# cafferychen777/flashdeconv

Hardware: AMD Instinct MI355X
Metric: spots/sec to convergence (1M x 2000 x 30) (higher is better)
Workload: dtype f64

## Files before the change

flashdeconv_amd/_lib.py:

```python
import ctypes
import os
import threading

import numpy as np

_HERE = os.path.dirname(os.path.abspath(__file__))
LIB_PATH = os.path.join(_HERE, "libfdx.so")

c_int = ctypes.c_int
c_i32 = ctypes.c_int32
c_i64 = ctypes.c_int64
c_double = ctypes.c_double
c_void_p = ctypes.c_void_p
c_size_t = ctypes.c_size_t
p_double = ctypes.POINTER(ctypes.c_double)
p_i64 = ctypes.POINTER(ctypes.c_int64)
p_i32 = ctypes.POINTER(ctypes.c_int32)


class FdxError(RuntimeError):
    """A libfdx call failed (message from fdx_last_error())."""


class SolveInfo(ctypes.Structure):
    _fields_ = [
        ("converged", c_i32),
        ("n_iterations", c_i32),
        ("final_objective", c_double),
        ("final_change", c_double),
        ("n_objectives", c_i32),
        ("reserved", c_i32),
        ("sweep_ms", c_double),
        ("total_ms", c_double),
    ]

    def as_dict(self, rel_changes=None, objective=True):
        n_it = int(self.n_iterations)
        d = {"converged": bool(self.converged), "n_iterations": n_it, "final_change": float(self.final_change)}
        if objective:
            d["final_objective"] = float(self.final_objective)
        if rel_changes is not None:
            d["rel_changes"] = [float(v) for v in rel_changes[:n_it]]
        return d


class FitParams(ctypes.Structure):
    _fields_ = [
        ("sketch_dim", c_i32), ("mode_y", c_i32), ("mode_x", c_i32), ("graph_method", c_i32), ("k_neighbors", c_i32),
        ("lambda_auto", c_i32), ("max_iter", c_i32), ("verbose", c_i32),
        ("radius", c_double), ("lambda_spatial", c_double), ("rho_sparsity", c_double), ("tol", c_double),
        ("stop_on_ties", c_i32), ("reserved", c_i32), ("carry", c_void_p), ("spot_diag_out_dev", c_void_p),
    ]


class ShardFitParams(ctypes.Structure):
    _fields_ = [("sketch_dim", c_i32), ("mode_y", c_i32), ("mode_x", c_i32), ("lambda_auto", c_i32), ("max_iter", c_i32),
                ("stop_on_ties", c_i32), ("lambda_spatial", c_double), ("rho_sparsity", c_double), ("tol", c_double),
                ("n_total_spots", c_i64), ("nnz_total", c_i64), ("X_dev", c_void_p)]


class ShardFitInfo(ctypes.Structure):
    _fields_ = [("status", c_i32), ("reserved", c_i32), ("nnz_total", c_i64), ("knn_ties_total", c_i64), ("own_nnz", c_i64),
                ("n_halo", c_i64), ("lambda_used", c_double), ("rho_effective", c_double), ("YtY", c_double), ("solve", SolveInfo)]


SHARD_FAR, SHARD_OVERFLOW, SHARD_TIES = 1, 2, 3


class CsrView(ctypes.Structure):
    _fields_ = [("indptr", c_void_p), ("indices", c_void_p), ("data", c_void_p), ("dtype", c_i32), ("n", c_i64),
                ("nnz", c_i64), ("G", c_i32), ("sorted_rows", c_i32)]


class FitInfo(ctypes.Structure):
    _fields_ = [
        ("solve", SolveInfo), ("lambda_used", c_double), ("rho_effective", c_double), ("YtY", c_double), ("nnz", c_i64),
        ("graph_ms", c_double), ("sketch_ms", c_double), ("gram_ms", c_double), ("solve_ms", c_double),
        ("finish_ms", c_double), ("total_ms", c_double), ("prologue_ms", c_double), ("span_ms", c_double),
        ("knn_ties", c_i64), ("status", c_i32), ("reserved", c_i32), ("carry", c_void_p), ("diag_ms", c_double),
    ]


FIT_TIES = 3


GRAPH_KNN, GRAPH_RADIUS, GRAPH_GIVEN = 0, 1, 2

SIGNATURES = {
    "fdx_column_sums_dev": (c_int, [c_void_p, c_i32, c_i64, c_i32, c_i64, p_double, c_void_p]),
    "fdx_leverage_scores": (c_int, [p_double, c_i32, c_i32, c_double, p_double]),
    "fdx_csr_check_dev": (c_int, [ctypes.POINTER(CsrView), c_void_p]),
    "fdx_csr_gene_moments_dev": (c_int, [ctypes.POINTER(CsrView), p_double, p_double, p_double, c_void_p]),
    "fdx_fit_csr_dev": (c_int, [ctypes.POINTER(CsrView), p_i32, c_i32, p_double, c_i32, p_i32, p_double, p_double, c_void_p,
                                c_i32, ctypes.POINTER(FitParams), ctypes.POINTER(c_void_p), c_void_p, c_void_p, p_double,
                                p_double, ctypes.POINTER(FitInfo), c_void_p]),
    "fdx_type_sums_dev": (c_int, [c_void_p, c_i32, c_i64, c_i32, c_i64, c_void_p, c_void_p, c_i32, c_i32, c_void_p, c_void_p]),
    "fdx_type_sums_csr_dev": (c_int, [ctypes.POINTER(CsrView), c_void_p, c_void_p, c_i32, c_i32, c_void_p, c_void_p]),
    "fdx_metrics_moments_dev": (c_int, [c_void_p, c_void_p, c_i32, c_i64, c_i32, c_i64, c_i64, c_double, c_double, c_void_p,
                                        p_double, p_i64, c_void_p]),
    "fdx_metrics_spearman_dev": (c_int, [c_void_p, c_void_p, c_i32, c_i64, c_i32, c_i64, c_i64, c_i32, p_double, c_void_p]),
    "fdx_metrics_evaluate_dev": (c_int, [c_void_p, c_void_p, c_i32, c_i64, c_i32, c_i64, c_i64, c_double, c_double, c_i32,
                                         c_void_p, p_double, p_i64, p_double, c_void_p]),
    "fdx_graph_build_radius_rows_dev": (c_int, [c_void_p, c_i64, c_i32, c_double, c_i64, c_i64, c_void_p, ctypes.POINTER(c_void_p)]),
    "fdx_graph_knn_lists_dev": (c_int, [c_void_p, c_i64, c_i32, c_i32, c_i64, c_i64, c_void_p, c_void_p, c_void_p,
                                        ctypes.POINTER(c_void_p)]),
    "fdx_graph_knn_lists_band_dev": (c_int, [c_void_p, c_i64, c_i32, c_i32, c_i64, c_i64, c_void_p, c_void_p, c_void_p,
                                             ctypes.POINTER(c_void_p)]),
    "fdx_graph_from_knn_lists_dev": (c_int, [c_void_p, c_void_p, c_void_p, c_i64, c_i64, c_void_p, ctypes.POINTER(c_void_p)]),
    "fdx_leverage_begin": (c_int, [p_double, c_i32, c_i32, c_double, ctypes.POINTER(c_void_p)]),
    "fdx_leverage_begin_opt": (c_int, [p_double, c_i32, c_i32, c_double, c_i32, ctypes.POINTER(c_void_p)]),
    "fdx_leverage_end": (c_int, [c_void_p, p_double]),
    "fdx_leverage_end_keep": (c_int, [c_void_p, p_double, ctypes.POINTER(c_void_p)]),
    "fdx_fit_dev": (c_int, [c_void_p, c_i32, c_i64, c_i32, c_i64, p_double, c_i32, p_i32, p_double, p_double, c_void_p,
                            c_i32, ctypes.POINTER(FitParams), ctypes.POINTER(c_void_p), c_void_p, c_void_p, p_double,
                            p_double, ctypes.POINTER(FitInfo), c_void_p]),
    "fdx_fit_carry_free": (c_int, [c_void_p]),
    "fdx_graph_build_dev": (c_int, [c_void_p, c_i64, c_i32, c_i32, c_i32, c_double, c_void_p, ctypes.POINTER(c_void_p)]),
    "fdx_graph_perm_dev": (c_int, [c_void_p, c_void_p, c_void_p]),
    "fdx_side_stream": (c_int, [ctypes.POINTER(c_void_p)]),
    "fdx_stream_wait_stream": (c_int, [c_void_p, c_void_p]),
    "fdx_graph_localize": (c_int, [c_void_p, c_i32, p_i64, c_i32, c_void_p, ctypes.POINTER(c_void_p)]),
    "fdx_graph_shard_knn_dev": (c_int, [c_void_p, c_i64, c_i32, c_i32, c_i32, p_i64, c_i32, c_void_p, ctypes.POINTER(c_void_p)]),
    "fdx_graph_shard_status": (c_int, [c_void_p, p_i64, p_i64, p_i32, p_i32]),
    "fdx_graph_row_indices": (c_int, [c_void_p, c_i64, p_i32, c_i32, p_i32]),
    "fdx_graph_tile_info": (c_int, [c_void_p, p_i32, p_i32, p_i32]),
    "fdx_graph_halo_info": (c_int, [c_void_p, p_i64, p_i32, p_i32]),
    "fdx_graph_send_indices_dev": (c_int, [c_void_p, c_void_p, c_void_p]),
    "fdx_prepare_dev": (c_int, [c_void_p, c_i32, c_i64, c_i32, c_i64, c_void_p, p_double, c_i32, p_i32, p_double, p_double,
                                c_i32, c_i32, c_i32, c_void_p, c_i64, c_void_p, p_double, p_double, c_void_p]),
    "fdx_init_beta_dev": (c_int, [c_void_p, c_i64, c_i64, c_i32, c_void_p]),
    "fdx_bcd_sweep_dev": (c_int, [c_void_p, c_void_p, c_i64, c_void_p, c_void_p, c_void_p, c_i64, c_i32, c_double, c_double,
                                  c_double, c_i32, c_void_p, c_void_p, c_void_p]),
    "fdx_bcd_fold_dev": (c_int, [c_void_p, c_void_p, c_i32, c_void_p]),
    "fdx_objective_partials_dev": (c_int, [c_void_p, c_void_p, c_i64, c_void_p, c_i64, c_void_p, c_i32, p_double, c_void_p]),
    "fdx_spot_diagnostics_dev": (c_int, [c_void_p, c_void_p, c_i64, c_void_p, c_i64, c_void_p, c_i32, c_i32, c_void_p, c_void_p,
                                         c_void_p]),
    "fdx_spatial_autocorr_dev": (c_int, [c_void_p, c_void_p, c_i64, c_i32, p_double, p_double, p_double, p_i64, c_void_p, c_void_p]),
    "fdx_spatial_perm_dev": (c_int, [c_void_p, c_void_p, c_i64, c_i32, ctypes.c_uint64, c_i64, c_i64, c_i32, c_void_p, p_double,
                                     p_double, p_double, p_i64, p_double, p_i64, p_i64, p_double, p_double, p_i32, c_void_p]),
    "fdx_permutation_indices_dev": (c_int, [ctypes.c_uint64, c_i64, c_i64, c_void_p, c_void_p]),
    "fdx_kmeans_assign_dev": (c_int, [c_void_p, c_i64, c_i64, c_i32, c_void_p, c_i32, c_void_p, c_void_p, p_i64, p_double, c_void_p]),
    "fdx_label_sums_dev": (c_int, [c_void_p, c_i64, c_i64, c_i32, c_void_p, c_i32, p_double, p_i64, c_void_p]),
    "fdx_kmeans_seed_dist_dev": (c_int, [c_void_p, c_i64, c_i64, c_i32, c_void_p, c_void_p, p_double, p_i64, p_i32, c_void_p]),
    "fdx_kmeans_dev": (c_int, [c_void_p, c_i64, c_i64, c_i32, c_i32, c_i32, c_void_p, c_void_p, p_i64, p_double, p_i32, p_i32,
                               c_void_p]),
    "fdx_normalize_dev": (c_int, [c_void_p, c_i64, c_i64, c_i32, c_void_p, c_void_p, c_void_p]),
    "fdx_export_dev": (c_int, [c_void_p, c_void_p, c_i64, c_i32, c_void_p, c_void_p, c_void_p]),
    "fdx_gene_moments_dev": (c_int, [c_void_p, c_i32, c_i64, c_i32, c_i64, p_double, p_double, c_void_p]),
    "fdx_gather_columns_dev": (c_int, [c_void_p, c_i32, c_i64, c_i32, c_i64, p_i32, c_i32, c_void_p, c_void_p]),
    "fdx_version": (c_int, []),
    "fdx_env_reload": (c_int, []),
    "fdx_env_switch": (ctypes.c_char_p, [c_i32, ctypes.POINTER(ctypes.c_char_p)]),
    "fdx_last_error": (ctypes.c_char_p, []),
    "fdx_device_count": (c_int, [ctypes.POINTER(c_int)]),
    "fdx_set_device": (c_int, [c_int]),
    "fdx_device_name": (c_int, [ctypes.c_char_p, c_int]),
    "fdx_malloc": (c_int, [ctypes.POINTER(c_void_p), c_size_t]),
    "fdx_free": (c_int, [c_void_p]),
    "fdx_trim": (c_int, []),
    "fdx_x_cache_stats": (c_int, [p_i64]),
    "fdx_memcpy_h2d": (c_int, [c_void_p, c_void_p, c_size_t, c_void_p]),
    "fdx_memcpy_d2h": (c_int, [c_void_p, c_void_p, c_size_t, c_void_p]),
    "fdx_memset": (c_int, [c_void_p, c_int, c_size_t, c_void_p]),
    "fdx_upload_convert_dev": (c_int, [c_void_p, c_i32, c_void_p, c_i32, c_i64, p_double, c_void_p]),
    "fdx_download_dev": (c_int, [c_void_p, c_void_p, c_size_t, c_void_p]),
    "fdx_pinned_copy_rate": (c_int, [c_size_t, c_i32, p_double]),
    "fdx_stream_sync": (c_int, [c_void_p]),
    "fdx_sketch": (c_int, [c_void_p, c_i32, c_i64, c_i32, p_i64, p_i32, p_double, c_i32, c_i32, p_double]),
    "fdx_prepare_csr_dev": (c_int, [ctypes.POINTER(CsrView), p_i32, c_i32, p_double, c_i32, p_i32, p_double, p_double, c_i32, c_i32,
                                    c_i32, c_void_p, c_i64, c_void_p, p_double, ctypes.POINTER(c_double), c_void_p]),
    "fdx_gram_xty": (c_int, [p_double, p_double, c_i64, c_i32, c_i32, p_double, p_double]),
    "fdx_objective": (c_int, [c_void_p, p_double, p_double, p_double, c_i64, c_i32, c_double, c_double, c_double, p_double]),
    "fdx_comm_unique_id": (c_int, [c_void_p]),
    "fdx_comm_init": (c_int, [c_void_p, c_i32, c_i32, ctypes.POINTER(c_void_p)]),
    "fdx_local_world_create": (c_int, [c_i32, ctypes.POINTER(c_void_p)]),
    "fdx_local_world_destroy": (c_int, [c_void_p]),
    "fdx_comm_init_local": (c_int, [c_void_p, c_i32, ctypes.POINTER(c_void_p)]),
    "fdx_comm_init_loopback": (c_int, [c_i32, c_i32, ctypes.POINTER(c_void_p)]),
    "fdx_comm_destroy": (c_int, [c_void_p]),
    "fdx_comm_info": (c_int, [c_void_p, p_i32, p_i32]),
    "fdx_comm_rccl_count": (c_int, [c_void_p, p_i32]),
    "fdx_comm_allreduce_sum_dev": (c_int, [c_void_p, c_void_p, c_i32, c_void_p]),
    "fdx_sharded_solve_dev": (c_int, [c_void_p, c_void_p, c_void_p, c_i64, c_void_p, c_i32, c_double, c_double, c_double, c_i32,
                                      c_void_p, c_void_p, c_i64, ctypes.POINTER(SolveInfo), p_double, p_i32, c_void_p]),
    "fdx_solver_padded_k": (c_i32, [c_i32]),
    "fdx_shard_fit_dev": (c_int, [c_void_p, c_void_p, c_void_p, c_i32, c_i64, c_i32, c_i64, p_double, c_i32, p_i32, p_double, p_double,
                                  ctypes.POINTER(ShardFitParams), c_void_p, c_void_p, p_double, ctypes.POINTER(ShardFitInfo), c_void_p]),
    "fdx_sharded_solve_padded_dev": (c_int, [c_void_p, c_void_p, c_void_p, c_i64, c_void_p, c_i32, c_i32, c_double, c_double, c_double,
                                             c_i32, c_void_p, c_void_p, c_i64, ctypes.POINTER(SolveInfo), p_double, p_i32, c_void_p]),
    "fdx_tile_schedule": (c_int, [p_i32, p_double, c_i32, c_i32, c_i32, c_i32, c_i32, p_i32, p_i32, c_void_p, p_i32, p_double,
                                  c_void_p, c_i64]),
    "fdx_sketch_path": (c_int, [c_i32, c_void_p, c_i64, c_i32, c_i32, c_i32, c_i32, p_i32, p_double, p_i32, p_i32]),
    "fdx_column_sums": (c_int, [c_void_p, c_i32, c_i64, c_i32, p_double]),
    "fdx_log1p_f32": (c_int, [c_void_p, ctypes.c_float, c_i64, c_void_p]),
    "fdx_graph_build_knn": (c_int, [p_double, c_i64, c_i32, c_i32, ctypes.POINTER(c_void_p)]),
    "fdx_graph_build_radius": (c_int, [p_double, c_i64, c_i32, c_double, ctypes.POINTER(c_void_p)]),
    "fdx_nearest_distance": (c_int, [p_double, c_i64, c_i32, p_double]),
    "fdx_graph_export_csr": (c_int, [c_void_p, p_i64, p_i32]),
    "fdx_graph_from_csr": (c_int, [p_i64, p_i64, c_i64, ctypes.POINTER(c_void_p)]),
    "fdx_graph_destroy": (c_int, [c_void_p]),
    "fdx_graph_info": (c_int, [c_void_p, p_i64, p_i64, p_i32]),
    "fdx_graph_knn_ties": (c_int, [c_void_p, p_i64]),
    "fdx_graph_knn_far": (c_int, [c_void_p, ctypes.POINTER(c_i32)]),
    "fdx_kdtree_set_threads": (c_int, [c_i32]),
    "fdx_kdtree_tune": (c_int, [c_i32, c_i64]),
    "fdx_ckdtree_indices_dev": (c_int, [c_void_p, c_i64, c_i32, p_i64, p_i32, c_void_p]),
    "fdx_ckdtree_prebuild": (c_int, [p_double, c_void_p, c_i64, c_i32]),
    "fdx_hvg_from_moments": (c_int, [p_double, p_double, c_i32, p_double, c_i32, c_i32, c_double, c_double, c_double, p_i64,
                                     ctypes.POINTER(c_i32), ctypes.POINTER(c_i32)]),
    "fdx_ckdtree_knn": (c_int, [p_double, c_i64, c_i32, c_i32, c_void_p, c_void_p]),
    "fdx_ckdtree_knn_rows": (c_int, [p_double, c_i64, c_i32, c_i32, p_i64, c_i64, c_void_p]),
    "fdx_graph_plan_set_ckdtree_lists_dev": (c_int, [c_void_p, p_double, c_void_p, c_i64, c_i32, c_void_p, c_i64, c_void_p, c_void_p, c_void_p]),
    "fdx_graph_plan_order_dev": (c_int, [c_void_p, c_void_p, c_void_p, c_void_p]),
    "fdx_graph_plan_lists_replaced": (c_int, [c_void_p]),
    "fdx_graph_plan_set_lists_dev": (c_int, [c_void_p, c_void_p, c_void_p, c_i64, c_void_p, c_void_p, c_void_p]),
    "fdx_bcd_solve": (c_int, [c_void_p, p_double, p_double, c_i64, c_i32, c_i32, c_double, c_double, c_i32, c_double,
                              c_i32, p_double, p_double, p_double, ctypes.POINTER(SolveInfo)]),
}

_lock = threading.Lock()
_lib = None


def _preload_shared_hip_runtime():
    import importlib.util
    try:
        spec = importlib.util.find_spec("torch")
    except (ImportError, ValueError):
        spec = None
    if spec is None or not spec.submodule_search_locations:
        return
    libdir = os.path.join(list(spec.submodule_search_locations)[0], "lib")
    for name in ("libhsa-runtime64.so", "libamdhip64.so"):
        path = os.path.join(libdir, name)
        if os.path.exists(path):
            try:
                ctypes.CDLL(path, mode=ctypes.RTLD_GLOBAL)
            except OSError:
                pass


def load():
    global _lib
    with _lock:
        if _lib is None:
            if not os.path.exists(LIB_PATH):
                raise FdxError(
                    f"{LIB_PATH} not found: build it with `make -C flashdeconv_amd/csrc` "
                    "(or `python -c 'import __graft_entry__ as g; g.build()'`). There is no CPU fallback.")
            _preload_shared_hip_runtime()
            lib = ctypes.CDLL(LIB_PATH)
            for name, (res, args) in SIGNATURES.items():
                fn = getattr(lib, name)
                fn.restype = res
                fn.argtypes = args
            _lib = lib
    return _lib


def env_reload():
    if _lib is not None:
        _lib.fdx_env_reload()


def runtime_switches():
    lib, out, i = load(), [], 0
    while True:
        what = ctypes.c_char_p()
        name = lib.fdx_env_switch(i, ctypes.byref(what))
        if not name:
            return out
        out.append((name.decode(), (what.value or b"").decode()))
        i += 1


def check(rc):
    if rc != 0:
        msg = load().fdx_last_error()
        raise FdxError(f"libfdx error {rc}: {msg.decode() if msg else 'unknown'}")


def require_gpu():
    lib = load()
    n = c_int(0)
    rc = lib.fdx_device_count(ctypes.byref(n))
    if rc != 0 or n.value <= 0:
        raise FdxError("flashdeconv_amd needs an AMD Instinct GPU (gfx950); no HIP device is visible "
                       "and there is no CPU fallback.")
    return n.value


def host_cpu_budget():
    cpus = float(len(os.sched_getaffinity(0))) if hasattr(os, "sched_getaffinity") else float(os.cpu_count() or 1)
    try:
        with open("/sys/fs/cgroup/cpu.max") as f:
            q, period = f.read().split()[:2]
        if q != "max" and float(period) > 0:
            cpus = min(cpus, float(q) / float(period))
    except (OSError, ValueError):
        try:
# ... 319 lines not shown
```

flashdeconv_amd/core/deconv.py:

```python
import ctypes
import os
import sys
import time

import numpy as np
from scipy import sparse

from .. import _lib
from ..utils import genes as _genes
from .sketching import sketch_tables

_PRE_MODES = ("log_cpm", "pearson", "raw")


def _is_torch_cuda(x):
    return hasattr(x, "data_ptr") and hasattr(x, "is_cuda") and bool(x.is_cuda)


def device_counts_as_float(Y):
    import torch
    f64_math = False
    if Y.dtype not in (torch.float32, torch.float64):
        f64_math = not Y.dtype.is_floating_point
        small = Y.dtype in (torch.uint8, torch.int8, torch.int16, torch.bool, torch.float16, torch.bfloat16)
# ... 284 lines not shown
                      file=sys.stderr)
            if G != G_all and csr is None:
                sub = _DeviceBuffer(n * G * (4 if y_code == _lib.FDX_F32 else 8))
                owned.append(sub)
                gi32 = np.ascontiguousarray(gene_idx, dtype=np.int32)
                _lib.check(lib.fdx_gather_columns_dev(y_ptr, y_code, n, G_all, G_all, _lib.ptr_i32(gi32), G, sub.ptr, None))
                y_ptr = sub.ptr
            ldy = G

            if big_k:
                from ..utils.graph import ckdtree_knn_adjacency
                t_graph = time.perf_counter()
                A = ckdtree_knn_adjacency(coords_host if coords_host is not None else _lib.tensor_to_host(coords), int(self.k_neighbors))
                self._graph = _lib.Graph.from_csr(A.indptr, A.indices, n)
                self._adjacency = A
            elif not graph_early:
                t_graph = time.perf_counter()
                gh = ctypes.c_void_p()
                _lib.check(lib.fdx_graph_build_dev(c_ptr, n, dim, g_method, g_k, g_radius, None, ctypes.byref(gh)))
                self._graph = _lib.Graph(gh.value)
            n_ties = 0
            if self.spatial_method == "knn" and self.knn_ties == "ckdtree" and not big_k:
                n_ties = self._graph.knn_ties()
                if n_ties:
                    self._graph.close()
                    self._graph = None
                    self._graph = reference_tie_graph(c_ptr, coords_host, n, dim, int(self.k_neighbors))
            t_lev = time.perf_counter()
            leverage = lev_job.result()
            t_done = time.perf_counter()

            log(f"Step 2: Preprocessing with method='{self.preprocess}'...")

            def y_colsum():
                if csr is not None:
                    return (csr_colsum if csr_colsum is not None else csr.gene_moments(want_colsum=True)[2])[gene_idx]
                sums = np.empty(G, dtype=np.float64)
                _lib.check(lib.fdx_column_sums_dev(y_ptr, y_code, n, G, ldy, _lib.ptr_f64(sums), None))
                return sums
            bucket32, wy, wx, mode_y, mode_x = sketch_tables(
                G, self.sketch_dim, leverage, self.random_state, self.preprocess, Xsel, y_sparse=y_sparse_rule,
                f64_math=y_f64_math and csr is None and y_code == _lib.FDX_F32, y_colsum=y_colsum, n_spots=n)
            log({"log_cpm": "  Y and X normalized to log-CPM space", "pearson": "  Y and X transformed with uncentered Pearson residuals",
                 "raw": "  No preprocessing applied (raw)"}[self.preprocess])
            log(f"Step 3: Sketching to {self.sketch_dim} dimensions...")
            log(f"  Compressed {G} genes -> {self.sketch_dim} dims")

            prm = _lib.FitParams()
            prm.sketch_dim = int(self.sketch_dim)
            prm.mode_y, prm.mode_x = mode_y, mode_x
            prm.k_neighbors = int(self.k_neighbors)
            prm.max_iter, prm.tol, prm.verbose = int(self.max_iter), float(self.tol), 1 if self.verbose else 0
            prm.rho_sparsity = float(self.rho_sparsity)
            prm.lambda_auto = 1 if self.lambda_spatial == "auto" else 0
            prm.lambda_spatial = 0.0 if prm.lambda_auto else float(self.lambda_spatial)
            prm.radius = 0.0
            prm.graph_method = _lib.GRAPH_GIVEN
            prm.stop_on_ties = 1 if (self.spatial_method == "knn" and self.knn_ties == "auto" and not big_k) else 0
            log("Step 4: Building spatial graph...")

            if output == "torch":
                import torch
                dev = Y.device if _is_torch_cuda(Y) else torch.device("cuda", torch.cuda.current_device())
                beta_t = torch.empty((n, K), dtype=torch.float64, device=dev)
                prop_t = torch.empty((n, K), dtype=torch.float64, device=dev)
                b_ptr, p_ptr = beta_t.data_ptr(), prop_t.data_ptr()
            else:
                bbuf, pbuf = _DeviceBuffer(n * K * 8), _DeviceBuffer(n * K * 8)
                owned += [bbuf, pbuf]
                b_ptr, p_ptr = bbuf.ptr, pbuf.ptr

            diag_t = dbuf = None
            if spot_diagnostics:
                if output == "torch":
                    diag_t = torch.empty(3 * n, dtype=torch.float64, device=dev)
                    prm.spot_diag_out_dev = diag_t.data_ptr()
                else:
                    dbuf = _DeviceBuffer(3 * n * 8)
                    owned.append(dbuf)
                    prm.spot_diag_out_dev = dbuf.ptr
            objs = np.zeros(max(int(self.max_iter), 1), dtype=np.float64)
            rels = np.zeros(max(int(self.max_iter), 1), dtype=np.float64)
            info = _lib.FitInfo()
            gh = ctypes.c_void_p(self._graph.handle.value)
            t_call = time.perf_counter()
            gi32 = np.ascontiguousarray(gene_idx, dtype=np.int32)

            def run_fit():
                if csr is not None:
                    _lib.check(lib.fdx_fit_csr_dev(ctypes.byref(csr.view), _lib.ptr_i32(gi32), G, _lib.ptr_f64(Xsel), K,
                                                   _lib.ptr_i32(bucket32), _lib.ptr_f64(wy), _lib.ptr_f64(wx), c_ptr, dim,
                                                   ctypes.byref(prm), ctypes.byref(gh), b_ptr, p_ptr, _lib.ptr_f64(objs),
                                                   _lib.ptr_f64(rels), ctypes.byref(info), None))
                else:
                    _lib.check(lib.fdx_fit_dev(y_ptr, y_code, n, G, ldy, _lib.ptr_f64(Xsel), K, _lib.ptr_i32(bucket32),
                                               _lib.ptr_f64(wy), _lib.ptr_f64(wx), c_ptr, dim, ctypes.byref(prm),
                                               ctypes.byref(gh), b_ptr, p_ptr, _lib.ptr_f64(objs), _lib.ptr_f64(rels),
                                               ctypes.byref(info), None))

            run_fit()
            ties_remedy_ms = 0.0
            if info.status == _lib.FIT_TIES:
                n_ties = int(info.knn_ties)
                log(f"k-NN ties on {n_ties} of {n} spots: rebuilding the graph on the reference's (cKDTree) neighbour choice")
                stale, carry = self._graph, info.carry
                self._graph = None
                try:
                    self._graph = reference_tie_graph(c_ptr, coords_host, n, dim, int(self.k_neighbors))
                    gh = ctypes.c_void_p(self._graph.handle.value)
                    prm.stop_on_ties = 0
                    prm.carry, carry = carry, None
                    ties_resolved_here = True
                    ties_remedy_ms = (time.perf_counter() - t_call) * 1e3
                    t_call = time.perf_counter()
                    run_fit()
                finally:
                    if carry:
                        lib.fdx_fit_carry_free(carry)
                    stale.close()
            else:
                ties_resolved_here = False
            t_ret = time.perf_counter()
            if os.environ.get("FDX_TRACE_HOST"):
                print(f"[fdx-host] python: entry->build {1e6 * (t_graph - t_entry):.0f} us, build call {1e6 * (t_lev - t_graph):.0f}, leverage wait "
                      f"{1e6 * (t_done - t_lev):.0f}, tables + setup {1e6 * (t_call - t_done):.0f}, fit call {1e6 * (t_ret - t_call):.0f}", file=sys.stderr)
            if output == "torch":
                self.beta_, self.proportions_ = beta_t, prop_t
            else:
                self.beta_ = bbuf.to_host((n, K), out=self._recyclable("beta_", (n, K)))
                self.proportions_ = pbuf.to_host((n, K), out=self._recyclable("proportions_", (n, K)))
            self.spot_diagnostics_ = None
            if spot_diagnostics:
                planes = diag_t if diag_t is not None else dbuf.to_host((3 * n,))
                self.spot_diagnostics_ = {name: planes[j * n:(j + 1) * n]
                                          for j, name in enumerate(("residual_sq", "sketch_sq", "neighbor_sq"))}
        finally:
            for b in owned:
                b.free()

        log(f"  Average neighbors per spot: {info.nnz / max(n, 1):.1f}")
        self.lambda_used_ = float(info.lambda_used)
        log(f"Step 5: {'Auto-tuned' if prm.lambda_auto else 'Using'} lambda = {self.lambda_used_:.4f}")
        log("Step 6: Solving via Block Coordinate Descent...")
        n_it = int(info.solve.n_iterations)
        objectives = [float(v) for v in objs[:info.solve.n_objectives]]
        if self.verbose:
            its = [t for t in range(n_it) if t % 10 == 0 or t == self.max_iter - 1]
            for t, obj in zip(its, objectives):
                print(f"Iteration {t}: objective = {obj:.6f}, rel_change = {rels[t]:.6e}")
            if info.solve.converged:
                print(f"Converged at iteration {n_it - 1}")
        self.info_ = info.solve.as_dict()
        self.info_["objectives"] = objectives if self.verbose else []
        resolved = self.spatial_method == "knn" and (self.knn_ties == "ckdtree" or ties_resolved_here)
        self.info_["knn_ties"] = (n_ties if resolved else int(info.knn_ties)) if self.spatial_method == "knn" else 0
        if self.info_["knn_ties"] and not resolved:
            import warnings
            warnings.warn(
                f"k-NN ties: {self.info_['knn_ties']} of {n} spots have their k-th and (k+1)-th nearest neighbours at exactly "
                "the same distance (regular lattice?), so the neighbour graph depends on how ties are broken - here by "
                "spot index, in the reference by cKDTree's traversal, i.e. by the order the spots are listed in.  "
                "Proportions can differ from the reference's by a few 1e-4 (relative); knn_ties='auto' (the default) or "
                "'ckdtree' reproduce the reference's choice (host-side, about a second per million spots), "
                "spatial_method='grid' builds a tie-free graph on lattices.", UserWarning, stacklevel=2)
        self.timings_ = _fit_timings(info, t_entry, t_graph, t_graph_done if graph_early else t_lev, t_sel, t_lev, t_done, t_call, t_ret,
                                     ties_remedy_ms, span_from_call=graph_early or ties_resolved_here or bool(resolved and n_ties))
        if spot_diagnostics:
            self.timings_["diagnostics_ms"] = float(info.diag_ms)
        self._fitted = True
        log(f"  Converged: {self.info_['converged']}")
        log(f"  Iterations: {self.info_['n_iterations']}")
        log("FlashDeconv: Done!")
        return self

    def _recyclable(self, name, shape):
        old = getattr(self, name, None)
        ok = (isinstance(old, np.ndarray) and old.shape == tuple(shape) and old.dtype == np.float64 and old.flags.c_contiguous
              and old.flags.owndata and old.flags.writeable and sys.getrefcount(old) <= 3)
        return old if ok else None

    def _graph_request(self, coords, coords_host):
        if self.spatial_method == "knn":
            return _lib.GRAPH_KNN, int(self.k_neighbors), 0.0
        if self.spatial_method == "radius":
            if self.radius is None:
                raise ValueError("radius must be specified for radius method")
            return _lib.GRAPH_RADIUS, 0, float(self.radius)
        if self.spatial_method == "grid":
            if coords.shape[0] < 2:
                return _lib.GRAPH_KNN, 0, 0.0
            from ..utils.graph import grid_radius
            ch = coords_host if coords_host is not None else _lib.tensor_to_host(coords)
            return _lib.GRAPH_RADIUS, 0, grid_radius(ch)
        raise ValueError(f"Unknown method: {self.spatial_method}. Choose from 'knn', 'radius', 'grid'.")

    def fit_transform(self, Y, X, coords, **kwargs):
        self.fit(Y, X, coords, **kwargs)
        return self.proportions_

    def _require_fitted(self):
        if not self._fitted:
            raise RuntimeError("Model has not been fitted. Call fit() first.")

    def get_cell_type_proportions(self):
        self._require_fitted()
        return self.proportions_

    def get_abundances(self):
        self._require_fitted()
        return self.beta_

    def get_spot_residuals(self, relative=True):
        self._require_fitted()
        if self.spot_diagnostics_ is None:
            raise RuntimeError("No per-spot diagnostics: call fit(..., spot_diagnostics=True) first.")
        res, sq = self.spot_diagnostics_["residual_sq"], self.spot_diagnostics_["sketch_sq"]
        if isinstance(res, np.ndarray):
            if not relative:
                return np.sqrt(res)
            return np.sqrt(np.divide(res, sq, out=np.zeros_like(res), where=sq > 0))
        import torch
        if not relative:
            return torch.sqrt(res)
        return torch.sqrt(torch.where(sq > 0, res / torch.where(sq > 0, sq, torch.ones_like(sq)), torch.zeros_like(res)))

    def get_spatial_autocorrelation(self, what="proportions", neighbor_mean=False, n_permutations=0, random_state=None):
        self._require_fitted()
        if what not in ("proportions", "abundances"):
            raise ValueError(f"Unknown what: {what}. Choose from 'proportions', 'abundances'.")
        from ..utils.spatial_stats import spatial_autocorrelation, spatial_permutation_test, spatial_sums
        values = self.proportions_ if what == "proportions" else self.beta_
        if isinstance(n_permutations, (bool, np.bool_)) or not isinstance(n_permutations, (int, np.integer)) or n_permutations < 0:
            raise ValueError(f"n_permutations must be an int >= 0, got {n_permutations!r}")
        if n_permutations == 0:
            return spatial_autocorrelation(values, self, neighbor_mean=neighbor_mean)
        out = spatial_permutation_test(values, self, n_permutations=n_permutations,
                                       random_state=self.random_state if random_state is None else random_state)
        if neighbor_mean:
            out["neighbor_mean"] = spatial_sums(values, self, neighbor_mean=True)["neighbor_mean"]
        return out

    def get_spatial_niches(self, n_niches, what="proportions", features="both", **kw):
        self._require_fitted()
        if what not in ("proportions", "abundances"):
            raise ValueError(f"Unknown what: {what}. Choose from 'proportions', 'abundances'.")
        from ..utils.niches import spatial_niches
        return spatial_niches(self.proportions_ if what == "proportions" else self.beta_, n_niches, graph=self, features=features,
                              **kw)

    def get_dominant_cell_type(self):
        self._require_fitted()
        if hasattr(self.proportions_, "argmax") and not isinstance(self.proportions_, np.ndarray):
            return self.proportions_.argmax(dim=1)
        return np.argmax(self.proportions_, axis=1)

    def summary(self):
        if not self._fitted:
            return {"fitted": False}
        return {
            "fitted": True,
            "n_spots": self.n_spots_,
            "n_cell_types": self.n_cell_types_,
            "n_genes_used": len(self.gene_idx_),
            "sketch_dim": self.sketch_dim,
            "lambda_spatial": self.lambda_used_,
            "rho_sparsity": self.rho_sparsity,
            "preprocess_method": self.preprocess,
            "converged": self.info_["converged"],
            "n_iterations": self.info_["n_iterations"],
            "final_objective": self.info_["final_objective"],
        }

    def __repr__(self):
        status = "fitted" if self._fitted else "not fitted"
        return f"FlashDeconv(sketch_dim={self.sketch_dim}, lambda_spatial={self.lambda_spatial}, status={status})"
```

flashdeconv_amd/csrc/bcd_sweep_inst.cpp:

```cpp
#include <algorithm>
#include <cstdlib>
#include "bcd_device.h"
#include "fdx_graph.h"

#ifndef FDX_PART
#error "compile with -DFDX_PART=<n> -DFDX_K_LO=<lo> -DFDX_K_HI=<hi>"
#endif

namespace fdx {

constexpr int sweep_chunk(int K) {
#ifdef FDX_KC_OVERRIDE
    return K < FDX_KC_OVERRIDE ? K : FDX_KC_OVERRIDE;
#endif
    return K < 8 ? K : K <= 29 ? 8 : K <= 33 ? 7 : K <= 37 ? 6 : K <= 41 ? 5 : K <= 45 ? 4 : K <= 49 ? 3 : K <= 51 ? 2 : K <= 64 ? 8 : K <= 72 ? 6 : K <= 88 ? 4 : K <= 96 ? 2 : 8;
}

template <int K, int KC>
__global__ __launch_bounds__(256) void bcd_sweep_kernel(
    const double* __restrict__ H, const double* __restrict__ XtX, const double* __restrict__ beta_in,
    double* __restrict__ beta_out, const int* __restrict__ ell_base, const int* __restrict__ slice_off,
    const int* __restrict__ deg, unsigned long long* __restrict__ stats, double* __restrict__ rel_change,
    const double lambda, const double rho, const double tol, const int ldh, const int ld_, const int n,
    const int n_slices, const int it) {
    const int lane = threadIdx.x & 63;
    const int wib = __builtin_amdgcn_readfirstlane(threadIdx.x >> 6);

    if (it > 0) {
        const double rc = fold_rel_change(stats + (size_t)(it - 1) * 128, lane);
        if (blockIdx.x == 0 && threadIdx.x == 0) rel_change[it - 1] = rc;
        if (rc < tol) return;
    }

    const int slice = xcd_remap(blockIdx.x, gridDim.x) * 4 + wib;
    if (slice >= n_slices) return;
    const int i = min(slice * 64 + lane, n - 1);
    const size_t ld = (size_t)ld_;

    const int w0 = slice_off[slice];
    const int w = slice_off[slice + 1] - w0;

    double b[K];
#pragma unroll
    for (int k = 0; k < K; ++k) b[k] = beta_in[k * ld + i];
    const int* ell = ell_base + (size_t)w0 * 64 + (i & 63);
    const int dg = deg[i];
    const double lam_deg = lambda * (double)dg;
    const double lam_eff = (dg > 0) ? lambda : 0.0;

    double dmax = 0.0, amax = 0.0;
#pragma unroll
    for (int kc = 0; kc < K; kc += KC) {
        double c[KC];
#pragma unroll
        for (int q = 0; q < KC; ++q) c[q] = 0.0;
#pragma unroll 2
        for (int m = 0; m < w; ++m) {
            const int j = ell[(size_t)m * 64];
#pragma unroll
            for (int q = 0; q < KC; ++q)
                if (kc + q < K) c[q] += beta_in[(kc + q) * ld + j];
        }
#pragma unroll
        for (int q = 0; q < KC; ++q) {
            const int k = kc + q;
            if (k < K) {
                const double h = H[k * (size_t)ldh + i];
                const double* g = XtX + k * K;
                double r0 = 0.0, r1 = 0.0;
#pragma unroll
                for (int j = 0; j + 1 < K; j += 2) {
                    r0 = fma(g[j], b[j], r0);
                    r1 = fma(g[j + 1], b[j + 1], r1);
                }
                if (K & 1) r0 = fma(g[K - 1], b[K - 1], r0);
                const double gkk = g[k];
                const double old = b[k];
                const double res = (h - (r0 + r1) + gkk * old) + lam_eff * c[q];
                const double den = gkk + lam_deg;
                const double st = res > rho ? res - rho : (res < -rho ? res + rho : 0.0);
                const double qv = fmax(0.0, st / den);
                const double nw = (den > 1e-10) ? qv : 0.0;
                dmax = fmax(dmax, fabs(nw - old));
                amax = fmax(amax, fabs(old));
                b[k] = nw;
                beta_out[k * ld + i] = nw;
            }
        }
    }
    dmax = wave_max(dmax);
    amax = wave_max(amax);
    if (lane == 0) {
        unsigned long long* s = stats + (size_t)it * 128;
        const int slot = slice & 63;
        atomicMax(s + slot, (unsigned long long)__double_as_longlong(dmax));
        atomicMax(s + 64 + slot, (unsigned long long)__double_as_longlong(amax));
    }
}

__device__ __forceinline__ const char __attribute__((address_space(1)))* plane_base(const double* p) {
    unsigned long long v = (unsigned long long)p;
    asm("" : "+s"(v));
    return (const char __attribute__((address_space(1)))*)v;
}

__device__ __forceinline__ unsigned lane_off(unsigned off) {
    asm("" : "+v"(off));
    return off;
}

#ifndef FDX_SWEEP_WPE
#define FDX_SWEEP_WPE 1
#endif
template <int K, int KC, bool OBJ, bool QUAD = true, bool INIT = false>
__global__ __launch_bounds__(256, ((OBJ && K > 40 && K <= 64) || (K > 64 && K <= 96)) ? 2 : (OBJ ? 1 : FDX_SWEEP_WPE)) void bcd_sweep_tiled_kernel(
    const double* __restrict__ H, const double* __restrict__ XtX, const double* __restrict__ beta_in,
    double* __restrict__ beta_out, const unsigned short* __restrict__ ell_local, const int* __restrict__ slice_off,
    const int* __restrict__ deg, const int* __restrict__ tile_halo, const int* __restrict__ tile_hcnt,
    unsigned long long* __restrict__ stats, double* __restrict__ rel_change, const double lambda, const double rho,
    const double tol, const int ldh, const int ld_, const int n, const int S, const int it,
    const int* __restrict__ tile_list, const double init_v, const int* __restrict__ send_head, const int4* __restrict__ send_ent,
    double* __restrict__ send_buf) {
    extern __shared__ __attribute__((aligned(16))) double lds[];
    const int tid = threadIdx.x;
    const int lane = tid & 63;
    const int tile = tile_list ? tile_list[xcd_remap(blockIdx.x, gridDim.x)] : xcd_remap(blockIdx.x, gridDim.x);
    const bool real = (tile * 256 + tid) < n;
    const int i = min(tile * 256 + tid, n - 1);
    const size_t ld = (size_t)ld_;
    const int slice = __builtin_amdgcn_readfirstlane(i >> 6);
    const int w0 = slice_off[slice];
    const int w = slice_off[slice + 1] - w0;
    const int Ht = tile_hcnt[tile];
    const int* halo = tile_halo + (size_t)tile * FDX_TILE_HALO_CAP;
    const int dg = deg[i];
    int hidx0 = halo[tid];
    if (!OBJ && it > 0) {
        const double rc = fold_rel_change(stats + (size_t)(it - 1) * 128, lane);
        if (blockIdx.x == 0 && tid == 0) rel_change[it - 1] = rc;
        asm volatile("" :: "v"(dg), "v"(hidx0), "s"(w0), "s"(w), "s"(Ht));
        if (rc < tol) return;
    }
    hidx0 = (tid < Ht) ? hidx0 : 0;

    const unsigned ioff = (unsigned)i * 8u, hoff = (unsigned)hidx0 * 8u;
#define PLANE_AT(base, off) (*(const double __attribute__((address_space(1)))*)(plane_base(base) + lane_off(off)))
    double b[K];
#pragma unroll
    for (int k = 0; k < K; ++k) b[k] = INIT ? init_v : PLANE_AT(beta_in + k * ld, ioff);
    const unsigned short* ell = ell_local + (size_t)w0 * 64 + (i & 63);
    const double lam_deg = lambda * (double)dg;
    const double lam_eff = (dg > 0) ? lambda : 0.0;
    unsigned slots[8];
    const unsigned zslot = (unsigned)(256 + Ht);
#pragma unroll
    for (int m2 = 0; m2 < 8; ++m2) {
        unsigned lo = (unsigned)__builtin_nontemporal_load(&ell[(size_t)(2 * m2) * 64]);
        unsigned hi = (unsigned)__builtin_nontemporal_load(&ell[(size_t)(2 * m2 + 1) * 64]);
        lo = (2 * m2 < w) ? lo : zslot;
        hi = (2 * m2 + 1 < w) ? hi : zslot;
        slots[m2] = lo | (hi << 16);
    }
    double hv[KC], hreg[KC];
#pragma unroll
    for (int q = 0; q < KC; ++q) {
        hv[q] = INIT ? init_v : PLANE_AT(beta_in + q * ld, hoff);
        hreg[q] = __builtin_nontemporal_load(&PLANE_AT(H + q * (size_t)ldh, ioff));
    }

    double dmax = 0.0, amax = 0.0;
    double o_cross = 0.0, o_quad = 0.0, o_spat = 0.0, o_l1 = 0.0;
#pragma unroll
    for (int kc = 0; kc < K; kc += KC) {
#pragma unroll
        for (int q = 0; q < KC; ++q)
            if (kc + q < K) lds[q * S + tid] = b[kc + q];
        if (tid < Ht) {
#pragma unroll
            for (int q = 0; q < KC; ++q)
                if (kc + q < K) lds[q * S + 256 + tid] = hv[q];
        }
        for (int h = tid + 256; h < Ht; h += 256) {
            const int j = halo[h];
#pragma unroll
            for (int q = 0; q < KC; ++q)
                if (kc + q < K) lds[q * S + 256 + h] = INIT ? init_v : beta_in[(kc + q) * ld + j];
        }
        if (tid < KC) lds[tid * S + 256 + Ht] = 0.0;
        __syncthreads();
        double c[KC];
#pragma unroll
        for (int q = 0; q < KC; ++q) c[q] = 0.0;
#pragma unroll
        for (int m4 = 0; m4 < 16; m4 += 4) {
            if (m4 < w) {
#pragma unroll
                for (int m = m4; m < m4 + 4; ++m) {
                    const int slot = (int)((slots[m >> 1] >> (16 * (m & 1))) & 0xffffu);
#pragma unroll
                    for (int q = 0; q < KC; ++q)
                        if (kc + q < K) c[q] += lds[q * S + slot];
                }
            }
        }
        for (int m = 16; m < w; ++m) {
            const int slot = ell[(size_t)m * 64];
#pragma unroll
            for (int q = 0; q < KC; ++q)
                if (kc + q < K) c[q] += lds[q * S + slot];
        }
        __syncthreads();
#pragma unroll
        for (int q = 0; q < KC; ++q) {
            const int k = kc + q;
            if (k < K) {
                const double h = hreg[q];
                const double* g = XtX + k * K;
                double r0 = 0.0, r1 = 0.0;
                if (!OBJ || QUAD) {
#pragma unroll
                    for (int j = 0; j + 1 < K; j += 2) {
                        r0 = fma(g[j], b[j], r0);
                        r1 = fma(g[j + 1], b[j + 1], r1);
                    }
                    if (K & 1) r0 = fma(g[K - 1], b[K - 1], r0);
                }
                const double gkk = (!OBJ || QUAD) ? g[k] : 0.0;
                const double old = b[k];
                if (OBJ) {
                    o_cross = fma(old, h, o_cross);
                    if (QUAD) o_quad = fma(old, r0 + r1, o_quad);
                    o_spat = fma(old, (double)dg * old - c[q], o_spat);
                    o_l1 += fabs(old);
                    asm volatile("" : "+v"(o_quad));
                } else {
                    const double res = (h - (r0 + r1) + gkk * old) + lam_eff * c[q];
                    const double den = gkk + lam_deg;
                    const double st = res > rho ? res - rho : (res < -rho ? res + rho : 0.0);
                    const double qv = fmax(0.0, st / den);
                    const double nw = (den > 1e-10) ? qv : 0.0;
                    dmax = fmax(dmax, fabs(nw - old));
                    amax = fmax(amax, fabs(old));
                    b[k] = nw;
                    __builtin_nontemporal_store(nw, (double __attribute__((address_space(1)))*)(plane_base(beta_out + k * ld) + lane_off(ioff)));
                }
            }
            if (kc + KC < K) {
#pragma unroll
                for (int t = 2 * q; t < 2 * q + 2; ++t) {
                    const int j = t < KC ? t : t - KC;
                    if (kc + KC + j < K) {
                        if (t < KC) { if (!INIT) hv[j] = PLANE_AT(beta_in + (kc + KC + j) * ld, hoff); }
                        else hreg[j] = __builtin_nontemporal_load(&PLANE_AT(H + (kc + KC + j) * (size_t)ldh, ioff));
                    }
                }
                __builtin_amdgcn_sched_barrier(0);
            }
        }
    }
    if (OBJ) {
        if (!real) { o_cross = o_quad = o_spat = o_l1 = 0.0; }
#pragma unroll
        for (int off = 32; off > 0; off >>= 1) {
            o_cross += __shfl_xor(o_cross, off, 64);
            o_quad += __shfl_xor(o_quad, off, 64);
            o_spat += __shfl_xor(o_spat, off, 64);
            o_l1 += __shfl_xor(o_l1, off, 64);
        }
        __syncthreads();
        if (lane == 0) { lds[(tid >> 6) * 4 + 0] = o_cross; lds[(tid >> 6) * 4 + 1] = o_quad; lds[(tid >> 6) * 4 + 2] = o_spat; lds[(tid >> 6) * 4 + 3] = o_l1; }
        __syncthreads();
        if (tid < 4) rel_change[(size_t)tile * 4 + tid] = ((lds[tid] + lds[4 + tid]) + lds[8 + tid]) + lds[12 + tid];
        return;
    }
    if (!OBJ && send_head != nullptr) {
        int hd = real ? send_head[i] : 0;
        while (hd != 0) {
            const int4 e = send_ent[hd - 1];
            double* o = send_buf + (size_t)K * e.x + e.z;
#pragma unroll
            for (int k = 0; k < K; ++k) o[(size_t)k * e.y] = b[k];
            hd = e.w;
        }
    }
    dmax = wave_max(dmax);
    amax = wave_max(amax);
    if (lane == 0) {
        unsigned long long* s = stats + (size_t)it * 128;
        const int slot = slice & 63;
        atomicMax(s + slot, (unsigned long long)__double_as_longlong(dmax));
        atomicMax(s + 64 + slot, (unsigned long long)__double_as_longlong(amax));
    }
}

template <int K>
static void launch_k(const BcdSweepArgs& a, hipStream_t st) {
    if (a.tiled) {
        constexpr int KC = sweep_chunk(K);
        const int S = 256 + a.halo_max + 1;
        const size_t lds = (size_t)KC * S * sizeof(double);
        if (lds <= 64 * 1024 && (long long)a.ld * 8 < (1LL << 32) && (long long)a.ldh * 8 < (1LL << 32)) {
            if (a.objective) {
                if constexpr (K > 64) {
                    hipLaunchKernelGGL((bcd_sweep_tiled_kernel<K, KC, true, false>), dim3(a.n_tiles), dim3(256), lds, st, a.H, a.XtX,
                                       a.beta_in, a.beta_out, a.ell_local, a.slice_off, a.deg, a.tile_halo, a.tile_hcnt,
                                       a.stats, a.rel_change, a.lambda, a.rho, a.tol, a.ldh, a.ld, a.n, S, a.it, nullptr, 0.0, a.send_head, a.send_ent, a.send_buf);
                } else {
                    hipLaunchKernelGGL((bcd_sweep_tiled_kernel<K, KC, true>), dim3(a.n_tiles), dim3(256), lds, st, a.H, a.XtX,
                                       a.beta_in, a.beta_out, a.ell_local, a.slice_off, a.deg, a.tile_halo, a.tile_hcnt,
                                       a.stats, a.rel_change, a.lambda, a.rho, a.tol, a.ldh, a.ld, a.n, S, a.it, nullptr, 0.0, a.send_head, a.send_ent, a.send_buf);
                }
            }
            else if (a.tile_list) {
                if (a.n_list > 0)
                    hipLaunchKernelGGL((bcd_sweep_tiled_kernel<K, KC, false>), dim3(a.n_list), dim3(256), lds, st, a.H, a.XtX,
                                       a.beta_in, a.beta_out, a.ell_local, a.slice_off, a.deg, a.tile_halo, a.tile_hcnt,
                                       a.stats, a.rel_change, a.lambda, a.rho, a.tol, a.ldh, a.ld, a.n, S, a.it, a.tile_list, 0.0, a.send_head, a.send_ent, a.send_buf);
            } else if (a.init_uniform != 0.0) {
                if constexpr (K <= 64) {
                    hipLaunchKernelGGL((bcd_sweep_tiled_kernel<K, KC, false, true, true>), dim3(a.n_tiles), dim3(256), lds, st, a.H, a.XtX,
                                       a.beta_in, a.beta_out, a.ell_local, a.slice_off, a.deg, a.tile_halo, a.tile_hcnt,
                                       a.stats, a.rel_change, a.lambda, a.rho, a.tol, a.ldh, a.ld, a.n, S, a.it, nullptr, a.init_uniform, a.send_head, a.send_ent, a.send_buf);
                }
            } else {
                hipLaunchKernelGGL((bcd_sweep_tiled_kernel<K, KC, false>), dim3(a.n_tiles), dim3(256), lds, st, a.H, a.XtX,
                                   a.beta_in, a.beta_out, a.ell_local, a.slice_off, a.deg, a.tile_halo, a.tile_hcnt,
                                   a.stats, a.rel_change, a.lambda, a.rho, a.tol, a.ldh, a.ld, a.n, S, a.it, nullptr, 0.0, a.send_head, a.send_ent, a.send_buf);
            }
            return;
        }
    }
    const int nblk = ceil_div(a.n_slices, 4);
    hipLaunchKernelGGL((bcd_sweep_kernel<K, sweep_chunk(K)>), dim3(nblk), dim3(256), 0, st, a.H, a.XtX, a.beta_in,
                       a.beta_out, a.ell, a.slice_off, a.deg, a.stats, a.rel_change, a.lambda, a.rho, a.tol, a.ldh,
                       a.ld, a.n, a.n_slices, a.it);
}

#ifndef FDX_K_STEP
#define FDX_K_STEP 1
#endif
template <int... Is>
static bool dispatch_range(const BcdSweepArgs& a, hipStream_t st, std::integer_sequence<int, Is...>) {
    bool hit = false;
    (void)std::initializer_list<int>{((a.K == FDX_K_LO + Is * FDX_K_STEP) ? (launch_k<FDX_K_LO + Is * FDX_K_STEP>(a, st), hit = true, 0) : 0)...};
    return hit;
}

#define FDX_CAT2(a, b) a##b
#define FDX_CAT(a, b) FDX_CAT2(a, b)
bool FDX_CAT(bcd_sweep_dispatch_part, FDX_PART)(const BcdSweepArgs& a, hipStream_t st) {
    if (a.K < FDX_K_LO || a.K > FDX_K_HI) return false;
    return dispatch_range(a, st, std::make_integer_sequence<int, (FDX_K_HI - FDX_K_LO) / FDX_K_STEP + 1>{});
}

}
```

flashdeconv_amd/csrc/capi_dev.cpp:

```cpp
#include "fdx_env.h"
#include <algorithm>
#include <cmath>
#include <memory>
#include <vector>

#include "fdx_graph.h"
#include "fdx_internal.h"
#include "fdx_kernels.h"
#include "graph_build.h"
#include "prepare.h"
#include "sketch_plan.h"
#include "solver.h"

using namespace fdx;

extern "C" {

int fdx_graph_build_dev(const double* coords_dev, int64_t n, int32_t dim, int32_t method, int32_t k, double radius,
                        void* stream, fdx_graph** out) {
    PoolStream pool_stream((hipStream_t)stream);
    FDX_REQUIRE(out != nullptr, "fdx_graph_build_dev: null output");
    *out = nullptr;
    FDX_REQUIRE(n == 0 || coords_dev != nullptr, "fdx_graph_build_dev: null coords");
    fdx_graph* g = new fdx_graph();
// ... 408 lines not shown
    FDX_TRY(out.alloc(plan.out_doubles * sizeof(double)));
    const int* perm = (g->identity_order || !g->perm.p) ? nullptr : g->perm.as<int>();
    FDX_TRY(launch_spatial_perm(plan, V_dev, ldv, (int)g->n, K, g->ell.as<int>(), g->slice_off.as<int>(), g->deg.as<int>(), perm,
                                seed, first_perm, n_perm, null_dev, scratch.as<double>(), out.as<double>(), st));
    std::vector<double> host(plan.out_doubles);
    FDX_TRY(copy_d2h(host.data(), out.p, plan.out_doubles * sizeof(double), st));
    const double* h = host.data();
    std::copy(h, h + K, mean_out);
    std::copy(h + K, h + 2 * (size_t)K, m2_out);
    std::copy(h + 2 * (size_t)K, h + 2 * (size_t)K + KK, C_out);
    std::memcpy(counts_out + 1, h + 2 * (size_t)K + KK, 2 * sizeof(int64_t));
    h += plan.s.out_doubles;
    std::copy(h, h + K, m4_out);
    std::memcpy(count_ge_out, h + K, KK * sizeof(int64_t));
    std::memcpy(count_le_out, h + K + KK, KK * sizeof(int64_t));
    std::copy(h + K + 2 * KK, h + K + 3 * KK, sum_d_out);
    std::copy(h + K + 3 * KK, h + K + 4 * KK, sumsq_d_out);
    return 0;
}

int fdx_permutation_indices_dev(uint64_t seed, int64_t r, int64_t n, int32_t* out_dev, void* stream) {
    FDX_REQUIRE(n >= 0 && n < (1LL << 31) - 128, "fdx_permutation_indices_dev: n must be between 0 and 2^31 - 129");
    FDX_REQUIRE(r >= 0, "fdx_permutation_indices_dev: r must not be negative");
    FDX_REQUIRE(n == 0 || out_dev, "fdx_permutation_indices_dev: null argument");
    return launch_permutation_indices(seed, r, (int)n, out_dev, (hipStream_t)stream);
}

}

static int kmeans_check_shape(const char* who, int64_t ldf, int64_t n, int32_t D, int32_t C, bool centres_are_rows) {
    const std::string w(who);
    FDX_REQUIRE(D >= 1, w + ": D must be positive");
    FDX_REQUIRE(ldf >= D, w + ": ldf must be at least D");
    FDX_REQUIRE(C >= 1 && C <= 64, w + ": C must be between 1 and 64");
    FDX_REQUIRE(n >= 0 && n < (1LL << 31) - 128, w + ": too many rows");
    if (centres_are_rows) FDX_REQUIRE(C <= n, w + ": C must not exceed n");
    return 0;
}

extern "C" {

int fdx_kmeans_assign_dev(const double* F_dev, int64_t ldf, int64_t n, int32_t D, const double* centres_dev, int32_t C,
                          int32_t* labels_dev, double* min_d2_dev, int64_t* changed_out, double* inertia_out, void* stream) {
    FDX_REQUIRE(F_dev && centres_dev && labels_dev && changed_out && inertia_out, "fdx_kmeans_assign_dev: null argument");
    FDX_TRY(kmeans_check_shape("fdx_kmeans_assign_dev", ldf, n, D, C, true));
    hipStream_t st = (hipStream_t)stream;
    PoolStream pool_stream(st);
    const KmeansPlan plan = kmeans_plan(n, D, C);
    DevBuf part, out;
    FDX_TRY(part.alloc(plan.dist_part_bytes));
    FDX_TRY(out.alloc(16));
    FDX_TRY(launch_kmeans_assign(plan, F_dev, ldf, (int)n, D, centres_dev, C, labels_dev, min_d2_dev, part.p, out.as<long long>(),
                                 out.as<double>() + 1, st));
    unsigned char host[16];
    FDX_TRY(copy_d2h(host, out.p, 16, st));
    std::memcpy(changed_out, host, 8);
    std::memcpy(inertia_out, host + 8, 8);
    return 0;
}

int fdx_label_sums_dev(const double* F_dev, int64_t ldf, int64_t n, int32_t D, const int32_t* labels_dev, int32_t C,
                       double* sums_out, int64_t* counts_out, void* stream) {
    FDX_REQUIRE(sums_out && counts_out && (n == 0 || (F_dev && labels_dev)), "fdx_label_sums_dev: null argument");
    FDX_TRY(kmeans_check_shape("fdx_label_sums_dev", ldf, n, D, C, false));
    const size_t CD = (size_t)C * D;
    std::fill(sums_out, sums_out + CD, 0.0);
    std::fill(counts_out, counts_out + C, (int64_t)0);
    if (n == 0) return 0;
    hipStream_t st = (hipStream_t)stream;
    PoolStream pool_stream(st);
    const KmeansPlan plan = kmeans_plan(n, D, C);
    DevBuf part, out;
    FDX_TRY(part.alloc(plan.sums_part_bytes));
    FDX_TRY(out.alloc((CD + C) * 8));
    FDX_TRY(launch_label_sums(plan, F_dev, ldf, labels_dev, (int)n, D, C, part.p, out.as<double>(),
                              reinterpret_cast<long long*>(out.as<double>() + CD), nullptr, st));
    std::vector<double> host(CD + C);
    FDX_TRY(copy_d2h(host.data(), out.p, (CD + C) * 8, st));
    std::copy(host.begin(), host.begin() + CD, sums_out);
    std::memcpy(counts_out, host.data() + CD, (size_t)C * 8);
    return 0;
}

int fdx_kmeans_seed_dist_dev(const double* F_dev, int64_t ldf, int64_t n, int32_t D, const double* centre_dev, double* d2_dev,
                             double* block_sums_out, int64_t* block_rows_out, int32_t* n_blocks_out, void* stream) {
    FDX_REQUIRE(F_dev && centre_dev && d2_dev && block_sums_out && block_rows_out && n_blocks_out,
                "fdx_kmeans_seed_dist_dev: null argument");
    FDX_TRY(kmeans_check_shape("fdx_kmeans_seed_dist_dev", ldf, n, D, 1, true));
    hipStream_t st = (hipStream_t)stream;
    PoolStream pool_stream(st);
    const KmeansPlan plan = kmeans_plan(n, D, 1);
    DevBuf part, out;
    FDX_TRY(part.alloc(plan.dist_part_bytes));
    FDX_TRY(out.alloc((size_t)plan.seed_blocks * 8));
    FDX_TRY(launch_kmeans_seed_dist(plan, F_dev, ldf, (int)n, D, centre_dev, d2_dev, part.p, out.as<double>(), st));
    FDX_TRY(copy_d2h(block_sums_out, out.p, (size_t)plan.seed_blocks * 8, st));
    *block_rows_out = plan.seed_rows;
    *n_blocks_out = plan.seed_blocks;
    return 0;
}

int fdx_kmeans_dev(const double* F_dev, int64_t ldf, int64_t n, int32_t D, int32_t C, int32_t max_iter, double* centres_dev,
                   int32_t* labels_dev, int64_t* counts_out, double* inertia_out, int32_t* n_iter_out, int32_t* converged_out,
                   void* stream) {
    FDX_REQUIRE(F_dev && centres_dev && labels_dev && counts_out && inertia_out && n_iter_out && converged_out,
                "fdx_kmeans_dev: null argument");
    FDX_TRY(kmeans_check_shape("fdx_kmeans_dev", ldf, n, D, C, true));
    FDX_REQUIRE(max_iter >= 1, "fdx_kmeans_dev: max_iter must be positive");
    hipStream_t st = (hipStream_t)stream;
    PoolStream pool_stream(st);
    const KmeansPlan plan = kmeans_plan(n, D, C);
    const size_t CD = (size_t)C * D;
    DevBuf dist_part, sums_part, out;
    FDX_TRY(dist_part.alloc(plan.dist_part_bytes));
    FDX_TRY(sums_part.alloc(plan.sums_part_bytes));
    FDX_TRY(out.alloc(16 + (CD + C) * 8));
    long long* changed_d = out.as<long long>();
    double* inertia_d = out.as<double>() + 1;
    double* sums_d = out.as<double>() + 2;
    long long* counts_d = reinterpret_cast<long long*>(sums_d + CD);
    FDX_HIP(hipMemsetAsync(labels_dev, 0xFF, (size_t)n * sizeof(int32_t), st));
    int it = 0, converged = 0;
    unsigned char host[16];
    for (;;) {
        ++it;
        FDX_TRY(launch_kmeans_assign(plan, F_dev, ldf, (int)n, D, centres_dev, C, labels_dev, nullptr, dist_part.p, changed_d,
                                     inertia_d, st));
        FDX_TRY(copy_d2h(host, out.p, 16, st));
        int64_t changed;
        std::memcpy(&changed, host, 8);
        if (changed == 0) { converged = 1; break; }
        if (it == max_iter) break;
        FDX_TRY(launch_label_sums(plan, F_dev, ldf, labels_dev, (int)n, D, C, sums_part.p, sums_d, counts_d, centres_dev, st));
    }
    FDX_TRY(launch_label_sums(plan, nullptr, ldf, labels_dev, (int)n, D, C, sums_part.p, sums_d, counts_d, nullptr, st));
    FDX_TRY(copy_d2h(counts_out, counts_d, (size_t)C * 8, st));
    std::memcpy(inertia_out, host + 8, 8);
    *n_iter_out = it;
    *converged_out = converged;
    return 0;
}

int fdx_export_dev(const fdx_graph* g, const double* beta_dev, int64_t ld, int32_t K, double* beta_out_dev, double* prop_out_dev,
                   void* stream) {
    FDX_TRY(fdx::graph_meta_sync(g));
    FDX_REQUIRE(g && beta_dev && K > 0, "fdx_export_dev: bad arguments");
    FDX_REQUIRE(ld >= g->n, "fdx_export_dev: ld must cover the own spots");
    FDX_REQUIRE(g->world_n == 0 && g->n_total == g->n, "fdx_export_dev: a shard's local graph is refused (its perm holds global ids)");
    if (g->n == 0) return 0;
    const int* perm = (g->identity_order || !g->perm.p) ? nullptr : g->perm.as<int>();
    return launch_normalize_export(beta_dev, ld, perm, (int)g->n, g->n_slices, K, beta_out_dev, prop_out_dev, (hipStream_t)stream);
}

int fdx_normalize_dev(const double* beta_dev, int64_t ld, int64_t n, int32_t K, double* beta_out_dev, double* prop_out_dev,
                      void* stream) {
    FDX_REQUIRE(beta_dev && n >= 0 && K > 0, "fdx_normalize_dev: bad arguments");
    if (n == 0) return 0;
    return launch_normalize_export(beta_dev, ld, nullptr, (int)n, (int)((n + 63) / 64), K, beta_out_dev, prop_out_dev,
                                   (hipStream_t)stream);
}

}

extern "C" int fdx_gene_moments_dev(const void* Y_dev, int32_t dtype, int64_t n, int32_t G, int64_t ldy, double* mean_out_host,
                                    double* var_out_host, void* stream) {
    FDX_REQUIRE(Y_dev && mean_out_host && var_out_host && n > 0 && G > 0, "fdx_gene_moments_dev: bad arguments");
    hipStream_t st = (hipStream_t)stream;
    PoolStream pool_stream(st);
    DevBuf scale, part, mean, var;
    FDX_TRY(scale.alloc((size_t)n * 8));
    FDX_TRY(part.alloc((size_t)column_sums_parts(n) * 2 * G * 8));
    FDX_TRY(mean.alloc((size_t)G * 8));
    FDX_TRY(var.alloc((size_t)G * 8));
    FDX_TRY(launch_gene_moments(Y_dev, dtype, ldy, n, G, scale.as<double>(), part.as<double>(), mean.as<double>(), var.as<double>(), st));
    FDX_TRY(copy_d2h(mean_out_host, mean.p, (size_t)G * 8, st));
    FDX_TRY(copy_d2h(var_out_host, var.p, (size_t)G * 8, st));
    return 0;
}

extern "C" int fdx_gather_columns_dev(const void* Y_dev, int32_t dtype, int64_t n, int32_t G, int64_t ldy, const int32_t* idx_host,
                                      int32_t G_sel, void* out_dev, void* stream) {
    FDX_REQUIRE(n >= 0 && G > 0 && G_sel > 0 && idx_host && (n == 0 || (Y_dev && out_dev)), "fdx_gather_columns_dev: bad arguments");
    for (int j = 0; j < G_sel; ++j) FDX_REQUIRE(idx_host[j] >= 0 && idx_host[j] < G, "fdx_gather_columns_dev: column index out of range");
    hipStream_t st = (hipStream_t)stream;
    PoolStream pool_stream(st);
    DevBuf di;
    FDX_TRY(di.alloc((size_t)G_sel * 4));
    FDX_TRY(copy_h2d(di.p, idx_host, (size_t)G_sel * 4, st));
    FDX_TRY(launch_gather_columns(Y_dev, dtype, ldy, n, G, di.as<int>(), G_sel, out_dev, st));
    FDX_HIP(hipStreamSynchronize(st));
    return 0;
}
```

flashdeconv_amd/csrc/fdx_env.cpp:

```cpp
#include "fdx_env.h"

#include <atomic>
#include <chrono>
#include <cstdio>
#include <cstdlib>
#include <cstring>
#include <deque>
#include <mutex>
#include <string>

#include "fdx_internal.h"

namespace fdx {
namespace {

struct Switch {
    const char* name;
    const char* what;
    std::atomic<const char*> value{nullptr};
};

Switch g_switches[] = {
    {"FDX_TRACE_HOST", "host time between the marked points of a fit / a graph build (stderr)"},
    {"FDX_DEBUG", "one-line reports of the routes taken (leverage route, ELL rebuilds)"},
    {"FDX_NO_LOG_TABLE", "log1p without the per-row table of the 64 small counts (bit-identical: tests)"},
    {"FDX_GRAPH_WCAP", "ELL width bound of a graph build: forces the 'bound too small' rebuild / remedy (tests)"},
    {"FDX_GRAPH_WCAP_RANK", "... on this rank of a shard plan only"},
    {"FDX_NO_TILED", "global-gather sweep instead of the LDS-tiled one"},
    {"FDX_NO_INIT_SWEEP", "first sweep reads a written start vector instead of the constant 1/K"},
    {"FDX_SPLIT_MIN_TILES", "tiles from which a shard sweeps boundary and interior separately"},
    {"FDX_NO_OVERLAP", "sharded loop: one sweep launch per iteration, halo on the compute stream"},
    {"FDX_NO_FUSED", "two-kernel sketch -> H (scatter + contraction) instead of the tile kernel"},
    {"FDX_NO_TILE_WIDE", "no wide tile kernel (K > 32 / d > 704): the two-kernel path takes those shapes"},
    {"FDX_TILE_LOGV", "0: float64 log1p chain for float32 rows in the tile kernel"},
    {"FDX_SKETCH_GATHER", "gather form of the row sketch kernel"},
    {"FDX_GRAPH_SORT", "Morton order by a radix sort instead of by counting"},
    {"FDX_GRAPH_SYNC", "graph build completed inside the call (no deferred counts)"},
    {"FDX_GRAPH_TWO_ELL_KERNELS", "fill_ell + tile_halo as two kernels"},
    {"FDX_NO_FUSED_PACK", "sharded loop: halo_pack_kernel instead of the sweep writing the send staging"},
    {"FDX_LEV_ONE_WG", "leverage scores by the single-workgroup route"},
    {"FDX_KDTREE_HOST_QUERIES", "tie remedy: cKDTree queries on host threads instead of kd_query_kernel"},
    {"FDX_KDTREE_THREADS", "host threads of the restated cKDTree (build forks, host queries)"},
    {"FDX_KDTREE_PAR_DEPTH", "fork depth of the restated cKDTree build"},
    {"FDX_NO_PLAN_CACHE", "sketch plans / tile schedules, leverage scores and the X side recomputed every fit (bench.py: cold_ms)"},
    {"FDX_NO_SIDE_STREAM", "everything on the caller's stream"},
    {"FDX_CSR_KEEP_CAP", "entries per wave of the fused CSR sketch's keep buffer (tests: rows that overflow it)"},
};
constexpr int kSwitches = sizeof(g_switches) / sizeof(g_switches[0]);
std::once_flag g_once;
std::mutex g_mu;
std::atomic<bool> g_trace_host{false};

const char* lookup(const char* name) {
    for (const Switch& s : g_switches)
        if (std::strcmp(s.name, name) == 0) return s.value.load(std::memory_order_acquire);
    return nullptr;
}

void load_all() {
    static std::deque<std::string>* const kept = new std::deque<std::string>();
    std::lock_guard<std::mutex> lk(g_mu);
    for (Switch& s : g_switches) {
        const char* v = getenv(s.name);
        const char* cur = s.value.load(std::memory_order_relaxed);
        if (v && cur && std::strcmp(v, cur) == 0) continue;
        if (v) {
            kept->emplace_back(v);
            v = kept->back().c_str();
        }
        s.value.store(v, std::memory_order_release);
    }
    g_trace_host.store(lookup("FDX_TRACE_HOST") != nullptr, std::memory_order_relaxed);
}

}

const char* env(const char* name) {
    std::call_once(g_once, load_all);
    return lookup(name);
}

void trace_host(const char* scope, const char* what) {
    std::call_once(g_once, load_all);
    if (!g_trace_host.load(std::memory_order_relaxed)) return;
    thread_local auto t_prev = std::chrono::steady_clock::now();
    const auto t = std::chrono::steady_clock::now();
    std::fprintf(stderr, "[fdx-host] +%7.1f us  %s%s%s\n", std::chrono::duration<double, std::micro>(t - t_prev).count(),
                 scope ? scope : "", scope ? ": " : "", what);
    t_prev = t;
}

void env_reload() {
    std::call_once(g_once, load_all);
    load_all();
}

}

extern "C" int fdx_env_reload(void) {
    fdx::env_reload();
    return 0;
}

extern "C" const char* fdx_env_switch(int32_t i, const char** what_out) {
    if (i < 0 || i >= fdx::kSwitches) return nullptr;
    if (what_out) *what_out = fdx::g_switches[i].what;
    return fdx::g_switches[i].name;
}
```

flashdeconv_amd/csrc/fdx_kernels.h:

```cpp
#pragma once
#include <cstdlib>
#include <hip/hip_runtime.h>

#include <cstddef>
#include <cstdint>
#include <utility>
#include <initializer_list>

namespace fdx {

constexpr int FDX_MAX_K_FAST = 64;
constexpr int FDX_MAX_K_PAD = 96;
inline int solver_padded_K(int K) {
    if (K <= FDX_MAX_K_FAST || K > FDX_MAX_K_PAD) return K;
    for (int kp : {72, 80, 88, 96})
        if (K <= kp) return kp;
    return K;
}
inline bool sweep_instantiated(int K) { return K >= 1 && (K <= FDX_MAX_K_FAST || K == 72 || K == 80 || K == 88 || K == 96); }

struct BcdSweepArgs {
    const double* H;
    const double* XtX;
    const double* beta_in;
    double* beta_out;
    const int* ell;
    const int* slice_off;
    const int* deg;
    const unsigned short* ell_local = nullptr;
    const int* tile_halo = nullptr;
    const int* tile_hcnt = nullptr;
    int n_tiles = 0;
    int halo_max = 0;
    int tiled = 0;
    int objective = 0;
    int skip_quad = 0;
    const int* tile_list = nullptr;
    int n_list = 0;
    const int* send_head = nullptr;
    const int4* send_ent = nullptr;
    double* send_buf = nullptr;
    double init_uniform = 0.0;
    unsigned long long* stats;
    double* rel_change;
    double lambda;
    double rho;
    double tol;
    int ldh;
    int ld;
    int n;
    int n_slices;
    int K;
    int it;
};

struct SketchPlanDev {
    const int* sched_gene = nullptr;
    const double* sched_w = nullptr;
    const int* group_off = nullptr;
    const int* slot_bucket = nullptr;
    int n_groups = 0;
    int total_len = 0;
    const unsigned int* sched_pack = nullptr;
    unsigned long long end_mask = 0ULL;
    int pack_ok = 0;
    const double* gene_w = nullptr;
    const int* gene_bucket = nullptr;
    int scatter_ok = 0;
    const struct SketchPlan* owner = nullptr;
};
inline bool sketch_scatter_fits(int G, int d) {
    return d < 65535 && (((size_t)G + 256 + 7) & ~(size_t)7) * 10 + ((size_t)d + 64) * 8 <= 150 * 1024;
}
int launch_sketch_rows(const void* Y, int dtype, long long ldy, const int* row_map, long long n, int G, int d, int mode,
                       const SketchPlanDev& plan, double* Ys, long long ldys, double* row_sumsq, hipStream_t st);
bool fused_sketch_contract_ok(int dtype, long long ldy, const void* Y, int G, int d, int K, int mode, const SketchPlanDev& plan,
                              hipStream_t st = nullptr);
struct TileF64Math {
    bool prev;
    explicit TileF64Math(bool on);
    ~TileF64Math();
};
bool tile_sketch_ok(int dtype, long long ldy, const void* Y, int G, int d, int K, int mode, const SketchPlanDev& plan, hipStream_t st);
int launch_tile_sketch(const void* Y, int dtype, long long ldy, const int* row_map, long long n, int G, int d, int mode,
                       const SketchPlanDev& plan, const double* Xs, int K, double* H, long long ldh, double* row_sumsq,
                       hipStream_t st);
int launch_sketch_contract(const void* Y, int dtype, long long ldy, const int* row_map, long long n, int G, int d, int mode,
                           const SketchPlanDev& plan, const double* Xs, int K, double* H, long long ldh, double* row_sumsq,
                           hipStream_t st);
int column_sums_parts(long long n);
int launch_column_sums(const void* Y, int dtype, long long ldy, long long n, int G, double* partials, double* out,
                       hipStream_t st);

int launch_xyt(const double* Xs, const double* Ys, long long ldy, long long n, int d, int K, double* Hout,
               long long ldh, double* sumsq_partials, hipStream_t st);
long long xyt_partials_count(long long n);
int launch_sum_partials(const double* in, long long count, double* out, int n_out, long long stride, hipStream_t st);

int objective_partials_count(int n_slices);
int launch_objective_partials(const double* beta, long long ld, const double* H, long long ldh, const double* XtX,
                              const int* ell, const int* slice_off, const int* deg, int n, int n_slices, int K,
                              double* partials, hipStream_t st, int skip_quad = 0);
int launch_normalize_export(const double* beta, long long ld, const int* perm, int n, int n_slices, int K,
                            double* beta_out, double* prop_out, hipStream_t st);
int launch_spot_diagnostics(const double* beta, long long ld, const double* H, long long ldh, const double* XtX, int ldg,
                            const double* row_sq, const int* ell, const int* slice_off, const int* deg, const int* perm, int n,
                            int n_slices, int K, double* out, hipStream_t st);

struct SpatialStatsPlan {
    long long ld;
    int n_slices;
    int colsum_blocks, rows_per_block, centre_blocks, lag_blocks, cross_blocks, pair_tiles_1d;
    size_t partials_doubles;
    size_t scratch_doubles;
    size_t out_doubles;
};
SpatialStatsPlan spatial_stats_plan(long long n, int K);
int launch_spatial_stats(const SpatialStatsPlan& s, const double* V, long long ldv, int n, int K, const int* ell,
                         const int* slice_off, const int* deg, const int* perm, double* scratch, double* out, double* nbr_mean,
                         hipStream_t st);
struct SpatialPermPlan {
    SpatialStatsPlan s;
    int batch, m4_blocks;
    size_t plane_doubles;
    size_t cross_part_doubles;
    size_t part_doubles;
    size_t null_doubles;
    size_t scratch_doubles;
    size_t out_doubles;
};
SpatialPermPlan spatial_perm_plan(long long n, int K, long long n_perm, int max_batch, bool own_null);
int launch_spatial_perm(const SpatialPermPlan& p, const double* V, long long ldv, int n, int K, const int* ell,
                        const int* slice_off, const int* deg, const int* perm, unsigned long long seed, long long first_perm,
                        long long n_perm, double* null_dev, double* scratch, double* out, hipStream_t st);
int launch_permutation_indices(unsigned long long seed, long long r, int n, int* out, hipStream_t st);

struct KmeansPlan {
    int dist_blocks;
    int seed_per, seed_blocks;
    long long seed_rows;
    int sums_blocks, rows_per_block;
    size_t dist_part_bytes;
    size_t sums_part_bytes;
};
KmeansPlan kmeans_plan(long long n, int D, int C);
int launch_kmeans_assign(const KmeansPlan& p, const double* F, long long ldf, int n, int D, const double* M, int C, int* labels,
                         double* min_d2, void* dist_part, long long* changed_out, double* inertia_out, hipStream_t st);
int launch_kmeans_seed_dist(const KmeansPlan& p, const double* F, long long ldf, int n, int D, const double* m, double* d2,
                            void* dist_part, double* block_sums, hipStream_t st);
int launch_label_sums(const KmeansPlan& p, const double* F, long long ldf, const int* labels, int n, int D, int C, void* sums_part,
                      double* sums, long long* counts, double* centres, hipStream_t st);

int launch_bcd_sweep(const BcdSweepArgs& a, double* generic_scratch, size_t scratch_ld, hipStream_t st);
bool sweep_uses_lds(int K);
size_t sweep_lds_pad_doubles(int K);
int sweep_lds_prepare(const double* XtX, int K, double* padded, hipStream_t st);
bool bcd_sweep_uses_tiles(const BcdSweepArgs& a);
int launch_bcd_objective_tiled(const BcdSweepArgs& a, double* partials , hipStream_t st);
int launch_bcd_fold_last(const unsigned long long* stats, double* rel_change, int it, hipStream_t st);
int launch_beta_quad(const double* beta, long long ld, long long n, int K, const double* XtX, double* partials, int rows,
                     hipStream_t st);

}

namespace fdx {
size_t leverage_scratch_doubles(int K, int G);
constexpr int LEV_ROUTE_SVD = 0, LEV_ROUTE_QR = 1;
bool leverage_qr_applies(int K, int G);
int launch_leverage(const double* X, int K, int G, double reg, double* work, double* sig2, double* lev, int* sweeps,
                    double* scratch, hipStream_t st, int route = LEV_ROUTE_SVD);
}

namespace fdx {
int launch_sketch_csr(const long long* indptr, const int* indices, const void* data, int dtype, const int* row_map,
                      long long row0, long long n, int d, int mode, const void* table, const unsigned* sel_bits,
                      int sel_words, double* Ys, long long ldys, double* row_sumsq, hipStream_t st);
bool csr_contract_ok(int d, int K, int sel_words);
struct CsrSelection;
int launch_sketch_csr_contract(const long long* indptr, const int* indices, const void* data, int dtype, const int* row_map,
                               long long n, int d, int mode, const CsrSelection& sel, const double* Xs, int K, double* H,
                               long long ldh, double* row_sumsq, hipStream_t st);
int csr_moment_stripes(long long n);
int launch_csr_moments(const long long* indptr, const int* indices, const void* data, int dtype, long long n, long long nnz, int G,
                       double* scale, double* part, double* mean, double* var, double* colsum, bool sorted_rows, hipStream_t st);
int launch_csr_check(const long long* indptr, const int* indices, long long n, long long nnz, int G, int check_sorted, int* flag,
                     hipStream_t st);
}

namespace fdx {
int launch_gene_moments(const void* Y, int dtype, long long ldy, long long n, int G, double* scale, double* partials,
                        double* mean, double* var, hipStream_t st);
int launch_gather_columns(const void* Y, int dtype, long long ldy, long long n, int G, const int* idx, int Gs, void* out,
                          hipStream_t st);
}
```

flashdeconv_amd/csrc/fit.cpp:

```cpp
#include "fdx_env.h"
#include <algorithm>
#include <cstdio>
#include <cmath>
#include <cstdlib>
#include <memory>
#include <vector>

#include "fdx_graph.h"
#include "fdx_internal.h"
#include "fdx_kernels.h"
#include "graph_build.h"
#include "prepare.h"
#include "sketch_plan.h"
#include "solver.h"
#include "x_cache.h"

using namespace fdx;

namespace {

int build_csc_from_tables(const int32_t* bucket, const double* weight, int G, int d, std::vector<long long>* col_ptr,
                          std::vector<int>* gene_idx, std::vector<double>* w) {
    col_ptr->assign((size_t)d + 1, 0);
    for (int g = 0; g < G; ++g) {
        FDX_REQUIRE(bucket[g] >= 0 && bucket[g] < d, "fit: bucket index out of range");
        (*col_ptr)[(size_t)bucket[g] + 1]++;
    }
    for (int c = 0; c < d; ++c) (*col_ptr)[(size_t)c + 1] += (*col_ptr)[(size_t)c];
    gene_idx->assign((size_t)G, 0);
    w->assign((size_t)G, 0.0);
    std::vector<long long> cur(col_ptr->begin(), col_ptr->end() - 1);
    for (int g = 0; g < G; ++g) {
        const long long e = cur[(size_t)bucket[g]]++;
        (*gene_idx)[(size_t)e] = g;
        (*w)[(size_t)e] = weight[g];
    }
    return 0;
}

}

struct LevEntry {
    XCacheKey key;
    std::vector<double> X;
    std::vector<double> scores;
    int route = LEV_ROUTE_SVD;
    int dbg[8] = {0};
};
static XCache<LevEntry>& lev_cache() {
    static XCache<LevEntry>* const c = new XCache<LevEntry>(4);
    return *c;
}
namespace fdx {
void leverage_cache_clear() { lev_cache().clear(); }
void leverage_cache_stats(long long* hits, long long* misses) { lev_cache().stats(hits, misses); }
}

struct fdx_leverage_job {
    double* pin = nullptr;
    size_t pin_cap = 0;
    Event done;
    double* hX = nullptr;
    size_t hX_cap = 0;
    ~fdx_leverage_job() {
        if (pin) fdx::pinned_buffer_put(pin, pin_cap);
        if (hX) fdx::pinned_buffer_put(hX, hX_cap);
    }
    DevBuf dX, dW, dS, dL, dDbg, dScratch;
    int K = 0, G = 0, route = LEV_ROUTE_SVD;
    double reg = 0.0;
    hipStream_t st = nullptr;
    std::shared_ptr<fdx::HelperTicket> ticket;
    std::shared_ptr<LevEntry> hit;
    bool cacheable = false;
    int route0 = LEV_ROUTE_SVD;
};

namespace fdx {
hipStream_t library_side_stream() {
    static hipStream_t streams[64] = {};
    int dev = 0;
    if (hipGetDevice(&dev) != hipSuccess || dev < 0 || dev >= 64) return nullptr;
    if (!streams[dev]) {
        int lo = 0, hi = 0;
        (void)hipDeviceGetStreamPriorityRange(&lo, &hi);
        if (hipStreamCreateWithPriority(&streams[dev], hipStreamNonBlocking, hi) != hipSuccess &&
            hipStreamCreateWithFlags(&streams[dev], hipStreamNonBlocking) != hipSuccess)
            streams[dev] = nullptr;
    }
    return streams[dev];
}
}

extern "C" int fdx_leverage_begin(const double* X, int32_t K, int32_t G, double regularization, fdx_leverage_job** out) {
    return fdx_leverage_begin_opt(X, K, G, regularization, 1, out);
}

extern "C" int fdx_leverage_begin_opt(const double* X, int32_t K, int32_t G, double regularization, int32_t queue_async,
                                      fdx_leverage_job** out) {
    FDX_REQUIRE(X && out && K > 0 && G > 0, "fdx_leverage_begin: bad arguments");
    *out = nullptr;
    auto* job = new fdx_leverage_job();
    job->K = K;
    job->G = G;
    job->reg = regularization;
    job->route0 = leverage_qr_applies(K, G) ? LEV_ROUTE_QR : LEV_ROUTE_SVD;
    if (!fdx::env("FDX_NO_PLAN_CACHE")) {
        XCacheKey key;
        key.K = K; key.G = G; key.reg = regularization; key.route = job->route0; key.X = X;
        job->hit = lev_cache().find(key);
        if (job->hit) {
            *out = job;
            return 0;
        }
        job->cacheable = true;
    }
    job->st = library_side_stream();
    job->hX = (double*)pinned_buffer_get((size_t)K * G * sizeof(double), &job->hX_cap);
    if (!job->hX) { delete job; return fail(FDX_ERR_HIP, "fdx_leverage_begin: pinned host buffer"); }
    std::memcpy(job->hX, X, (size_t)K * G * sizeof(double));
    const bool async = queue_async != 0;
    auto run = [job, K, G, regularization]() -> int {
        PoolStream pool_stream(job->st);
        FDX_TRY(job->dX.alloc((size_t)K * G * sizeof(double)));
        FDX_TRY(job->dW.alloc((size_t)K * G * sizeof(double)));
        FDX_TRY(job->dS.alloc((size_t)K * sizeof(double)));
        FDX_TRY(job->dL.alloc((size_t)G * sizeof(double)));
        FDX_TRY(job->dDbg.alloc(8 * sizeof(int)));
        FDX_HIP(hipMemcpyAsync(job->dX.p, job->hX, (size_t)K * G * sizeof(double), hipMemcpyHostToDevice, job->st));
        FDX_TRY(job->dScratch.alloc(leverage_scratch_doubles(K, G) * sizeof(double)));
        job->route = job->route0;
        FDX_TRY(launch_leverage(job->dX.as<double>(), K, G, regularization, job->dW.as<double>(), job->dS.as<double>(),
                                job->dL.as<double>(), job->dDbg.as<int>(), job->dScratch.as<double>(), job->st, job->route));
        job->pin = (double*)pinned_buffer_get((size_t)G * sizeof(double) + 64, &job->pin_cap);
        FDX_REQUIRE(job->pin != nullptr, "fdx_leverage_begin: pinned host buffer");
        FDX_HIP(hipMemcpyAsync(job->pin, job->dL.p, (size_t)G * sizeof(double), hipMemcpyDeviceToHost, job->st));
        FDX_HIP(hipMemcpyAsync(job->pin + G, job->dDbg.p, 8 * sizeof(int), hipMemcpyDeviceToHost, job->st));
        return job->done.record(job->st);
    };
    if (async) {
        job->ticket = helper_submit(run);
        *out = job;
        return 0;
    }
    const int rc = run();
    if (rc) {
        (void)hipStreamSynchronize(job->st);
        delete job;
        return rc;
    }
    *out = job;
    return 0;
}

static int leverage_end_impl(fdx_leverage_job* job, double* lev_out, double** x_dev_out);
extern "C" int fdx_leverage_end(fdx_leverage_job* job, double* lev_out) { return leverage_end_impl(job, lev_out, nullptr); }
extern "C" int fdx_leverage_end_keep(fdx_leverage_job* job, double* lev_out, double** x_dev_out) {
// ... 127 lines not shown
extern "C" int fdx_fit_carry_free(void* carry) {
    delete static_cast<fdx_fit_carry*>(carry);
    return 0;
}

namespace {

std::unique_ptr<fdx_fit_carry> adopt_carry(const fdx_fit_params* prm) {
    return std::unique_ptr<fdx_fit_carry>(prm ? static_cast<fdx_fit_carry*>(prm->carry) : nullptr);
}

int fit_impl(const YSource& ysrc, int64_t n, int32_t G, const double* X, int32_t K, const int32_t* bucket,
             const double* weight_y, const double* weight_x, const double* coords_dev, int32_t dim,
             const fdx_fit_params* prm_in, std::unique_ptr<fdx_fit_carry> carry_in, fdx_graph** graph_inout, double* beta_out_dev,
             double* prop_out_dev, double* objectives_out, double* rel_changes_out, fdx_fit_info* info, void* stream) {
    FDX_REQUIRE(info != nullptr && prm_in != nullptr && graph_inout != nullptr, "fdx_fit_dev: null argument");
    fdx_fit_params prm_local = *prm_in;
    prm_local.mode_y &= 0xff;
    const fdx_fit_params* prm = &prm_local;
    TileF64Math f64_math((prm_in->mode_y & FDX_PRE_F64_MATH) != 0);
    std::memset(info, 0, sizeof(*info));
    const int32_t y_dtype = ysrc.row_dtype();
    FDX_REQUIRE(y_dtype == FDX_F32 || y_dtype == FDX_F64, "fdx_fit_dev: Y dtype must be FDX_F32 or FDX_F64");
    FDX_REQUIRE(n > 0 && G > 0 && K > 0, "fdx_fit_dev: empty problem");
    FDX_REQUIRE(n < 0x7fffff00LL, "fdx_fit_dev: n too large for one device");
    FDX_REQUIRE(ysrc.csr || ysrc.ldy >= G, "fdx_fit_dev: ldy < G");
    FDX_REQUIRE((ysrc.dense || ysrc.csr) && X && bucket && weight_y && weight_x, "fdx_fit_dev: null array");
    const int d = prm->sketch_dim;
    FDX_REQUIRE(d > 0, "fdx_fit_dev: sketch_dim must be positive");
    FDX_REQUIRE(prm->max_iter >= 0, "fdx_fit_dev: max_iter must be non-negative");
    hipStream_t st = (hipStream_t)stream;
    PoolStream pool_stream(st);
    Event t_begin(true), t_graph(true), eS0(true), eS1(true), t_solved(true), t_end(true);
    FDX_TRY(t_begin.record(st));
    trace_host("fit", "entry");

    fdx_graph* g = nullptr;
    if (prm->graph_method == FDX_GRAPH_GIVEN) {
        g = *graph_inout;
        FDX_REQUIRE(g != nullptr && g->n == n, "fdx_fit_dev: given graph does not match n");
    } else {
        FDX_REQUIRE(coords_dev != nullptr, "fdx_fit_dev: null coords");
        g = new fdx_graph();
        int rc = (prm->graph_method == FDX_GRAPH_KNN)
                     ? graph_build_knn(coords_dev, n, dim, prm->k_neighbors, g, st)
                     : graph_build_radius(coords_dev, n, dim, prm->radius, 0, n, g, st);
        if (rc) { delete g; return rc; }
        *graph_inout = g;
    }
    if (g->meta_pending && g->meta_event && g->meta_stream != st) FDX_HIP(hipStreamWaitEvent(st, g->meta_event, 0));
    FDX_TRY(t_graph.record(st));

    const long long ld = round_up(n + 1, 64);
    const int KP = solver_padded_K(K);
    DevBuf dB0, dB1, dH, dSum;
    XSide x;
    YTables tables;
    RowsToH rows;
    struct SideDrain { hipStream_t s = nullptr; ~SideDrain() { if (s) (void)hipStreamSynchronize(s); } } side_drain;
    struct AbortDrain { hipStream_t s; bool armed = true; ~AbortDrain() { if (armed) (void)hipStreamSynchronize(s); } } abort_drain{st};
    Event evInit, evG;
    hipStream_t side = fdx::env("FDX_NO_SIDE_STREAM") ? nullptr : library_side_stream();
    if (side == st) side = nullptr;
    const hipStream_t xs = side ? side : st;
    if (side) side_drain.s = side;
    for (int g_ = 0; g_ < G; ++g_) FDX_REQUIRE(bucket[g_] >= 0 && bucket[g_] < d, "fit: bucket index out of range");
    double* Gh = (double*)pinned_scratch(0, (size_t)K * K * sizeof(double));
    FDX_REQUIRE(Gh != nullptr, "fit: pinned host buffer");
    const bool beta0_virtual = side && KP == K && K <= FDX_MAX_K_FAST && prm->max_iter > 0 && !prm->verbose && !fdx::env("FDX_NO_INIT_SWEEP");
    {
        PoolStream pool_xs(xs);
        FDX_TRY(dB0.alloc((size_t)KP * ld * sizeof(double)));
        FDX_TRY(dB1.alloc((size_t)KP * ld * sizeof(double)));
        if (side) {
            if (beta0_virtual) FDX_TRY(solver_zero_pad(dB0.as<double>(), ld, g->n_total, KP, xs));
            else FDX_TRY(solver_init_beta(dB0.as<double>(), ld, g->n_total, K, xs, KP));
            FDX_TRY(solver_zero_pad(dB1.as<double>(), ld, g->n_total, KP, xs));
        }
        FDX_TRY(tables.build(ysrc, G, d, K, bucket, weight_y, xs, "fdx_fit_csr_dev"));
    }
    if (weight_x == weight_y) x.plan = tables.plan;
    FDX_TRY(queue_x_side(&x, X, nullptr, K, KP, G, d, prm->mode_x, bucket, weight_x, nullptr, Gh, &evG, xs));
    if (side) {
        FDX_TRY(evInit.record(side));
        FDX_TRY(evInit.wait_on(st));
    }
    const double* XtX_dev = x.XtX(K, KP);

    if (carry_in) {
        FDX_REQUIRE(carry_in->n == n && carry_in->ld == ld && carry_in->K == K && carry_in->KP == KP && carry_in->d == d &&
                        carry_in->G == G && carry_in->mode_y == prm->mode_y && carry_in->y_id == ysrc.id(),
                    "fdx_fit_dev: the carry belongs to a different problem");
    } else {
        FDX_TRY(dH.alloc((size_t)KP * ld * sizeof(double)));
        if (KP != K) FDX_HIP(hipMemsetAsync(dH.as<double>() + (size_t)K * ld, 0, (size_t)(KP - K) * ld * sizeof(double), st));
        FDX_TRY(solver_zero_pad(dH.as<double>(), ld, n, K, st));
    }
    FDX_TRY(dSum.alloc(sizeof(double)));
    const int* row_map = g->identity_order ? nullptr : g->perm.as<int>();
    trace_host("fit", "side-stream preamble queued, buffers allocated");
    FDX_TRY(eS0.record(st));
    if (carry_in) {
        FDX_TRY(carry_in->done.wait_on(st));
        dH.take(carry_in->dH);
        rows.dRowSq.take(carry_in->dRowSq);
        rows.fused = carry_in->fused;
        rows.gram_ms = carry_in->gram_ms;
    } else {
        FDX_TRY(queue_rows_to_h(ysrc, tables, n, G, d, K, prm->mode_y, row_map, x.Xs(), dH.as<double>(), ld, true, &rows, st));
    }
    FDX_TRY(eS1.record(st));
    if (!prm->verbose && evG) FDX_TRY(evG.sync());
    if (!prm->verbose) x_side_publish(&x, X, Gh);
    FDX_TRY(graph_meta_sync(g));
    info->knn_ties = g->knn_ties;
    info->nnz = g->nnz;
    if (prm->stop_on_ties && g->knn_ties > 0) {
        info->status = FDX_FIT_TIES;
        if (carry_in) return 0;
        auto carry = std::make_unique<fdx_fit_carry>();
        FDX_TRY(carry->done.record(st));
        carry->dH.take(dH);
        carry->dRowSq.take(rows.dRowSq);
        carry->xs = x.b;
        carry->tables = std::move(tables);
        carry->n = n; carry->ld = ld; carry->K = K; carry->KP = KP; carry->d = d; carry->G = G; carry->mode_y = prm->mode_y;
        carry->y_id = ysrc.id();
        carry->fused = rows.fused;
        carry->gram_ms = rows.gram_ms;
        if (!rows.fused) FDX_HIP(hipStreamSynchronize(st));
        info->carry = carry.release();
        abort_drain.armed = false;
        return 0;
    }
    double* YtY_h = (double*)pinned_scratch(1, sizeof(double));
    FDX_REQUIRE(YtY_h != nullptr, "fit: pinned host buffer");
    *YtY_h = 0.0;
    Event evY;
    FDX_TRY(queue_yty(rows.dRowSq.as<double>(), n, dSum.as<double>(), YtY_h, &evY, st, (side && !prm->verbose) ? side : st));
    if (prm->verbose) {
        FDX_HIP(hipStreamSynchronize(st));
        x_side_publish(&x, X, Gh);
    }
    trace_host("fit", "sketch queued, XtX on the host");
    const double diag_mean = xtx_diag_mean(Gh, K);
    const double lambda = prm->lambda_auto ? auto_lambda(diag_mean, (double)g->nnz / (double)n) : prm->lambda_spatial;

    SolveProblem p;
    p.graph = g; p.H = dH.as<double>(); p.ldh = ld; p.XtX = XtX_dev;
    p.beta[0] = dB0.as<double>(); p.beta[1] = dB1.as<double>(); p.ld = ld; p.K = KP; p.K_real = K; p.YtY = prm->verbose ? *YtY_h : 0.0;
    p.lambda = lambda; p.rho_eff = prm->rho_sparsity * diag_mean; p.max_iter = prm->max_iter; p.tol = prm->tol;
    p.verbose = prm->verbose;
    p.compute_objective = prm->verbose ? 1 : 0;
    SolveResult r;
    if (evInit) {
        p.init_beta = 0;
        p.beta0_virtual = beta0_virtual ? 1 : 0;
        FDX_TRY(evInit.wait_on(st));
    }
    FDX_TRY(solver_run(p, &r, st));
    Event evSolved, evExported;
    if ((beta_out_dev || prop_out_dev) && !prm->verbose && side) {
        FDX_TRY(evSolved.record(st));
        FDX_TRY(evSolved.wait_on(side));
        FDX_TRY(launch_normalize_export(p.beta[r.result_buffer], ld, row_map, (int)n, g->n_slices, K, beta_out_dev,
                                        prop_out_dev, side));
        FDX_TRY(evExported.record(side));
    }
    if (!prm->verbose) {
        DevBuf objp, objo;
        FDX_TRY(objp.alloc((size_t)std::max(objective_partials_count(g->n_slices), g->n_tiles) * 4 * sizeof(double)));
        FDX_TRY(objo.alloc(4 * sizeof(double)));
        if (prm->max_iter == 0) FDX_HIP(hipStreamSynchronize(st));
        if (evY) FDX_TRY(evY.sync());
        FDX_TRY(solver_objective(*g, p.beta[r.result_buffer], ld, p.H, ld, p.XtX, KP, *YtY_h, lambda, p.rho_eff, objp.as<double>(),
                                 objo.as<double>(), &r.final_objective, st));
    }
    FDX_TRY(t_solved.record(st));
    if (evExported) FDX_TRY(evExported.wait_on(st));
    else if (beta_out_dev || prop_out_dev)
        FDX_TRY(launch_normalize_export(p.beta[r.result_buffer], ld, row_map, (int)n, g->n_slices, K, beta_out_dev,
                                        prop_out_dev, st));
    Event t_diag0(true), t_diag1(true);
    if (prm->spot_diag_out_dev) {
        FDX_TRY(t_diag0.record(st));
        FDX_TRY(launch_spot_diagnostics(p.beta[r.result_buffer], ld, p.H, ld, XtX_dev, KP, rows.dRowSq.as<double>(), g->ell.as<int>(),
                                        g->slice_off.as<int>(), g->deg.as<int>(), row_map, (int)n, g->n_slices, K,
                                        prm->spot_diag_out_dev, st));
        FDX_TRY(t_diag1.record(st));
    }
    FDX_TRY(t_end.record(st));
    FDX_HIP(hipStreamSynchronize(st));
    abort_drain.armed = false;

    info->solve.converged = r.converged;
    info->solve.n_iterations = r.n_iterations;
    info->solve.final_objective = r.final_objective;
    info->solve.final_change = r.final_change;
    info->solve.n_objectives = (int32_t)r.objectives.size();
    info->solve.sweep_ms = r.sweep_ms;
    info->lambda_used = lambda;
    info->rho_effective = p.rho_eff;
    info->YtY = *YtY_h;
    info->nnz = g->nnz;
    info->graph_ms = t_graph.ms_since(t_begin.e);
    info->sketch_ms = rows.fused ? eS1.ms_since(eS0.e) : rows.sketch_ms;
    info->gram_ms = rows.gram_ms;
    const bool from_build = g->begin_event && g->begin_stream == st && prm->graph_method == FDX_GRAPH_GIVEN;
    const hipEvent_t t0 = from_build ? g->begin_event : t_begin.e;
    info->prologue_ms = eS0.ms_since(t0);
    info->span_ms = t_end.ms_since(t0);
    if (from_build) {
        (void)hipEventDestroy(g->begin_event);
        g->begin_event = nullptr;
        g->begin_stream = nullptr;
    }
    info->solve_ms = t_solved.ms_since(eS1.e);
    info->finish_ms = t_end.ms_since(t_solved.e);
    info->diag_ms = t_diag1.ms_since(t_diag0.e);
    info->total_ms = t_end.ms_since(t_begin.e);
    info->solve.total_ms = info->total_ms;
    if (objectives_out)
        for (size_t t = 0; t < r.objectives.size(); ++t) objectives_out[t] = r.objectives[t];
    if (rel_changes_out)
        for (size_t t = 0; t < r.rel_changes.size(); ++t) rel_changes_out[t] = r.rel_changes[t];
    return 0;
}

}

extern "C" int fdx_fit_dev(const void* Y_dev, int32_t y_dtype, int64_t n, int32_t G, int64_t ldy, const double* X, int32_t K,
                           const int32_t* bucket, const double* weight_y, const double* weight_x, const double* coords_dev,
                           int32_t dim, const fdx_fit_params* prm, fdx_graph** graph_inout, double* beta_out_dev,
                           double* prop_out_dev, double* objectives_out, double* rel_changes_out, fdx_fit_info* info,
                           void* stream) {
    auto carry = adopt_carry(prm);
    FDX_REQUIRE(Y_dev != nullptr, "fdx_fit_dev: null array");
    YSource ys;
    ys.dense = Y_dev;
    ys.dtype = y_dtype;
    ys.ldy = ldy;
    return fit_impl(ys, n, G, X, K, bucket, weight_y, weight_x, coords_dev, dim, prm, std::move(carry), graph_inout, beta_out_dev,
                    prop_out_dev, objectives_out, rel_changes_out, info, stream);
}

static int csr_view_ok(const fdx_csr_view* Y, const char* who) {
    FDX_REQUIRE(Y != nullptr, std::string(who) + ": null matrix");
    FDX_REQUIRE(Y->n >= 0 && Y->nnz >= 0 && Y->G > 0, std::string(who) + ": bad CSR shape");
    FDX_REQUIRE(Y->indptr != nullptr && (Y->nnz == 0 || (Y->indices && Y->data)), std::string(who) + ": null CSR array");
    FDX_REQUIRE(Y->dtype == FDX_F32 || Y->dtype == FDX_F64, std::string(who) + ": dtype must be FDX_F32 or FDX_F64");
    return 0;
}

extern "C" int fdx_csr_check_dev(const fdx_csr_view* Y, void* stream) {
    FDX_TRY(csr_view_ok(Y, "fdx_csr_check_dev"));
    hipStream_t st = (hipStream_t)stream;
    PoolStream pool_stream(st);
    DevBuf flag;
    FDX_TRY(flag.alloc(sizeof(int)));
    FDX_TRY(launch_csr_check((const long long*)Y->indptr, Y->indices, Y->n, Y->nnz, Y->G, Y->sorted_rows, flag.as<int>(), st));
    int bad = 0;
    FDX_HIP(hipMemcpyAsync(&bad, flag.p, sizeof(int), hipMemcpyDeviceToHost, st));
    FDX_HIP(hipStreamSynchronize(st));
    FDX_REQUIRE((bad & 1) == 0, "CSR matrix is malformed (indptr not monotone from 0 to nnz, or a column index outside [0, G))");
    FDX_REQUIRE((bad & 2) == 0, "CSR matrix claims sorted_rows but a row's column indices are not ascending");
    return 0;
}

extern "C" int fdx_csr_gene_moments_dev(const fdx_csr_view* Y, double* mean_out_host, double* var_out_host,
                                        double* colsum_out_host, void* stream) {
    FDX_TRY(csr_view_ok(Y, "fdx_csr_gene_moments_dev"));
    FDX_REQUIRE(Y->n > 0, "fdx_csr_gene_moments_dev: empty matrix");
    hipStream_t st = (hipStream_t)stream;
    PoolStream pool_stream(st);
    const size_t G = (size_t)Y->G;
    DevBuf scale, part, out;
    const int ns = colsum_out_host ? 3 : 2;
    FDX_TRY(scale.alloc((size_t)Y->n * sizeof(double)));
    FDX_TRY(part.alloc((size_t)csr_moment_stripes(Y->n) * ns * G * sizeof(double)));
    FDX_TRY(out.alloc(3 * G * sizeof(double)));
    double* o = out.as<double>();
    FDX_TRY(launch_csr_moments((const long long*)Y->indptr, Y->indices, Y->data, Y->dtype, Y->n, Y->nnz, Y->G, scale.as<double>(),
                               part.as<double>(), o, o + G, colsum_out_host ? o + 2 * G : nullptr, Y->sorted_rows != 0, st));
    if (mean_out_host) FDX_TRY(copy_d2h(mean_out_host, o, G * sizeof(double), st));
    if (var_out_host) FDX_TRY(copy_d2h(var_out_host, o + G, G * sizeof(double), st));
    if (colsum_out_host) FDX_TRY(copy_d2h(colsum_out_host, o + 2 * G, G * sizeof(double), st));
    FDX_HIP(hipStreamSynchronize(st));
    return 0;
}

extern "C" int fdx_fit_csr_dev(const fdx_csr_view* Y, const int32_t* gene_idx, int32_t G, const double* X, int32_t K,
                               const int32_t* bucket, const double* weight_y, const double* weight_x,
                               const double* coords_dev, int32_t dim, const fdx_fit_params* prm, fdx_graph** graph_inout,
                               double* beta_out_dev, double* prop_out_dev, double* objectives_out, double* rel_changes_out,
                               fdx_fit_info* info, void* stream) {
    auto carry = adopt_carry(prm);
    FDX_TRY(csr_view_ok(Y, "fdx_fit_csr_dev"));
    FDX_REQUIRE(gene_idx != nullptr || G == Y->G, "fdx_fit_csr_dev: gene_idx may be NULL only when G equals the matrix width");
    FDX_REQUIRE(prm != nullptr, "fdx_fit_csr_dev: null argument");
    FDX_REQUIRE(prm->mode_y == FDX_PRE_RAW || prm->mode_y == FDX_PRE_LOG_CPM_SPARSE,
                "fdx_fit_csr_dev: mode_y must be FDX_PRE_RAW or FDX_PRE_LOG_CPM_SPARSE");
    YSource ys;
    ys.csr = Y;
    ys.gene_idx = gene_idx;
    return fit_impl(ys, Y->n, G, X, K, bucket, weight_y, weight_x, coords_dev, dim, prm, std::move(carry), graph_inout,
                    beta_out_dev, prop_out_dev, objectives_out, rel_changes_out, info, stream);
}
```

flashdeconv_amd/csrc/gram_kernels.cpp:

```cpp
#include <algorithm>
#include <cstdlib>

#include "fdx_internal.h"
#include "fdx_kernels.h"

namespace fdx {

typedef double double4_t __attribute__((ext_vector_type(4)));

__device__ __forceinline__ void load4_guarded(const double* row, int c0, int d, bool row_ok, double (&v)[4]) {
#pragma unroll
    for (int s = 0; s < 4; ++s) v[s] = (row_ok && (c0 + s) < d) ? row[c0 + s] : 0.0;
}

template <bool ALIGNED>
__global__ __launch_bounds__(256) void xyt_kernel(const double* __restrict__ Xs, const double* __restrict__ Ys,
                                                  long long ldy, int n, int d, int K, double* __restrict__ Hout,
                                                  long long ldh, double* __restrict__ sumsq_partials) {
    const int lane = threadIdx.x & 63;
    const int wave = (int)((blockIdx.x * (long long)blockDim.x + threadIdx.x) >> 6);
    const int s0 = wave * 16;
    if (s0 >= n) return;
    const int r = lane & 15, q = lane >> 4;
    const int spot = s0 + r;
    const bool spot_ok = spot < n;
    const double* yrow = Ys + (size_t)(spot_ok ? spot : (n - 1)) * ldy;
    double sq = 0.0;
    const int n_tt = (K + 15) / 16;
    for (int tg = 0; tg < n_tt; tg += 4) {
        double4_t acc[4];
#pragma unroll
        for (int t = 0; t < 4; ++t) acc[t] = double4_t{0.0, 0.0, 0.0, 0.0};
        for (int d0 = 0; d0 < d; d0 += 16) {
            const int c0 = d0 + 4 * q;
            double bv[4];
            if (ALIGNED) {
                const double4_t t4 = *reinterpret_cast<const double4_t*>(yrow + c0);
                bv[0] = t4.x; bv[1] = t4.y; bv[2] = t4.z; bv[3] = t4.w;
                if (!spot_ok) { bv[0] = bv[1] = bv[2] = bv[3] = 0.0; }
            } else {
                load4_guarded(yrow, c0, d, spot_ok, bv);
            }
            if (tg == 0) sq += bv[0] * bv[0] + bv[1] * bv[1] + bv[2] * bv[2] + bv[3] * bv[3];
#pragma unroll
            for (int t = 0; t < 4; ++t) {
                const int type = (tg + t) * 16 + r;
                if ((tg + t) < n_tt) {
                    double av[4];
                    const bool type_ok = type < K;
                    const double* xrow = Xs + (size_t)(type_ok ? type : 0) * d;
                    if (ALIGNED) {
                        const double4_t t4 = *reinterpret_cast<const double4_t*>(xrow + c0);
                        av[0] = t4.x; av[1] = t4.y; av[2] = t4.z; av[3] = t4.w;
                        if (!type_ok) { av[0] = av[1] = av[2] = av[3] = 0.0; }
                    } else {
                        load4_guarded(xrow, c0, d, type_ok, av);
                    }
#pragma unroll
                    for (int s = 0; s < 4; ++s)
                        acc[t] = __builtin_amdgcn_mfma_f64_16x16x4f64(av[s], bv[s], acc[t], 0, 0, 0);
                }
            }
        }
#pragma unroll
        for (int t = 0; t < 4; ++t) {
            if ((tg + t) < n_tt) {
#pragma unroll
                for (int rr = 0; rr < 4; ++rr) {
                    const int type = (tg + t) * 16 + q + 4 * rr;
                    if (type < K && spot_ok) Hout[(size_t)type * ldh + spot] = acc[t][rr];
                }
            }
        }
    }
    if (sumsq_partials) {
#pragma unroll
        for (int off = 32; off > 0; off >>= 1) sq += __shfl_xor(sq, off, 64);
        if (lane == 0) sumsq_partials[wave] = sq;
    }
}

template <int NB, int T>
__global__ __launch_bounds__(512) void xyt_split_kernel(const double* __restrict__ Xs, const double* __restrict__ Ys,
                                                        long long ldy, int n, int d, int K, double* __restrict__ Hout,
                                                        long long ldh) {
    constexpr int NBUF = (T <= 2) ? 2 : 1;
    __shared__ double red[NBUF][8][T * 4 * 64];
    const int tid = threadIdx.x, lane = tid & 63;
    const int wave = __builtin_amdgcn_readfirstlane(tid >> 6);
    const int r = lane & 15, q = lane >> 4;
    double a[NB][T][4];
#pragma unroll
    for (int b = 0; b < NB; ++b) {
        const int c0 = (wave * NB + b) * 16 + 4 * q;
#pragma unroll
        for (int t = 0; t < T; ++t) {
            const int type = t * 16 + r;
            const bool ok = type < K && c0 < d;
            const double4_t v = ok ? *reinterpret_cast<const double4_t*>(Xs + (size_t)type * d + c0) : double4_t{0.0, 0.0, 0.0, 0.0};
            a[b][t][0] = v.x; a[b][t][1] = v.y; a[b][t][2] = v.z; a[b][t][3] = v.w;
        }
    }
    const int n_tiles = (n + 15) / 16;
    int buf = 0;
    for (int tile = blockIdx.x; tile < n_tiles; tile += gridDim.x, buf = (NBUF == 2) ? (buf ^ 1) : 0) {
        const int s0 = tile * 16;
        const int spot = s0 + r;
        const bool spot_ok = spot < n;
        const double* yrow = Ys + (size_t)(spot_ok ? spot : (n - 1)) * ldy;
        double4_t acc[T];
#pragma unroll
        for (int t = 0; t < T; ++t) acc[t] = double4_t{0.0, 0.0, 0.0, 0.0};
        double4_t bv[NB];
#pragma unroll
        for (int b = 0; b < NB; ++b) {
            const int c0 = (wave * NB + b) * 16 + 4 * q;
            bv[b] = (c0 < d) ? *reinterpret_cast<const double4_t*>(yrow + c0) : double4_t{0.0, 0.0, 0.0, 0.0};
        }
#pragma unroll
        for (int b = 0; b < NB; ++b) {
            double x[4] = {bv[b].x, bv[b].y, bv[b].z, bv[b].w};
            if (!spot_ok) { x[0] = x[1] = x[2] = x[3] = 0.0; }
#pragma unroll
            for (int t = 0; t < T; ++t)
#pragma unroll
                for (int s = 0; s < 4; ++s) acc[t] = __builtin_amdgcn_mfma_f64_16x16x4f64(a[b][t][s], x[s], acc[t], 0, 0, 0);
        }
#pragma unroll
        for (int t = 0; t < T; ++t)
#pragma unroll
            for (int rr = 0; rr < 4; ++rr) red[buf][wave][(t * 4 + rr) * 64 + lane] = acc[t][rr];
        __syncthreads();
        for (int o = tid; o < T * 4 * 64; o += 512) {
            double sum = 0.0;
#pragma unroll
            for (int v = 0; v < 8; ++v) sum += red[buf][v][o];
            const int l = o & 63, tr = o >> 6;
            const int type = (tr >> 2) * 16 + (l >> 4) + 4 * (tr & 3);
            const int sp = s0 + (l & 15);
            if (type < K && sp < n) Hout[(size_t)type * ldh + sp] = sum;
        }
        if (NBUF == 1) __syncthreads();
    }
}

__global__ __launch_bounds__(1024) void sum_partials_kernel(const double* __restrict__ in, long long count,
                                                            double* __restrict__ out, int n_out, long long stride) {
    __shared__ double sh[1024];
    for (int o = 0; o < n_out; ++o) {
        double acc = 0.0;
        for (long long i = threadIdx.x; i < count; i += 1024) acc += in[i * stride + o];
        sh[threadIdx.x] = acc;
        __syncthreads();
        for (int s = 512; s > 0; s >>= 1) {
            if ((int)threadIdx.x < s) sh[threadIdx.x] += sh[threadIdx.x + s];
            __syncthreads();
        }
        if (threadIdx.x == 0) out[o] = sh[0];
        __syncthreads();
    }
}

__global__ __launch_bounds__(256) void sum_ranges_kernel(const double* __restrict__ in, long long count, int n_out,
                                                         long long stride, long long per_block, double* __restrict__ mid) {
    __shared__ double sh[256];
    const long long i0 = (long long)blockIdx.x * per_block, i1 = min(count, i0 + per_block);
    for (int o = 0; o < n_out; ++o) {
        double acc = 0.0;
        for (long long i = i0 + threadIdx.x; i < i1; i += 256) acc += in[i * stride + o];
        sh[threadIdx.x] = acc;
        __syncthreads();
        for (int s = 128; s > 0; s >>= 1) {
            if ((int)threadIdx.x < s) sh[threadIdx.x] += sh[threadIdx.x + s];
            __syncthreads();
        }
        if (threadIdx.x == 0) mid[(size_t)blockIdx.x * n_out + o] = sh[0];
        __syncthreads();
    }
}

int launch_sum_partials(const double* in, long long count, double* out, int n_out, long long stride, hipStream_t st) {
    if (count > 65536) {
        static thread_local DevBuf mid;
        const int nb = 512;
        const long long per_block = (count + nb - 1) / nb;
        if (mid.bytes < (size_t)nb * n_out * sizeof(double)) FDX_TRY(mid.alloc((size_t)nb * n_out * sizeof(double)));
        hipLaunchKernelGGL(sum_ranges_kernel, dim3(nb), dim3(256), 0, st, in, count, n_out, stride, per_block, mid.as<double>());
        FDX_CHECK_LAUNCH();
        hipLaunchKernelGGL(sum_partials_kernel, dim3(1), dim3(1024), 0, st, mid.as<double>(), (long long)nb, out, n_out, (long long)n_out);
        FDX_CHECK_LAUNCH();
        return 0;
    }
    hipLaunchKernelGGL(sum_partials_kernel, dim3(1), dim3(1024), 0, st, in, count, out, n_out, stride);
    FDX_CHECK_LAUNCH();
    return 0;
}

long long xyt_partials_count(long long n) { return (n + 15) / 16; }

int launch_xyt(const double* Xs, const double* Ys, long long ldy, long long n, int d, int K, double* Hout,
               long long ldh, double* sumsq_partials, hipStream_t st) {
    if (n <= 0 || K <= 0) return 0;
    if (n > 0x7fffff00LL) return fail(FDX_ERR_UNSUPPORTED, "launch_xyt: n too large");
    const long long waves = (n + 15) / 16;
    const int blocks = (int)((waves + 3) / 4);
    {
        const bool ok = !sumsq_partials && (d % 16 == 0) && d <= 1024 && K <= 64 && (ldy % 4 == 0) &&
                        ((reinterpret_cast<uintptr_t>(Xs) & 31) == 0) && ((reinterpret_cast<uintptr_t>(Ys) & 31) == 0);
        if (ok) {
            const int nb = (d + 127) / 128;
            const int T = (K + 15) / 16;
            const int grid = (int)std::min<long long>(waves, 256LL * 2);
#define FDX_XYT_SPLIT(NB_, T_, XS_, H_, K_) hipLaunchKernelGGL((xyt_split_kernel<NB_, T_>), dim3(grid), dim3(512), 0, st, XS_, Ys, ldy, (int)n, d, K_, H_, ldh)
            if (T <= 2) {
                if (nb <= 1) { if (T == 1) FDX_XYT_SPLIT(1, 1, Xs, Hout, K); else FDX_XYT_SPLIT(1, 2, Xs, Hout, K); }
                else if (nb <= 2) { if (T == 1) FDX_XYT_SPLIT(2, 1, Xs, Hout, K); else FDX_XYT_SPLIT(2, 2, Xs, Hout, K); }
                else if (nb <= 4) { if (T == 1) FDX_XYT_SPLIT(4, 1, Xs, Hout, K); else FDX_XYT_SPLIT(4, 2, Xs, Hout, K); }
                else { if (T == 1) FDX_XYT_SPLIT(8, 1, Xs, Hout, K); else FDX_XYT_SPLIT(8, 2, Xs, Hout, K); }
            } else if (nb <= 4) {
                if (nb <= 1) FDX_XYT_SPLIT(1, 4, Xs, Hout, K);
                else if (nb <= 2) FDX_XYT_SPLIT(2, 4, Xs, Hout, K);
                else FDX_XYT_SPLIT(4, 4, Xs, Hout, K);
            } else {
                const int K2 = K - 32;
                FDX_XYT_SPLIT(8, 2, Xs, Hout, 32);
                FDX_CHECK_LAUNCH();
                if (K2 <= 16) FDX_XYT_SPLIT(8, 1, Xs + (size_t)32 * d, Hout + (size_t)32 * ldh, K2);
                else FDX_XYT_SPLIT(8, 2, Xs + (size_t)32 * d, Hout + (size_t)32 * ldh, K2);
            }
#undef FDX_XYT_SPLIT
            FDX_CHECK_LAUNCH();
            return 0;
        }
    }
    const bool aligned = (d % 16 == 0) && (ldy % 4 == 0) && ((reinterpret_cast<uintptr_t>(Xs) & 31) == 0) &&
                         ((reinterpret_cast<uintptr_t>(Ys) & 31) == 0);
    if (aligned)
        hipLaunchKernelGGL(xyt_kernel<true>, dim3(blocks), dim3(256), 0, st, Xs, Ys, ldy, (int)n, d, K, Hout, ldh, sumsq_partials);
    else
        hipLaunchKernelGGL(xyt_kernel<false>, dim3(blocks), dim3(256), 0, st, Xs, Ys, ldy, (int)n, d, K, Hout, ldh, sumsq_partials);
    FDX_CHECK_LAUNCH();
    return 0;
}

}
```

flashdeconv_amd/csrc/solver.cpp:

```cpp
#include "fdx_env.h"
#include "solver.h"

#include <algorithm>
#include <cmath>
#include <cstdlib>
#include <vector>

namespace fdx {

__global__ void fill_beta_kernel(double* b, long long ld, long long n_fill, int K, double value, int K_planes) {
    const long long i = blockIdx.x * (long long)blockDim.x + threadIdx.x;
    if (i >= ld) return;
    const double v = (i < n_fill) ? value : 0.0;
    for (int k = 0; k < K; ++k) b[(size_t)k * ld + i] = v;
    for (int k = K; k < K_planes; ++k) b[(size_t)k * ld + i] = 0.0;
}

__global__ void pad_square_kernel(const double* __restrict__ A, int K, double* __restrict__ B, int KP) {
    const int e = blockIdx.x * blockDim.x + threadIdx.x;
    if (e >= KP * KP) return;
    const int i = e / KP, j = e - i * KP;
    B[e] = (i < K && j < K) ? A[i * K + j] : 0.0;
}

__global__ void zero_pad_kernel(double* b, long long ld, long long n_used, int K) {
    const long long i = n_used + blockIdx.x * (long long)blockDim.x + threadIdx.x;
    if (i >= ld) return;
    for (int k = 0; k < K; ++k) b[(size_t)k * ld + i] = 0.0;
}

int solver_zero_pad(double* b, long long ld, long long n_used, int K, hipStream_t st) {
    if (ld <= n_used || K <= 0) return 0;
    hipLaunchKernelGGL(zero_pad_kernel, dim3(ceil_div(ld - n_used, 256)), dim3(256), 0, st, b, ld, n_used, K);
    FDX_CHECK_LAUNCH();
    return 0;
}

int solver_init_beta(double* beta, long long ld, long long n_fill, int K, hipStream_t st, int K_planes) {
    if (ld <= 0 || K <= 0) return 0;
    hipLaunchKernelGGL(fill_beta_kernel, dim3(ceil_div(ld, 256)), dim3(256), 0, st, beta, ld, n_fill, K, 1.0 / (double)K, K_planes);
    FDX_CHECK_LAUNCH();
    return 0;
}

int solver_pad_square(const double* A, int K, double* B, int KP, hipStream_t st) {
    hipLaunchKernelGGL(pad_square_kernel, dim3(ceil_div((long long)KP * KP, 256)), dim3(256), 0, st, A, K, B, KP);
    FDX_CHECK_LAUNCH();
    return 0;
}

BcdSweepArgs sweep_args_for_graph(const fdx_graph& g, bool honour_no_tiled) {
    BcdSweepArgs a{};
    a.ell = g.ell.as<int>(); a.slice_off = g.slice_off.as<int>(); a.deg = g.deg.as<int>();
    a.n = (int)g.n; a.n_slices = g.n_slices;
    if (g.tiled && !(honour_no_tiled && fdx::env("FDX_NO_TILED"))) {
        a.tiled = 1; a.ell_local = g.ell_local.as<unsigned short>(); a.tile_halo = g.tile_halo.as<int>();
        a.tile_hcnt = g.tile_hcnt.as<int>(); a.n_tiles = g.n_tiles; a.halo_max = g.halo_max;
    }
    return a;
}

int sweep_scratch_prepare(const double* XtX, int K, int n_slices, DevBuf* scratch, size_t* scratch_ld, hipStream_t st) {
    *scratch_ld = 0;
    if (sweep_uses_lds(K)) {
        FDX_TRY(scratch->alloc(sweep_lds_pad_doubles(K) * sizeof(double)));
        FDX_TRY(sweep_lds_prepare(XtX, K, scratch->as<double>(), st));
    } else if (!sweep_instantiated(K)) {
        *scratch_ld = (size_t)n_slices * 64;
        FDX_TRY(scratch->alloc(*scratch_ld * 2 * K * sizeof(double)));
    }
    return 0;
}

double xtx_diag_mean(const double* XtX_host, int K) {
    double diag_mean = 0.0;
    for (int k = 0; k < K; ++k) diag_mean += XtX_host[(size_t)k * K + k];
    return diag_mean / (double)K;
}

double auto_lambda(double diag_mean, double mean_degree) { return 0.005 * diag_mean / std::max(mean_degree, 1.0); }

int solver_objective_partials(const fdx_graph& g, const double* beta, long long ld, const double* H, long long ldh,
                              const double* XtX, int K, double* scratch_partials, double* out4_dev, hipStream_t st) {
    int nblk = objective_partials_count(g.n_slices);
    int rc_t = 1;
    BcdSweepArgs a = sweep_args_for_graph(g, true);
    if (a.tiled) {
        a.H = H; a.XtX = XtX; a.beta_in = beta; a.ldh = (int)ldh; a.ld = (int)ld; a.K = K;
        a.skip_quad = (K > FDX_MAX_K_FAST && sweep_instantiated(K)) ? 1 : 0;
        rc_t = launch_bcd_objective_tiled(a, scratch_partials, st);
        if (rc_t < 0) return rc_t;
        if (rc_t == 0) {
            nblk = g.n_tiles;
            if (a.skip_quad) FDX_TRY(launch_beta_quad(beta, ld, g.n, K, XtX, scratch_partials, g.n_tiles, st));
        }
    }
    if (rc_t != 0) {
        const int skip_quad = K > FDX_MAX_K_FAST ? 1 : 0;
        FDX_TRY(launch_objective_partials(beta, ld, H, ldh, XtX, g.ell.as<int>(), g.slice_off.as<int>(), g.deg.as<int>(),
                                          (int)g.n, g.n_slices, K, scratch_partials, st, skip_quad));
        if (skip_quad) FDX_TRY(launch_beta_quad(beta, ld, g.n, K, XtX, scratch_partials, nblk, st));
    }
    return launch_sum_partials(scratch_partials, nblk, out4_dev, 4, 4, st);
}

int solver_objective(const fdx_graph& g, const double* beta, long long ld, const double* H, long long ldh,
                     const double* XtX, int K, double YtY, double lambda, double rho_eff, double* scratch_partials,
                     double* scratch_out4, double* obj_host, hipStream_t st) {
    FDX_TRY(solver_objective_partials(g, beta, ld, H, ldh, XtX, K, scratch_partials, scratch_out4, st));
    double r[4];
    FDX_HIP(hipMemcpyAsync(r, scratch_out4, sizeof(r), hipMemcpyDeviceToHost, st));
    FDX_HIP(hipStreamSynchronize(st));
    *obj_host = objective_from_sums(r, YtY, lambda, rho_eff);
    return 0;
}

int SweepStats::init(int max_iter, hipStream_t st) {
    const size_t iters = (size_t)std::max(max_iter, 1);
    const size_t stats_bytes = iters * 128 * sizeof(unsigned long long);
    FDX_TRY(block.alloc(stats_bytes + iters * sizeof(double)));
    FDX_HIP(hipMemsetAsync(block.p, 0, block.bytes, st));
    stats = block.as<unsigned long long>();
    rel_change = reinterpret_cast<double*>(static_cast<char*>(block.p) + stats_bytes);
    return 0;
}

int solver_loop(const SweepStats& s, int max_iter, double tol, int first_chunk, int n_ahead,
                const std::function<int(int, bool)>& queue_iteration, LoopResult* res, hipStream_t st) {
    Event ev0[2] = {Event(true), Event(true)}, ev1[2] = {Event(true), Event(true)}, evCopy;
    const size_t rc_count = (size_t)std::max(max_iter, 1);
    double* rc_host = (double*)pinned_scratch(2, rc_count * sizeof(double));
    if (!rc_host) return fail(FDX_ERR_HIP, "solver: pinned host buffer");
    for (size_t j = 0; j < rc_count; ++j) rc_host[j] = 0.0;
    *res = LoopResult();
    res->rel_changes = rc_host;
    int done = 0;
    int chunk = first_chunk > 0 ? first_chunk : 4;
    int queued_ahead = 0;
    int ci = 0;
    while (done < max_iter && !res->converged) {
        const int end = std::min(max_iter, done + chunk);
        const int pair = ci & 1;
        if (queued_ahead == 0) FDX_TRY(ev0[pair].record(st));
        for (int it = done + queued_ahead; it < end; ++it) FDX_TRY(queue_iteration(it, it + 1 == end));
        FDX_TRY(launch_bcd_fold_last(s.stats, s.rel_change, end - 1, st));
        FDX_TRY(ev1[pair].record(st));
        FDX_HIP(hipMemcpyAsync(rc_host + done, s.rel_change + done, (size_t)(end - done) * sizeof(double), hipMemcpyDeviceToHost, st));
        FDX_TRY(evCopy.record(st));
        int ahead = 0;
        if (end < max_iter && n_ahead > 0) {
            ahead = std::min(n_ahead, max_iter - end);
            FDX_TRY(ev0[pair ^ 1].record(st));
            for (int it = end; it < end + ahead; ++it) FDX_TRY(queue_iteration(it, false));
        }
        FDX_TRY(evCopy.sync());
        float ms_chunk = 0.f;
        FDX_HIP(hipEventElapsedTime(&ms_chunk, ev0[pair].e, ev1[pair].e));
        res->sweep_ms += ms_chunk;
        for (int it = done; it < end; ++it) {
            res->n_iter = it + 1;
            if (rc_host[it] < tol) { res->converged = true; break; }
        }
        done = end;
        queued_ahead = ahead;
        chunk = std::max(std::min(ci == 0 ? chunk : chunk * 2, 32), ahead);
        ++ci;
    }
    return 0;
}

int solver_run(const SolveProblem& p, SolveResult* res, hipStream_t st) {
    const fdx_graph& g = *p.graph;
    const int K = p.K;
    *res = SolveResult();
    if (g.n == 0 || K == 0) {
        res->converged = 1;
        return 0;
    }
    FDX_REQUIRE(p.ld >= g.n_total + 1, "solver: ld must cover owned + halo spots + the zero pad row");
    FDX_REQUIRE(p.max_iter >= 0, "solver: max_iter must be >= 0");

    const int max_iter = p.max_iter;
    SweepStats stats;
    DevBuf obj_partials, obj_out, generic_scratch;
    FDX_TRY(stats.init(max_iter, st));
    FDX_TRY(obj_partials.alloc((size_t)objective_partials_count(g.n_slices) * 4 * sizeof(double)));
    FDX_TRY(obj_out.alloc(4 * sizeof(double)));
    size_t scratch_ld = 0;
    FDX_TRY(sweep_scratch_prepare(p.XtX, K, g.n_slices, &generic_scratch, &scratch_ld, st));
    const int K_real = p.K_real > 0 ? p.K_real : K;
    if (p.init_beta) FDX_TRY(solver_init_beta(p.beta[0], p.ld, g.n_total, K_real, st, K));
    if (p.init_beta) FDX_TRY(solver_zero_pad(p.beta[1], p.ld, g.n_total, K, st));

    BcdSweepArgs a = sweep_args_for_graph(g, true);
    a.H = p.H; a.XtX = p.XtX; a.stats = stats.stats; a.rel_change = stats.rel_change;
    a.lambda = p.lambda; a.rho = p.rho_eff; a.tol = p.tol; a.ldh = (int)p.ldh; a.ld = (int)p.ld; a.K = K;

    double init_uniform = 0.0;
    if (!p.init_beta && p.beta0_virtual) {
        BcdSweepArgs probe = a;
        probe.beta_in = p.beta[0];
        probe.beta_out = p.beta[1];
        if (max_iter > 0 && K_real == K && K <= FDX_MAX_K_FAST && g.n_total == g.n && bcd_sweep_uses_tiles(probe) && !fdx::env("FDX_NO_INIT_SWEEP"))
            init_uniform = 1.0 / (double)K;
        else
            FDX_TRY(solver_init_beta(p.beta[0], p.ld, g.n_total, K_real, st, K));
    }

    std::vector<std::pair<int, double>> trace;
    auto queue_sweep = [&](int it, bool) -> int {
        a.it = it;
        a.beta_in = p.beta[it & 1];
        a.beta_out = p.beta[(it + 1) & 1];
        a.init_uniform = it == 0 ? init_uniform : 0.0;
        FDX_TRY(launch_bcd_sweep(a, generic_scratch.as<double>(), scratch_ld, st));
        if (p.verbose && (it % 10 == 0 || it == max_iter - 1)) {
            double obj = 0.0;
            FDX_TRY(solver_objective(g, a.beta_out, p.ld, p.H, p.ldh, p.XtX, K, p.YtY, p.lambda, p.rho_eff,
                                     obj_partials.as<double>(), obj_out.as<double>(), &obj, st));
            trace.emplace_back(it, obj);
        }
        return 0;
    };
    LoopResult loop;
    const int n_ahead = p.verbose ? 0 : 2;
    FDX_TRY(solver_loop(stats, max_iter, p.tol, p.first_chunk, n_ahead, queue_sweep, &loop, st));

    const int n_iter = loop.n_iter;
    res->sweep_ms = loop.sweep_ms;
    res->n_iterations = n_iter;
    res->converged = loop.converged ? 1 : 0;
    res->final_change = n_iter > 0 ? loop.rel_changes[n_iter - 1] : 0.0;
    res->result_buffer = n_iter & 1;
    res->rel_changes.assign(loop.rel_changes, loop.rel_changes + n_iter);
    for (auto& t : trace)
        if (t.first < n_iter) { res->objective_iters.push_back(t.first); res->objectives.push_back(t.second); }
    if (p.compute_objective)
        FDX_TRY(solver_objective(g, p.beta[res->result_buffer], p.ld, p.H, p.ldh, p.XtX, K, p.YtY, p.lambda, p.rho_eff,
                                 obj_partials.as<double>(), obj_out.as<double>(), &res->final_objective, st));
    return 0;
}

}
```

flashdeconv_amd/csrc/solver.h:

```cpp
#pragma once
#include <functional>
#include <vector>

#include "fdx_graph.h"
#include "fdx_internal.h"
#include "fdx_kernels.h"

namespace fdx {

struct SolveProblem {
    const fdx_graph* graph = nullptr;
    const double* H = nullptr;
    long long ldh = 0;
    const double* XtX = nullptr;
    double* beta[2] = {nullptr, nullptr};
    long long ld = 0;
    int K = 0;
    int K_real = 0;
    double YtY = 0.0;
    double lambda = 0.0;
    double rho_eff = 0.0;
    int max_iter = 100;
    double tol = 1e-4;
    int verbose = 0;
    int init_beta = 1;
    int beta0_virtual = 0;
    int compute_objective = 1;
    int first_chunk = 4;
};

struct SolveResult {
    int result_buffer = 0;
    int n_iterations = 0;
    int converged = 0;
    double final_change = 0.0;
    double final_objective = 0.0;
    double sweep_ms = 0.0;
    std::vector<int> objective_iters;
    std::vector<double> objectives;
    std::vector<double> rel_changes;
};

int solver_init_beta(double* beta, long long ld, long long n_fill, int K, hipStream_t st, int K_planes = 0);
int solver_pad_square(const double* A, int K, double* B, int KP, hipStream_t st);
int solver_zero_pad(double* b, long long ld, long long n_used, int K, hipStream_t st);
int solver_objective_partials(const fdx_graph& g, const double* beta, long long ld, const double* H, long long ldh,
                              const double* XtX, int K, double* scratch_partials, double* out4_dev, hipStream_t st);
int solver_objective(const fdx_graph& g, const double* beta, long long ld, const double* H, long long ldh,
                     const double* XtX, int K, double YtY, double lambda, double rho_eff, double* scratch_partials,
                     double* scratch_out4, double* obj_host, hipStream_t st);
int solver_run(const SolveProblem& p, SolveResult* res, hipStream_t st);

BcdSweepArgs sweep_args_for_graph(const fdx_graph& g, bool honour_no_tiled);
int sweep_scratch_prepare(const double* XtX, int K, int n_slices, DevBuf* scratch, size_t* scratch_ld, hipStream_t st);
double xtx_diag_mean(const double* XtX_host, int K);
double auto_lambda(double diag_mean, double mean_degree);
inline double objective_from_sums(const double* r4, double YtY, double lambda, double rho_eff) {
    return 0.5 * (YtY - 2.0 * r4[0] + r4[1]) + 0.5 * lambda * r4[2] + rho_eff * r4[3];
}

struct SweepStats {
    DevBuf block;
    unsigned long long* stats = nullptr;
    double* rel_change = nullptr;
    int init(int max_iter, hipStream_t st);
};
struct LoopResult {
    int n_iter = 0;
    bool converged = false;
    const double* rel_changes = nullptr;
    double sweep_ms = 0.0;
};
int solver_loop(const SweepStats& s, int max_iter, double tol, int first_chunk, int n_ahead,
                const std::function<int(int, bool)>& queue_iteration, LoopResult* res, hipStream_t st);

}
```

include/fdx.h:

```cpp
#ifndef FDX_H
#define FDX_H

#include <stddef.h>
#include <stdint.h>

#ifdef __cplusplus
extern "C" {
#endif

#define FDX_OK 0
#define FDX_ERR_INVALID (-1)
#define FDX_ERR_HIP (-2)
#define FDX_ERR_UNSUPPORTED (-3)
#define FDX_ERR_INTERNAL (-4)

#define FDX_F32 0
#define FDX_F64 1

#define FDX_PRE_RAW 0
#define FDX_PRE_LOG_CPM 1
#define FDX_PRE_LOG_CPM_SPARSE 2
#define FDX_PRE_F64_MATH 0x100

int fdx_version(void);
int fdx_env_reload(void);
const char* fdx_env_switch(int32_t i, const char** what_out);
const char* fdx_last_error(void);
int fdx_device_count(int* count);
int fdx_set_device(int device);
int fdx_device_name(char* buf, int buflen);

int fdx_malloc(void** dev_ptr, size_t bytes);
int fdx_free(void* dev_ptr);
int fdx_trim(void);
int fdx_x_cache_stats(int64_t out[4]);
int fdx_memcpy_h2d(void* dev_dst, const void* host_src, size_t bytes, void* stream);
int fdx_memcpy_d2h(void* host_dst, const void* dev_src, size_t bytes, void* stream);
int fdx_memset(void* dev_dst, int value, size_t bytes, void* stream);
int fdx_stream_sync(void* stream);

#define FDX_SRC_F32 0
#define FDX_SRC_F64 1
#define FDX_SRC_I8 2
#define FDX_SRC_U8 3
#define FDX_SRC_I16 4
#define FDX_SRC_U16 5
#define FDX_SRC_I32 6
#define FDX_SRC_U32 7
#define FDX_SRC_I64 8
#define FDX_SRC_U64 9
int fdx_upload_convert_dev(void* dst_dev, int32_t dst_dtype, const void* src_host, int32_t src_code, int64_t count,
                           double* max_abs_out, void* stream);
int fdx_download_dev(void* dst_host, const void* src_dev, size_t bytes, void* stream);
int fdx_pinned_copy_rate(size_t bytes, int32_t to_device, double* gbps_out);

int fdx_sketch(const void* Y, int32_t dtype, int64_t n, int32_t G, const int64_t* col_ptr, const int32_t* gene_idx,
               const double* weight, int32_t d, int32_t mode, double* Ys_out);
int fdx_tile_schedule(const int32_t* gene_bucket, const double* gene_w, int32_t G, int32_t d, int32_t NW, int32_t JW,
                      int32_t GB, int32_t* dims_out, int32_t* slot_bucket_out, uint8_t* len_out, int32_t* ent_base_out,
                      double* w_out, uint16_t* off_out, int64_t cap_entries);
int fdx_sketch_path(int32_t y_dtype, const void* Y_dev, int64_t ldy, int32_t G, int32_t d, int32_t K, int32_t mode_y,
                    const int32_t* bucket, const double* weight_y, int32_t* path_out, int32_t* dims_out);
int fdx_log1p_f32(const float* y, float scale, int64_t n, float* out);
int fdx_column_sums(const void* Y, int32_t dtype, int64_t n, int32_t G, double* sums_out);

int fdx_column_sums_dev(const void* Y_dev, int32_t dtype, int64_t n, int32_t G, int64_t ldy, double* sums_out_host,
                        void* stream);

int fdx_gene_moments_dev(const void* Y_dev, int32_t dtype, int64_t n, int32_t G, int64_t ldy, double* mean_out_host,
                         double* var_out_host, void* stream);
int fdx_gather_columns_dev(const void* Y_dev, int32_t dtype, int64_t n, int32_t G, int64_t ldy, const int32_t* idx_host,
                           int32_t G_sel, void* out_dev, void* stream);

int fdx_leverage_scores(const double* X, int32_t K, int32_t G, double regularization, double* lev_out);
typedef struct fdx_leverage_job fdx_leverage_job;
int fdx_leverage_begin(const double* X, int32_t K, int32_t G, double regularization, fdx_leverage_job** job);
int fdx_leverage_end(fdx_leverage_job* job, double* lev_out);
int fdx_leverage_end_keep(fdx_leverage_job* job, double* lev_out, double** x_dev_out);
int fdx_leverage_begin_opt(const double* X, int32_t K, int32_t G, double regularization, int32_t queue_async, fdx_leverage_job** job);

typedef struct fdx_graph fdx_graph;

int fdx_graph_from_csr(const int64_t* indptr, const int64_t* indices, int64_t n, fdx_graph** out);
int fdx_graph_build_knn(const double* coords, int64_t n, int32_t dim, int32_t k, fdx_graph** out);
int fdx_graph_build_radius(const double* coords, int64_t n, int32_t dim, double radius, fdx_graph** out);
int fdx_nearest_distance(const double* coords, int64_t n, int32_t dim, double* dist_out);
int fdx_graph_export_csr(const fdx_graph* g, int64_t* indptr, int32_t* indices);
int fdx_graph_destroy(fdx_graph* g);
int fdx_graph_info(const fdx_graph* g, int64_t* n, int64_t* nnz, int32_t* max_deg);
int fdx_graph_knn_ties(const fdx_graph* g, int64_t* ties);
int fdx_hvg_from_moments(const double* mean, const double* var, int32_t G, const double* sorted_pos, int32_t n_pos, int32_t n_top,
                         double min_mean, double max_mean, double min_disp, int64_t* idx_out, int32_t* n_out, int32_t* ambiguous);
int fdx_ckdtree_prebuild(const double* coords_host, const double* coords_dev, int64_t n, int32_t dim);
int fdx_kdtree_set_threads(int32_t threads);
int fdx_kdtree_tune(int32_t what, int64_t points);
int fdx_ckdtree_indices_dev(const double* coords_dev, int64_t n, int32_t dim, int64_t* indices_out, int32_t* info_out, void* stream);
int fdx_ckdtree_knn(const double* coords, int64_t n, int32_t dim, int32_t kk, int64_t* idx_out, int64_t* tree_indices_out);
int fdx_ckdtree_knn_rows(const double* coords, int64_t n, int32_t dim, int32_t kk, const int64_t* rows, int64_t n_rows,
                         int64_t* idx_out);

typedef struct fdx_solve_info {
    int32_t converged;
    int32_t n_iterations;
    double final_objective;
    double final_change;
    int32_t n_objectives;
    int32_t reserved;
    double sweep_ms;
    double total_ms;
} fdx_solve_info;

int fdx_bcd_solve(const fdx_graph* g, const double* Y_sketch, const double* X_sketch, int64_t n, int32_t d,
                  int32_t K, double lambda, double rho, int32_t max_iter, double tol, int32_t verbose,
                  double* beta_out, double* objectives_out, double* rel_changes_out, fdx_solve_info* info);

int fdx_gram_xty(const double* X_sketch, const double* Y_sketch, int64_t n, int32_t d, int32_t K, double* XtX_out,
                 double* H_out);
int fdx_objective(const fdx_graph* g, const double* beta, const double* H, const double* XtX, int64_t n, int32_t K,
                  double YtY, double lambda, double rho, double* obj_out);

#define FDX_GRAPH_KNN 0
#define FDX_GRAPH_RADIUS 1
#define FDX_GRAPH_GIVEN 2

typedef struct fdx_fit_params {
    int32_t sketch_dim;
    int32_t mode_y;
    int32_t mode_x;
    int32_t graph_method;
    int32_t k_neighbors;
    int32_t lambda_auto;
    int32_t max_iter;
    int32_t verbose;
    double radius;
    double lambda_spatial;
    double rho_sparsity;
    double tol;
    int32_t stop_on_ties;
    int32_t reserved;
    void* carry;
    double* spot_diag_out_dev;
} fdx_fit_params;
#define FDX_FIT_TIES 3

typedef struct fdx_fit_info {
    fdx_solve_info solve;
    double lambda_used;
    double rho_effective;
    double YtY;
    int64_t nnz;
    double graph_ms, sketch_ms, gram_ms, solve_ms, finish_ms, total_ms;
    double prologue_ms, span_ms;
    int64_t knn_ties;
    int32_t status;
    int32_t reserved;
    void* carry;
    double diag_ms;
} fdx_fit_info;
int fdx_fit_carry_free(void* carry);

int fdx_fit_dev(const void* Y_dev, int32_t y_dtype, int64_t n, int32_t G, int64_t ldy, const double* X, int32_t K,
                const int32_t* bucket, const double* weight_y, const double* weight_x, const double* coords_dev,
                int32_t dim, const fdx_fit_params* params, fdx_graph** graph_inout, double* beta_out_dev,
                double* prop_out_dev, double* objectives_out, double* rel_changes_out, fdx_fit_info* info, void* stream);

typedef struct fdx_csr_view {
    const int64_t* indptr;
    const int32_t* indices;
    const void* data;
    int32_t dtype;
    int64_t n;
    int64_t nnz;
    int32_t G;
    int32_t sorted_rows;
} fdx_csr_view;

int fdx_csr_check_dev(const fdx_csr_view* Y, void* stream);
int fdx_csr_gene_moments_dev(const fdx_csr_view* Y, double* mean_out_host, double* var_out_host, double* colsum_out_host,
                             void* stream);
int fdx_fit_csr_dev(const fdx_csr_view* Y, const int32_t* gene_idx, int32_t G, const double* X, int32_t K,
                    const int32_t* bucket, const double* weight_y, const double* weight_x, const double* coords_dev,
                    int32_t dim, const fdx_fit_params* params, fdx_graph** graph_inout, double* beta_out_dev,
                    double* prop_out_dev, double* objectives_out, double* rel_changes_out, fdx_fit_info* info, void* stream);

int fdx_type_sums_dev(const void* Y_dev, int32_t dtype, int64_t n, int32_t G, int64_t ldy, const int32_t* rows_dev,
                      const int32_t* type_off_dev, int32_t K, int32_t mean, double* X_out_dev, void* stream);
int fdx_type_sums_csr_dev(const fdx_csr_view* Y, const int32_t* rows_dev, const int32_t* type_off_dev, int32_t K, int32_t mean,
                          double* X_out_dev, void* stream);

#define FDX_MX_SSE 0
#define FDX_MX_SAE 1
#define FDX_MX_SUM_P 2
#define FDX_MX_SUM_T 3
#define FDX_MX_MIN_P 4
#define FDX_MX_MAX_P 5
#define FDX_MX_MIN_T 6
#define FDX_MX_MAX_T 7
#define FDX_MX_NAN_P 8
#define FDX_MX_NAN_T 9
#define FDX_MX_N_RARE 10
#define FDX_MX_TP 11
#define FDX_MX_FP 12
#define FDX_MX_FN 13
#define FDX_MX_JSD_SUM 14
#define FDX_MX_C_PT 15
#define FDX_MX_C_PP 16
#define FDX_MX_C_TT 17
#define FDX_METRICS_FIELDS 18
#define FDX_SPEARMAN_OVERALL 1
#define FDX_SPEARMAN_PER_TYPE 2

int fdx_metrics_moments_dev(const void* pred_dev, const void* true_dev, int32_t dtype, int64_t n, int32_t K, int64_t ld_pred,
                            int64_t ld_true, double threshold, double epsilon, double* jsd_out_dev, double* stats_host,
                            int64_t* rare_host, void* stream);
int fdx_metrics_spearman_dev(const void* pred_dev, const void* true_dev, int32_t dtype, int64_t n, int32_t K, int64_t ld_pred,
                             int64_t ld_true, int32_t flags, double* rho_host, void* stream);
int fdx_metrics_evaluate_dev(const void* pred_dev, const void* true_dev, int32_t dtype, int64_t n, int32_t K, int64_t ld_pred,
                             int64_t ld_true, double threshold, double epsilon, int32_t flags, double* jsd_out_dev,
                             double* stats_host, int64_t* rare_host, double* rho_host, void* stream);


int fdx_graph_build_dev(const double* coords_dev, int64_t n, int32_t dim, int32_t method, int32_t k, double radius,
                        void* stream, fdx_graph** out);
int fdx_side_stream(void** stream_out);
int fdx_stream_wait_stream(void* waiter, void* producer);
int fdx_graph_build_radius_rows_dev(const double* coords_dev, int64_t n, int32_t dim, double radius, int64_t lo, int64_t hi,
                                    void* stream, fdx_graph** out);
typedef struct fdx_graph_plan fdx_graph_plan;
int fdx_graph_knn_lists_dev(const double* coords_dev, int64_t n, int32_t dim, int32_t k, int64_t lo, int64_t hi,
                            int32_t* nbr_dev, int32_t* cnt_dev, void* stream, fdx_graph_plan** plan);
int fdx_graph_from_knn_lists_dev(fdx_graph_plan* plan, const int32_t* nbr_dev, const int32_t* cnt_dev, int64_t lo, int64_t hi,
                                 void* stream, fdx_graph** out);
int fdx_graph_knn_lists_band_dev(const double* coords_dev, int64_t n, int32_t dim, int32_t k, int64_t lo, int64_t hi,
                                 int32_t* nbr_dev, int32_t* cnt_dev, void* stream, fdx_graph_plan** plan);
int fdx_graph_knn_far(const fdx_graph* g, int32_t* far);
int fdx_graph_plan_order_dev(const fdx_graph_plan* plan, int32_t* perm_out_dev, int32_t* rank_out_dev, void* stream);
int fdx_graph_plan_lists_replaced(fdx_graph_plan* plan);
int fdx_graph_plan_set_lists_dev(fdx_graph_plan* plan, const int64_t* ids_host, const int64_t* rows_host, int64_t n_rows,
                                 int32_t* nbr_dev, int32_t* cnt_dev, void* stream);
int fdx_graph_plan_set_ckdtree_lists_dev(fdx_graph_plan* plan, const double* coords_host, const double* coords_dev, int64_t n,
                                         int32_t dim, const int64_t* rows_host, int64_t n_rows, int32_t* nbr_dev, int32_t* cnt_dev,
                                         void* stream);
int fdx_graph_perm_dev(const fdx_graph* g, int32_t* perm_out_dev, void* stream);
int fdx_graph_localize(const fdx_graph* full, int32_t n_ranks, const int64_t* bounds, int32_t my_rank, void* stream,
                       fdx_graph** local);
int fdx_graph_shard_knn_dev(const double* coords_dev, int64_t n, int32_t dim, int32_t k, int32_t n_ranks, const int64_t* bounds,
                            int32_t my_rank, void* stream, fdx_graph** local);
int fdx_graph_shard_status(const fdx_graph* local, int64_t* own_nnz, int64_t* knn_ties, int32_t* far, int32_t* overflow);
int fdx_graph_row_indices(const fdx_graph* g, int64_t row, int32_t* idx_out, int32_t cap, int32_t* deg_out);
int fdx_graph_tile_info(const fdx_graph* g, int32_t* n_tiles, int32_t* halo_max, int32_t* tiled);
int fdx_graph_halo_info(const fdx_graph* local, int64_t* n_halo, int32_t* send_counts, int32_t* recv_counts);
int fdx_graph_send_indices_dev(const fdx_graph* local, int32_t* idx_out_dev, void* stream);

int fdx_prepare_dev(const void* Y_dev, int32_t y_dtype, int64_t n, int32_t G, int64_t ldy, const int32_t* row_map_dev,
                    const double* X, int32_t K, const int32_t* bucket, const double* weight_y, const double* weight_x,
                    int32_t d, int32_t mode_y, int32_t mode_x, double* H_out_dev, int64_t ldh, double* XtX_out_dev,
                    double* XtX_out_host, double* YtY_partial_out, void* stream);
int fdx_prepare_csr_dev(const fdx_csr_view* Y, const int32_t* gene_idx, int32_t G, const double* X, int32_t K,
                        const int32_t* bucket, const double* weight_y, const double* weight_x, int32_t d, int32_t mode_y,
                        int32_t mode_x, double* H_out_dev, int64_t ldh, double* XtX_out_dev, double* XtX_out_host,
                        double* YtY_partial_out, void* stream);
int fdx_init_beta_dev(double* beta_dev, int64_t ld, int64_t n_fill, int32_t K, void* stream);
int fdx_bcd_sweep_dev(const fdx_graph* g, const double* H_dev, int64_t ldh, const double* XtX_dev, const double* beta_in,
                      double* beta_out, int64_t ld, int32_t K, double lambda, double rho_eff, double tol, int32_t it,
                      void* stats_dev, double* rel_change_dev, void* stream);
int fdx_bcd_fold_dev(void* stats_dev, double* rel_change_dev, int32_t it, void* stream);
int fdx_objective_partials_dev(const fdx_graph* g, const double* beta_dev, int64_t ld, const double* H_dev, int64_t ldh,
                               const double* XtX_dev, int32_t K, double* out4_host, void* stream);
int fdx_spot_diagnostics_dev(const fdx_graph* g, const double* beta_dev, int64_t ld, const double* H_dev, int64_t ldh,
                             const double* XtX_dev, int32_t ldg, int32_t K, const double* row_sq_dev, double* out_dev,
                             void* stream);
int fdx_spatial_autocorr_dev(const fdx_graph* g, const double* V_dev, int64_t ldv, int32_t K, double* mean_out, double* m2_out,
                             double* C_out, int64_t* counts_out, double* neighbor_mean_dev, void* stream);
int fdx_spatial_perm_dev(const fdx_graph* g, const double* V_dev, int64_t ldv, int32_t K, uint64_t seed, int64_t first_perm,
                         int64_t n_perm, int32_t max_batch, double* null_dev, double* mean_out, double* m2_out, double* C_out,
                         int64_t* counts_out, double* m4_out, int64_t* count_ge_out, int64_t* count_le_out, double* sum_d_out,
                         double* sumsq_d_out, int32_t* batch_out, void* stream);
int fdx_permutation_indices_dev(uint64_t seed, int64_t r, int64_t n, int32_t* out_dev, void* stream);
int fdx_kmeans_assign_dev(const double* F_dev, int64_t ldf, int64_t n, int32_t D, const double* centres_dev, int32_t C,
                          int32_t* labels_dev, double* min_d2_dev, int64_t* changed_out, double* inertia_out, void* stream);
int fdx_label_sums_dev(const double* F_dev, int64_t ldf, int64_t n, int32_t D, const int32_t* labels_dev, int32_t C,
                       double* sums_out, int64_t* counts_out, void* stream);
int fdx_kmeans_seed_dist_dev(const double* F_dev, int64_t ldf, int64_t n, int32_t D, const double* centre_dev, double* d2_dev,
                             double* block_sums_out, int64_t* block_rows_out, int32_t* n_blocks_out, void* stream);
int fdx_kmeans_dev(const double* F_dev, int64_t ldf, int64_t n, int32_t D, int32_t C, int32_t max_iter, double* centres_dev,
                   int32_t* labels_dev, int64_t* counts_out, double* inertia_out, int32_t* n_iter_out, int32_t* converged_out,
                   void* stream);
int fdx_normalize_dev(const double* beta_dev, int64_t ld, int64_t n, int32_t K, double* beta_out_dev, double* prop_out_dev,
                      void* stream);
int fdx_export_dev(const fdx_graph* g, const double* beta_dev, int64_t ld, int32_t K, double* beta_out_dev, double* prop_out_dev,
                   void* stream);

typedef struct fdx_comm fdx_comm;
typedef struct fdx_local_world fdx_local_world;
int fdx_comm_unique_id(void* id_out_128);
int fdx_comm_init(const void* id_128, int32_t rank, int32_t world, fdx_comm** out);
int fdx_local_world_create(int32_t world, fdx_local_world** out);
int fdx_comm_init_loopback(int32_t rank, int32_t world, fdx_comm** out);
int fdx_local_world_destroy(fdx_local_world* w);
int fdx_comm_init_local(fdx_local_world* w, int32_t rank, fdx_comm** out);
int fdx_comm_destroy(fdx_comm* comm);
int fdx_comm_info(const fdx_comm* comm, int32_t* rank, int32_t* world);
int fdx_comm_rccl_count(const fdx_comm* comm, int32_t* count);
int fdx_comm_allreduce_sum_dev(fdx_comm* comm, double* buf_dev, int32_t count, void* stream);
typedef struct {
    int32_t sketch_dim, mode_y, mode_x, lambda_auto, max_iter, stop_on_ties;
    double lambda_spatial, rho_sparsity, tol;
    int64_t n_total_spots, nnz_total;
    const double* X_dev;
} fdx_shard_fit_params;
typedef struct {
    int32_t status, reserved;
    int64_t nnz_total, knn_ties_total, own_nnz, n_halo;
    double lambda_used, rho_effective, YtY;
    fdx_solve_info solve;
} fdx_shard_fit_info;
#define FDX_SHARD_FAR 1
#define FDX_SHARD_OVERFLOW 2
#define FDX_SHARD_TIES 3
int fdx_shard_fit_dev(fdx_comm* comm, const fdx_graph* local, const void* Y_dev, int32_t y_dtype, int64_t n_own, int32_t G,
                      int64_t ldy, const double* X, int32_t K, const int32_t* bucket, const double* weight_y,
                      const double* weight_x, const fdx_shard_fit_params* prm, double* beta_out_dev, double* prop_out_dev,
                      double* rel_changes_out, fdx_shard_fit_info* info, void* stream);
int fdx_sharded_solve_dev(fdx_comm* comm, const fdx_graph* local, const double* H_dev, int64_t ldh, const double* XtX_dev,
                          int32_t K, double lambda, double rho_eff, double tol, int32_t max_iter, double* beta0_dev,
                          double* beta1_dev, int64_t ld, fdx_solve_info* info, double* rel_changes_out,
                          int32_t* result_buffer, void* stream);
int32_t fdx_solver_padded_k(int32_t K);
int fdx_sharded_solve_padded_dev(fdx_comm* comm, const fdx_graph* local, const double* H_dev, int64_t ldh, const double* XtX_dev,
                                 int32_t K, int32_t K_real, double lambda, double rho_eff, double tol, int32_t max_iter,
                                 double* beta0_dev, double* beta1_dev, int64_t ld, fdx_solve_info* info, double* rel_changes_out,
                                 int32_t* result_buffer, void* stream);

#ifdef __cplusplus
}
#endif
#endif
```

Before: 237.5 million.

## Fuse final objective pass with beta/proportion export and gate it on device

Adds a fused fit tail: the last objective sweep kernel also normalizes and writes beta and proportions (through LDS staging and the permutation), replacing a separate export kernel. A gated variant is queued by the host right after the iteration chunk and reads the convergence trace on the device to pick the right beta buffer, or exits early if not converged. This is meant to save a kernel launch, a re-read of beta, and a host round trip at the end of the solve. The cost is larger LDS for the objective kernel and speculative tail launches that may be wasted.

After: 235.2 million. -1.0%, worse.

```diff
diff --git a/flashdeconv_amd/_lib.py b/flashdeconv_amd/_lib.py
--- a/flashdeconv_amd/_lib.py
+++ b/flashdeconv_amd/_lib.py
@@ -77,8 +77,11 @@
         ("solve", SolveInfo), ("lambda_used", c_double), ("rho_effective", c_double), ("YtY", c_double), ("nnz", c_i64),
         ("graph_ms", c_double), ("sketch_ms", c_double), ("gram_ms", c_double), ("solve_ms", c_double),
         ("finish_ms", c_double), ("total_ms", c_double), ("prologue_ms", c_double), ("span_ms", c_double),
-        ("knn_ties", c_i64), ("status", c_i32), ("reserved", c_i32), ("carry", c_void_p), ("diag_ms", c_double),
+        ("knn_ties", c_i64), ("status", c_i32), ("tail_route", c_i32), ("carry", c_void_p), ("diag_ms", c_double),
     ]
+
+
+TAIL_ROUTES = ("two_kernels", "fused", "gated")
 
 
 FIT_TIES = 3
@@ -146,6 +149,8 @@
                                c_void_p]),
     "fdx_normalize_dev": (c_int, [c_void_p, c_i64, c_i64, c_i32, c_void_p, c_void_p, c_void_p]),
     "fdx_export_dev": (c_int, [c_void_p, c_void_p, c_i64, c_i32, c_void_p, c_void_p, c_void_p]),
+    "fdx_fit_tail_dev": (c_int, [c_void_p, c_void_p, c_void_p, c_i64, c_void_p, c_i64, c_void_p, c_i32, c_void_p, c_i32, c_i32, c_double,
+                                 c_void_p, c_void_p, c_void_p, p_double, p_i32, c_void_p]),
     "fdx_gene_moments_dev": (c_int, [c_void_p, c_i32, c_i64, c_i32, c_i64, p_double, p_double, c_void_p]),
     "fdx_gather_columns_dev": (c_int, [c_void_p, c_i32, c_i64, c_i32, c_i64, p_i32, c_i32, c_void_p, c_void_p]),
     "fdx_version": (c_int, []),
diff --git a/flashdeconv_amd/core/deconv.py b/flashdeconv_amd/core/deconv.py
--- a/flashdeconv_amd/core/deconv.py
+++ b/flashdeconv_amd/core/deconv.py
@@ -460,6 +460,7 @@
                 print(f"Converged at iteration {n_it - 1}")
         self.info_ = info.solve.as_dict()
         self.info_["objectives"] = objectives if self.verbose else []
+        self.info_["tail_route"] = _lib.TAIL_ROUTES[int(info.tail_route)]
         resolved = self.spatial_method == "knn" and (self.knn_ties == "ckdtree" or ties_resolved_here)
         self.info_["knn_ties"] = (n_ties if resolved else int(info.knn_ties)) if self.spatial_method == "knn" else 0
         if self.info_["knn_ties"] and not resolved:
diff --git a/flashdeconv_amd/csrc/bcd_sweep_inst.cpp b/flashdeconv_amd/csrc/bcd_sweep_inst.cpp
--- a/flashdeconv_amd/csrc/bcd_sweep_inst.cpp
+++ b/flashdeconv_amd/csrc/bcd_sweep_inst.cpp
@@ -2,6 +2,7 @@
 #include <cstdlib>
 #include "bcd_device.h"
 #include "fdx_graph.h"
+#include "tail_gate.h"
 
 #ifndef FDX_PART
 #error "compile with -DFDX_PART=<n> -DFDX_K_LO=<lo> -DFDX_K_HI=<hi>"
@@ -112,6 +113,8 @@
 #ifndef FDX_SWEEP_WPE
 #define FDX_SWEEP_WPE 1
 #endif
+constexpr size_t tail_export_lds(int K, int R) { return (size_t)R * (K | 1) * sizeof(double) + 256 * (sizeof(double) + sizeof(int)); }
+constexpr int tail_export_rows(int K) { return tail_export_lds(K, 256) <= 80 * 1024 ? 256 : 128; }
 template <int K, int KC, bool OBJ, bool QUAD = true, bool INIT = false>
 __global__ __launch_bounds__(256, ((OBJ && K > 40 && K <= 64) || (K > 64 && K <= 96)) ? 2 : (OBJ ? 1 : FDX_SWEEP_WPE)) void bcd_sweep_tiled_kernel(
     const double* __restrict__ H, const double* __restrict__ XtX, const double* __restrict__ beta_in,
@@ -120,10 +123,18 @@
     unsigned long long* __restrict__ stats, double* __restrict__ rel_change, const double lambda, const double rho,
     const double tol, const int ldh, const int ld_, const int n, const int S, const int it,
     const int* __restrict__ tile_list, const double init_v, const int* __restrict__ send_head, const int4* __restrict__ send_ent,
-    double* __restrict__ send_buf) {
+    double* __restrict__ send_buf, double* __restrict__ prop_out, const int* __restrict__ perm, const double* __restrict__ beta_alt,
+    const double* __restrict__ gate_trace, const int gate_end, const int gate_max_iter, int* __restrict__ gate_n_iter) {
     extern __shared__ __attribute__((aligned(16))) double lds[];
     const int tid = threadIdx.x;
     const int lane = tid & 63;
+    const double* bsrc = beta_in;
+    if (OBJ && gate_trace != nullptr) {
+        const int n_it = tail_gate_n_iter(gate_trace, gate_end, gate_max_iter, tol);
+        if (n_it < 0) return;
+        if (n_it & 1) bsrc = beta_alt;
+        if (blockIdx.x == 0 && tid == 0 && gate_n_iter != nullptr) *gate_n_iter = n_it;
+    }
     const int tile = tile_list ? tile_list[xcd_remap(blockIdx.x, gridDim.x)] : xcd_remap(blockIdx.x, gridDim.x);
     const bool real = (tile * 256 + tid) < n;
     const int i = min(tile * 256 + tid, n - 1);
@@ -147,7 +158,7 @@
 #define PLANE_AT(base, off) (*(const double __attribute__((address_space(1)))*)(plane_base(base) + lane_off(off)))
     double b[K];
 #pragma unroll
-    for (int k = 0; k < K; ++k) b[k] = INIT ? init_v : PLANE_AT(beta_in + k * ld, ioff);
+    for (int k = 0; k < K; ++k) b[k] = INIT ? init_v : PLANE_AT(bsrc + k * ld, ioff);
     const unsigned short* ell = ell_local + (size_t)w0 * 64 + (i & 63);
     const double lam_deg = lambda * (double)dg;
     const double lam_eff = (dg > 0) ? lambda : 0.0;
@@ -164,7 +175,7 @@
     double hv[KC], hreg[KC];
 #pragma unroll
     for (int q = 0; q < KC; ++q) {
-        hv[q] = INIT ? init_v : PLANE_AT(beta_in + q * ld, hoff);
+        hv[q] = INIT ? init_v : PLANE_AT(bsrc + q * ld, hoff);
         hreg[q] = __builtin_nontemporal_load(&PLANE_AT(H + q * (size_t)ldh, ioff));
     }
 
@@ -184,7 +195,7 @@
             const int j = halo[h];
 #pragma unroll
             for (int q = 0; q < KC; ++q)
-                if (kc + q < K) lds[q * S + 256 + h] = INIT ? init_v : beta_in[(kc + q) * ld + j];
+                if (kc + q < K) lds[q * S + 256 + h] = INIT ? init_v : bsrc[(kc + q) * ld + j];
         }
         if (tid < KC) lds[tid * S + 256 + Ht] = 0.0;
         __syncthreads();
@@ -250,7 +261,7 @@
                 for (int t = 2 * q; t < 2 * q + 2; ++t) {
                     const int j = t < KC ? t : t - KC;
                     if (kc + KC + j < K) {
-                        if (t < KC) { if (!INIT) hv[j] = PLANE_AT(beta_in + (kc + KC + j) * ld, hoff); }
+                        if (t < KC) { if (!INIT) hv[j] = PLANE_AT(bsrc + (kc + KC + j) * ld, hoff); }
                         else hreg[j] = __builtin_nontemporal_load(&PLANE_AT(H + (kc + KC + j) * (size_t)ldh, ioff));
                     }
                 }
@@ -271,6 +282,42 @@
         if (lane == 0) { lds[(tid >> 6) * 4 + 0] = o_cross; lds[(tid >> 6) * 4 + 1] = o_quad; lds[(tid >> 6) * 4 + 2] = o_spat; lds[(tid >> 6) * 4 + 3] = o_l1; }
         __syncthreads();
         if (tid < 4) rel_change[(size_t)tile * 4 + tid] = ((lds[tid] + lds[4 + tid]) + lds[8 + tid]) + lds[12 + tid];
+        if constexpr (K <= FDX_MAX_K_FAST) if (beta_out != nullptr || prop_out != nullptr) {
+            constexpr int Ks = K | 1, R = tail_export_rows(K);
+            double* const den_s = lds + R * Ks;
+            int* const row_s = (int*)(den_s + 256);
+            double s = 0.0;
+    #pragma unroll
+            for (int k = 0; k < K; ++k) s += b[k];
+            const double den = (s < 1e-10) ? 1e-10 : s;
+            const double inv_K = 1.0 / (double)K;
+            __syncthreads();
+            den_s[tid] = (s == 0.0) ? -1.0 : den;
+            row_s[tid] = real ? (perm ? perm[i] : i) : -1;
+            constexpr int ds = 256 / K, dk = 256 - ds * K;
+    #pragma unroll
+            for (int r0 = 0; r0 < 256; r0 += R) {
+                if (r0 > 0) __syncthreads();
+                if (tid >= r0 && tid < r0 + R) {
+    #pragma unroll
+                    for (int k = 0; k < K; ++k) lds[(tid - r0) * Ks + k] = b[k];
+                }
+                __syncthreads();
+                int sp = tid / K, k = tid - sp * K;
+                for (int f = tid; f < R * K; f += 256) {
+                    const int row = row_s[r0 + sp];
+                    if (row >= 0) {
+                        const double v = lds[sp * Ks + k];
+                        const double dd = den_s[r0 + sp];
+                        if (beta_out) __builtin_nontemporal_store(v, beta_out + (size_t)row * K + k);
+                        if (prop_out) __builtin_nontemporal_store((dd < 0.0) ? inv_K : v / dd, prop_out + (size_t)row * K + k);
+                    }
+                    sp += ds;
+                    k += dk;
+                    if (k >= K) { k -= K; ++sp; }
+                }
+            }
+        }
         return;
     }
     if (!OBJ && send_head != nullptr) {
@@ -304,28 +351,33 @@
                 if constexpr (K > 64) {
                     hipLaunchKernelGGL((bcd_sweep_tiled_kernel<K, KC, true, false>), dim3(a.n_tiles), dim3(256), lds, st, a.H, a.XtX,
                                        a.beta_in, a.beta_out, a.ell_local, a.slice_off, a.deg, a.tile_halo, a.tile_hcnt,
-                                       a.stats, a.rel_change, a.lambda, a.rho, a.tol, a.ldh, a.ld, a.n, S, a.it, nullptr, 0.0, a.send_head, a.send_ent, a.send_buf);
+                                       a.stats, a.rel_change, a.lambda, a.rho, a.tol, a.ldh, a.ld, a.n, S, a.it, nullptr, 0.0, a.send_head, a.send_ent, a.send_buf, nullptr, nullptr, nullptr, nullptr, 0, 0, nullptr);
                 } else {
-                    hipLaunchKernelGGL((bcd_sweep_tiled_kernel<K, KC, true>), dim3(a.n_tiles), dim3(256), lds, st, a.H, a.XtX,
-                                       a.beta_in, a.beta_out, a.ell_local, a.slice_off, a.deg, a.tile_halo, a.tile_hcnt,
-                                       a.stats, a.rel_change, a.lambda, a.rho, a.tol, a.ldh, a.ld, a.n, S, a.it, nullptr, 0.0, a.send_head, a.send_ent, a.send_buf);
+                    const bool exports = a.export_beta != nullptr || a.export_prop != nullptr;
+                    const size_t lds_tail = exports ? std::max(lds, tail_export_lds(K, tail_export_rows(K))) : lds;
+                    if (lds_tail > 64 * 1024)
+                        (void)hipFuncSetAttribute((const void*)bcd_sweep_tiled_kernel<K, KC, true>, hipFuncAttributeMaxDynamicSharedMemorySize, (int)lds_tail);
+                    hipLaunchKernelGGL((bcd_sweep_tiled_kernel<K, KC, true>), dim3(a.n_tiles), dim3(256), lds_tail, st, a.H, a.XtX,
+                                       a.beta_in, a.export_beta, a.ell_local, a.slice_off, a.deg, a.tile_halo, a.tile_hcnt,
+                                       a.stats, a.rel_change, a.lambda, a.rho, a.tol, a.ldh, a.ld, a.n, S, a.it, nullptr, 0.0, a.send_head, a.send_ent, a.send_buf,
+                                       a.export_prop, a.export_perm, a.beta_alt, a.gate_trace, a.gate_end, a.gate_max_iter, a.gate_n_iter);
                 }
             }
             else if (a.tile_list) {
                 if (a.n_list > 0)
                     hipLaunchKernelGGL((bcd_sweep_tiled_kernel<K, KC, false>), dim3(a.n_list), dim3(256), lds, st, a.H, a.XtX,
                                        a.beta_in, a.beta_out, a.ell_local, a.slice_off, a.deg, a.tile_halo, a.tile_hcnt,
-                                       a.stats, a.rel_change, a.lambda, a.rho, a.tol, a.ldh, a.ld, a.n, S, a.it, a.tile_list, 0.0, a.send_head, a.send_ent, a.send_buf);
+                                       a.stats, a.rel_change, a.lambda, a.rho, a.tol, a.ldh, a.ld, a.n, S, a.it, a.tile_list, 0.0, a.send_head, a.send_ent, a.send_buf, nullptr, nullptr, nullptr, nullptr, 0, 0, nullptr);
             } else if (a.init_uniform != 0.0) {
                 if constexpr (K <= 64) {
                     hipLaunchKernelGGL((bcd_sweep_tiled_kernel<K, KC, false, true, true>), dim3(a.n_tiles), dim3(256), lds, st, a.H, a.XtX,
                                        a.beta_in, a.beta_out, a.ell_local, a.slice_off, a.deg, a.tile_halo, a.tile_hcnt,
-                                       a.stats, a.rel_change, a.lambda, a.rho, a.tol, a.ldh, a.ld, a.n, S, a.it, nullptr, a.init_uniform, a.send_head, a.send_ent, a.send_buf);
+                                       a.stats, a.rel_change, a.lambda, a.rho, a.tol, a.ldh, a.ld, a.n, S, a.it, nullptr, a.init_uniform, a.send_head, a.send_ent, a.send_buf, nullptr, nullptr, nullptr, nullptr, 0, 0, nullptr);
                 }
             } else {
                 hipLaunchKernelGGL((bcd_sweep_tiled_kernel<K, KC, false>), dim3(a.n_tiles), dim3(256), lds, st, a.H, a.XtX,
                                    a.beta_in, a.beta_out, a.ell_local, a.slice_off, a.deg, a.tile_halo, a.tile_hcnt,
-                                   a.stats, a.rel_change, a.lambda, a.rho, a.tol, a.ldh, a.ld, a.n, S, a.it, nullptr, 0.0, a.send_head, a.send_ent, a.send_buf);
+                                   a.stats, a.rel_change, a.lambda, a.rho, a.tol, a.ldh, a.ld, a.n, S, a.it, nullptr, 0.0, a.send_head, a.send_ent, a.send_buf, nullptr, nullptr, nullptr, nullptr, 0, 0, nullptr);
             }
             return;
         }
diff --git a/flashdeconv_amd/csrc/capi_dev.cpp b/flashdeconv_amd/csrc/capi_dev.cpp
--- a/flashdeconv_amd/csrc/capi_dev.cpp
+++ b/flashdeconv_amd/csrc/capi_dev.cpp
@@ -584,6 +584,37 @@
     return launch_normalize_export(beta_dev, ld, perm, (int)g->n, g->n_slices, K, beta_out_dev, prop_out_dev, (hipStream_t)stream);
 }
 
+int fdx_fit_tail_dev(const fdx_graph* g, const double* beta0_dev, const double* beta1_dev, int64_t ld, const double* H_dev, int64_t ldh,
+                     const double* XtX_dev, int32_t K, const double* trace_dev, int32_t end, int32_t max_iter, double tol,
+                     double* beta_out_dev, double* prop_out_dev, double* partials_dev, double* out4_host, int32_t* n_iter_out,
+                     void* stream) {
+    FDX_TRY(fdx::graph_meta_sync(g));
+    FDX_REQUIRE(g && beta0_dev && H_dev && XtX_dev && out4_host && n_iter_out && K > 0, "fdx_fit_tail_dev: bad arguments");
+    FDX_REQUIRE(trace_dev == nullptr || (beta1_dev != nullptr && end >= 0 && end <= max_iter), "fdx_fit_tail_dev: bad gate");
+    FDX_REQUIRE(ld >= g->n_total + 1 && ldh >= g->n, "fdx_fit_tail_dev: ld must cover the spots and the zero pad row, ldh the spots");
+    FDX_REQUIRE(solver_tail_fused_ok(*g, ld, ldh, K), "fdx_fit_tail_dev: no fused tail for this graph and K (whole tiled graph, K <= 64)");
+    hipStream_t st = (hipStream_t)stream;
+    PoolStream pool_stream(st);
+    DevBuf part, out;
+    if (!partials_dev) FDX_TRY(part.alloc((size_t)g->n_tiles * 4 * sizeof(double)));
+    FDX_TRY(out.alloc(5 * sizeof(double)));
+    int* n_iter_dev = reinterpret_cast<int*>(out.as<double>() + 4);
+    FDX_HIP(hipMemsetAsync(n_iter_dev, 0xff, sizeof(int), st));
+    FitTail t;
+    t.beta_out = beta_out_dev; t.prop_out = prop_out_dev;
+    t.perm = (g->identity_order || !g->perm.p) ? nullptr : g->perm.as<int>();
+    t.gate_trace = trace_dev; t.gate_end = end; t.gate_max_iter = max_iter; t.tol = tol; t.gate_n_iter = n_iter_dev;
+    FDX_TRY(solver_fit_tail(*g, t, beta0_dev, beta1_dev, ld, H_dev, ldh, XtX_dev, K, partials_dev ? partials_dev : part.as<double>(),
+                            out.as<double>(), st));
+    double host[5];
+    FDX_HIP(hipMemcpyAsync(host, out.p, sizeof(host), hipMemcpyDeviceToHost, st));
+    FDX_HIP(hipStreamSynchronize(st));
+    for (int o = 0; o < 4; ++o) out4_host[o] = host[o];
+    std::memcpy(n_iter_out, &host[4], sizeof(int));
+    if (!trace_dev) *n_iter_out = 0;
+    return 0;
+}
+
 int fdx_normalize_dev(const double* beta_dev, int64_t ld, int64_t n, int32_t K, double* beta_out_dev, double* prop_out_dev,
                       void* stream) {
     FDX_REQUIRE(beta_dev && n >= 0 && K > 0, "fdx_normalize_dev: bad arguments");
diff --git a/flashdeconv_amd/csrc/fdx_env.cpp b/flashdeconv_amd/csrc/fdx_env.cpp
--- a/flashdeconv_amd/csrc/fdx_env.cpp
+++ b/flashdeconv_amd/csrc/fdx_env.cpp
@@ -44,6 +44,7 @@
     {"FDX_KDTREE_PAR_DEPTH", "fork depth of the restated cKDTree build"},
     {"FDX_NO_PLAN_CACHE", "sketch plans / tile schedules, leverage scores and the X side recomputed every fit (bench.py: cold_ms)"},
     {"FDX_NO_SIDE_STREAM", "everything on the caller's stream"},
+    {"FDX_NO_FUSED_TAIL", "fit tail as two kernels (export beside the objective pass); 'gate': one launch, but queued by the host"},
     {"FDX_CSR_KEEP_CAP", "entries per wave of the fused CSR sketch's keep buffer (tests: rows that overflow it)"},
 };
 constexpr int kSwitches = sizeof(g_switches) / sizeof(g_switches[0]);
diff --git a/flashdeconv_amd/csrc/fdx_kernels.h b/flashdeconv_amd/csrc/fdx_kernels.h
--- a/flashdeconv_amd/csrc/fdx_kernels.h
+++ b/flashdeconv_amd/csrc/fdx_kernels.h
@@ -40,6 +40,13 @@
     const int* send_head = nullptr;
     const int4* send_ent = nullptr;
     double* send_buf = nullptr;
+    double* export_beta = nullptr;
+    double* export_prop = nullptr;
+    const int* export_perm = nullptr;
+    const double* beta_alt = nullptr;
+    const double* gate_trace = nullptr;
+    int gate_end = 0, gate_max_iter = 0;
+    int* gate_n_iter = nullptr;
     double init_uniform = 0.0;
     unsigned long long* stats;
     double* rel_change;
@@ -96,6 +103,8 @@
                long long ldh, double* sumsq_partials, hipStream_t st);
 long long xyt_partials_count(long long n);
 int launch_sum_partials(const double* in, long long count, double* out, int n_out, long long stride, hipStream_t st);
+int launch_sum_partials_gated(const double* in, long long count, double* out, int n_out, long long stride, const double* gate_trace,
+                              int gate_end, int gate_max_iter, double tol, hipStream_t st);
 
 int objective_partials_count(int n_slices);
 int launch_objective_partials(const double* beta, long long ld, const double* H, long long ldh, const double* XtX,
diff --git a/flashdeconv_amd/csrc/fit.cpp b/flashdeconv_amd/csrc/fit.cpp
--- a/flashdeconv_amd/csrc/fit.cpp
+++ b/flashdeconv_amd/csrc/fit.cpp
@@ -3,6 +3,7 @@
 #include <cstdio>
 #include <cmath>
 #include <cstdlib>
+#include <cstring>
 #include <memory>
 #include <vector>
 
@@ -436,6 +437,9 @@
     p.lambda = lambda; p.rho_eff = prm->rho_sparsity * diag_mean; p.max_iter = prm->max_iter; p.tol = prm->tol;
     p.verbose = prm->verbose;
     p.compute_objective = prm->verbose ? 1 : 0;
+    const char* no_fused_tail = fdx::env("FDX_NO_FUSED_TAIL");
+    p.tail_route = !no_fused_tail ? TAIL_GATED : std::strcmp(no_fused_tail, "gate") == 0 ? TAIL_FUSED : TAIL_TWO_KERNELS;
+    p.tail.beta_out = beta_out_dev; p.tail.prop_out = prop_out_dev; p.tail.perm = row_map;
     SolveResult r;
     if (evInit) {
         p.init_beta = 0;
@@ -444,14 +448,19 @@
     }
     FDX_TRY(solver_run(p, &r, st));
     Event evSolved, evExported;
-    if ((beta_out_dev || prop_out_dev) && !prm->verbose && side) {
+    const bool tail_done = r.tail_route != TAIL_TWO_KERNELS;
+    if (tail_done) {
+        if (evY) FDX_TRY(evY.sync());
+        r.final_objective = objective_from_sums(r.tail_sums, *YtY_h, lambda, p.rho_eff);
+    }
+    if (!tail_done && (beta_out_dev || prop_out_dev) && !prm->verbose && side) {
         FDX_TRY(evSolved.record(st));
         FDX_TRY(evSolved.wait_on(side));
         FDX_TRY(launch_normalize_export(p.beta[r.result_buffer], ld, row_map, (int)n, g->n_slices, K, beta_out_dev,
                                         prop_out_dev, side));
         FDX_TRY(evExported.record(side));
     }
-    if (!prm->verbose) {
+    if (!prm->verbose && !tail_done) {
         DevBuf objp, objo;
         FDX_TRY(objp.alloc((size_t)std::max(objective_partials_count(g->n_slices), g->n_tiles) * 4 * sizeof(double)));
         FDX_TRY(objo.alloc(4 * sizeof(double)));
@@ -462,7 +471,7 @@
     }
     FDX_TRY(t_solved.record(st));
     if (evExported) FDX_TRY(evExported.wait_on(st));
-    else if (beta_out_dev || prop_out_dev)
+    else if (!tail_done && (beta_out_dev || prop_out_dev))
         FDX_TRY(launch_normalize_export(p.beta[r.result_buffer], ld, row_map, (int)n, g->n_slices, K, beta_out_dev,
                                         prop_out_dev, st));
     Event t_diag0(true), t_diag1(true);
@@ -483,6 +492,7 @@
     info->solve.final_change = r.final_change;
     info->solve.n_objectives = (int32_t)r.objectives.size();
     info->solve.sweep_ms = r.sweep_ms;
+    info->tail_route = r.tail_route;
     info->lambda_used = lambda;
     info->rho_effective = p.rho_eff;
     info->YtY = *YtY_h;
diff --git a/flashdeconv_amd/csrc/gram_kernels.cpp b/flashdeconv_amd/csrc/gram_kernels.cpp
--- a/flashdeconv_amd/csrc/gram_kernels.cpp
+++ b/flashdeconv_amd/csrc/gram_kernels.cpp
@@ -3,6 +3,7 @@
 
 #include "fdx_internal.h"
 #include "fdx_kernels.h"
+#include "tail_gate.h"
 
 namespace fdx {
 
@@ -144,9 +145,8 @@
     }
 }
 
-__global__ __launch_bounds__(1024) void sum_partials_kernel(const double* __restrict__ in, long long count,
-                                                            double* __restrict__ out, int n_out, long long stride) {
-    __shared__ double sh[1024];
+__device__ __forceinline__ void sum_partials_body(const double* __restrict__ in, long long count, double* __restrict__ out,
+                                                  int n_out, long long stride, double* sh) {
     for (int o = 0; o < n_out; ++o) {
         double acc = 0.0;
         for (long long i = threadIdx.x; i < count; i += 1024) acc += in[i * stride + o];
@@ -159,6 +159,21 @@
         if (threadIdx.x == 0) out[o] = sh[0];
         __syncthreads();
     }
+}
+
+__global__ __launch_bounds__(1024) void sum_partials_kernel(const double* __restrict__ in, long long count,
+                                                            double* __restrict__ out, int n_out, long long stride) {
+    __shared__ double sh[1024];
+    sum_partials_body(in, count, out, n_out, stride, sh);
+}
+
+__global__ __launch_bounds__(1024) void sum_partials_gated_kernel(const double* __restrict__ in, long long count,
+                                                                  double* __restrict__ out, int n_out, long long stride,
+                                                                  const double* __restrict__ gate_trace, int gate_end,
+                                                                  int gate_max_iter, double tol) {
+    __shared__ double sh[1024];
+    if (tail_gate_n_iter(gate_trace, gate_end, gate_max_iter, tol) < 0) return;
+    sum_partials_body(in, count, out, n_out, stride, sh);
 }
 
 __global__ __launch_bounds__(256) void sum_ranges_kernel(const double* __restrict__ in, long long count, int n_out,
@@ -192,6 +207,15 @@
         return 0;
     }
     hipLaunchKernelGGL(sum_partials_kernel, dim3(1), dim3(1024), 0, st, in, count, out, n_out, stride);
+    FDX_CHECK_LAUNCH();
+    return 0;
+}
+
+int launch_sum_partials_gated(const double* in, long long count, double* out, int n_out, long long stride, const double* gate_trace,
+                              int gate_end, int gate_max_iter, double tol, hipStream_t st) {
+    if (count > 65536) return fail(FDX_ERR_UNSUPPORTED, "gated sum: more rows than one level takes");
+    hipLaunchKernelGGL(sum_partials_gated_kernel, dim3(1), dim3(1024), 0, st, in, count, out, n_out, stride, gate_trace, gate_end,
+                       gate_max_iter, tol);
     FDX_CHECK_LAUNCH();
     return 0;
 }
diff --git a/flashdeconv_amd/csrc/hosttest/tail_gate_asan.cpp b/flashdeconv_amd/csrc/hosttest/tail_gate_asan.cpp
--- /dev/null
+++ b/flashdeconv_amd/csrc/hosttest/tail_gate_asan.cpp
@@ -0,0 +1,85 @@
+#include <cstdio>
+#include <vector>
+
+#include "../tail_gate.h"
+
+namespace {
+
+void plain_loop(const std::vector<double>& rc, int max_iter, double tol, int* n_iter, bool* converged) {
+    *n_iter = 0;
+    *converged = false;
+    for (int it = 0; it < max_iter; ++it) {
+        *n_iter = it + 1;
+        if (rc[it] < tol) { *converged = true; break; }
+    }
+}
+
+std::vector<int> chunk_ends(int max_iter, int first_chunk, int n_ahead) {
+    std::vector<int> ends;
+    int done = 0, chunk = first_chunk, ci = 0;
+    while (done < max_iter) {
+        const int end = done + chunk < max_iter ? done + chunk : max_iter;
+        ends.push_back(end);
+        const int ahead = end < max_iter ? (n_ahead < max_iter - end ? n_ahead : max_iter - end) : 0;
+        done = end;
+        int next = ci == 0 ? chunk : chunk * 2;
+        if (next > 32) next = 32;
+        chunk = next > ahead ? next : ahead;
+        ++ci;
+    }
+    return ends;
+}
+
+int bad = 0;
+#define CHECK(cond, ...) do { if (!(cond)) { std::printf("tail gate: line %d: %s  [", __LINE__, #cond); std::printf(__VA_ARGS__); std::printf("]\n"); ++bad; } } while (0)
+
+void replay(int max_iter, int conv, double tol, int first_chunk, int n_ahead) {
+    std::vector<double> full((size_t)max_iter);
+    for (int it = 0; it < max_iter; ++it) full[it] = (conv >= 0 && it == conv) ? tol * 0.5 : (conv >= 0 && it > conv) ? 0.0 : tol * (2.0 + it);
+    int want_n = 0;
+    bool want_conv = false;
+    plain_loop(full, max_iter, tol, &want_n, &want_conv);
+    const std::vector<int> ends = chunk_ends(max_iter, first_chunk, n_ahead);
+    bool opened = false;
+    for (size_t c = 0; c < ends.size() && !opened; ++c) {
+        const int end = ends[c];
+        std::vector<double> dev(full.begin(), full.begin() + end);
+        const int got = fdx::tail_gate_n_iter(dev.data(), end, max_iter, tol);
+        std::vector<double> padded((size_t)max_iter, 0.0);
+        for (int it = 0; it < end; ++it) padded[it] = full[it];
+        const int got_padded = fdx::tail_gate_n_iter(padded.data(), end, max_iter, tol);
+        CHECK(got == got_padded, "max_iter %d conv %d end %d: %d vs %d", max_iter, conv, end, got, got_padded);
+        const bool should_open = (want_conv && want_n <= end) || (!want_conv && end == max_iter);
+        if (!should_open) {
+            CHECK(got == -1, "max_iter %d conv %d end %d: gate open (%d) before the solve is over", max_iter, conv, end, got);
+        } else {
+            CHECK(got == want_n, "max_iter %d conv %d end %d: n_iter %d, want %d", max_iter, conv, end, got, want_n);
+            CHECK((got & 1) == (want_n & 1), "buffer parity");
+            opened = true;
+        }
+    }
+    CHECK(opened, "max_iter %d conv %d: the gate never opened", max_iter, conv);
+}
+
+}
+
+int main() {
+    const double tols[] = {1e-4, 1e-300, 0.5};
+    for (double tol : tols)
+        for (int first_chunk : {4, 1, 3})
+            for (int n_ahead : {2, 0})
+                for (int max_iter = 1; max_iter <= 80; ++max_iter)
+                    for (int conv = -1; conv < max_iter; ++conv) replay(max_iter, conv, tol, first_chunk, n_ahead);
+    for (int e : {4, 8, 16, 32, 64})
+        for (int conv : {e - 1, e, e + 1}) replay(100, conv, 1e-4, 4, 2);
+    CHECK(fdx::tail_gate_n_iter(nullptr, 0, 0, 1e-4) == 0, "max_iter 0");
+    {
+        const double nan = __builtin_nan("");
+        const double t[3] = {1.0, nan, 1e-9};
+        CHECK(fdx::tail_gate_n_iter(t, 2, 5, 1e-4) == -1, "NaN closed");
+        CHECK(fdx::tail_gate_n_iter(t, 2, 2, 1e-4) == 2, "NaN, end == max_iter");
+        CHECK(fdx::tail_gate_n_iter(t, 3, 5, 1e-4) == 3, "behind a NaN");
+    }
+    std::printf(bad ? "FAILED\n" : "tail gate: ok under the sanitizers\n");
+    return bad ? 1 : 0;
+}
diff --git a/flashdeconv_amd/csrc/solver.cpp b/flashdeconv_amd/csrc/solver.cpp
--- a/flashdeconv_amd/csrc/solver.cpp
+++ b/flashdeconv_amd/csrc/solver.cpp
@@ -1,5 +1,6 @@
 #include "fdx_env.h"
 #include "solver.h"
+#include "tail_gate.h"
 
 #include <algorithm>
 #include <cmath>
@@ -115,25 +116,53 @@
     return 0;
 }
 
+bool solver_tail_fused_ok(const fdx_graph& g, long long ld, long long ldh, int K) {
+    if (K > FDX_MAX_K_FAST || g.n <= 0 || g.n_total != g.n) return false;
+    BcdSweepArgs a = sweep_args_for_graph(g, true);
+    a.K = K; a.ld = (int)ld; a.ldh = (int)ldh;
+    return ld < (1LL << 31) && ldh < (1LL << 31) && bcd_sweep_uses_tiles(a);
+}
+
+int solver_fit_tail(const fdx_graph& g, const FitTail& t, const double* beta0, const double* beta1, long long ld, const double* H,
+                    long long ldh, const double* XtX, int K, double* scratch_partials, double* out4_dev, hipStream_t st) {
+    FDX_REQUIRE(solver_tail_fused_ok(g, ld, ldh, K), "fit tail: no tiled traversal for this graph and K");
+    BcdSweepArgs a = sweep_args_for_graph(g, true);
+    a.H = H; a.XtX = XtX; a.beta_in = beta0; a.ldh = (int)ldh; a.ld = (int)ld; a.K = K;
+    a.export_beta = t.beta_out; a.export_prop = t.prop_out; a.export_perm = t.perm;
+    if (t.gate_trace) {
+        FDX_REQUIRE(beta1 != nullptr && t.gate_end >= 0 && t.gate_end <= t.gate_max_iter, "fit tail: bad gate");
+        a.beta_alt = beta1; a.gate_trace = t.gate_trace; a.gate_end = t.gate_end; a.gate_max_iter = t.gate_max_iter;
+        a.gate_n_iter = t.gate_n_iter; a.tol = t.tol;
+    }
+    const int rc = launch_bcd_objective_tiled(a, scratch_partials, st);
+    if (rc != 0) return rc < 0 ? rc : fail(FDX_ERR_INTERNAL, "fit tail: dispatch failed");
+    if (t.gate_trace)
+        return launch_sum_partials_gated(scratch_partials, g.n_tiles, out4_dev, 4, 4, t.gate_trace, t.gate_end, t.gate_max_iter, t.tol, st);
+    return launch_sum_partials(scratch_partials, g.n_tiles, out4_dev, 4, 4, st);
+}
+
 int SweepStats::init(int max_iter, hipStream_t st) {
     const size_t iters = (size_t)std::max(max_iter, 1);
     const size_t stats_bytes = iters * 128 * sizeof(unsigned long long);
-    FDX_TRY(block.alloc(stats_bytes + iters * sizeof(double)));
+    FDX_TRY(block.alloc(stats_bytes + (iters + 4) * sizeof(double)));
     FDX_HIP(hipMemsetAsync(block.p, 0, block.bytes, st));
     stats = block.as<unsigned long long>();
     rel_change = reinterpret_cast<double*>(static_cast<char*>(block.p) + stats_bytes);
+    tail_sums = rel_change + iters;
     return 0;
 }
 
 int solver_loop(const SweepStats& s, int max_iter, double tol, int first_chunk, int n_ahead,
-                const std::function<int(int, bool)>& queue_iteration, LoopResult* res, hipStream_t st) {
+                const std::function<int(int, bool)>& queue_iteration, LoopResult* res, hipStream_t st,
+                const std::function<int(int)>& queue_tail) {
     Event ev0[2] = {Event(true), Event(true)}, ev1[2] = {Event(true), Event(true)}, evCopy;
     const size_t rc_count = (size_t)std::max(max_iter, 1);
-    double* rc_host = (double*)pinned_scratch(2, rc_count * sizeof(double));
+    double* rc_host = (double*)pinned_scratch(2, (rc_count + 4) * sizeof(double));
     if (!rc_host) return fail(FDX_ERR_HIP, "solver: pinned host buffer");
-    for (size_t j = 0; j < rc_count; ++j) rc_host[j] = 0.0;
+    for (size_t j = 0; j < rc_count + 4; ++j) rc_host[j] = 0.0;
     *res = LoopResult();
     res->rel_changes = rc_host;
+    res->tail_sums = rc_host + rc_count;
     int done = 0;
     int chunk = first_chunk > 0 ? first_chunk : 4;
     int queued_ahead = 0;
@@ -145,7 +174,9 @@
         for (int it = done + queued_ahead; it < end; ++it) FDX_TRY(queue_iteration(it, it + 1 == end));
         FDX_TRY(launch_bcd_fold_last(s.stats, s.rel_change, end - 1, st));
         FDX_TRY(ev1[pair].record(st));
-        FDX_HIP(hipMemcpyAsync(rc_host + done, s.rel_change + done, (size_t)(end - done) * sizeof(double), hipMemcpyDeviceToHost, st));
+        if (queue_tail) FDX_TRY(queue_tail(end));
+        const size_t n_copy = queue_tail ? rc_count + 4 - (size_t)done : (size_t)(end - done);
+        FDX_HIP(hipMemcpyAsync(rc_host + done, s.rel_change + done, n_copy * sizeof(double), hipMemcpyDeviceToHost, st));
         FDX_TRY(evCopy.record(st));
         int ahead = 0;
         if (end < max_iter && n_ahead > 0) {
@@ -157,10 +188,11 @@
         float ms_chunk = 0.f;
         FDX_HIP(hipEventElapsedTime(&ms_chunk, ev0[pair].e, ev1[pair].e));
         res->sweep_ms += ms_chunk;
-        for (int it = done; it < end; ++it) {
-            res->n_iter = it + 1;
-            if (rc_host[it] < tol) { res->converged = true; break; }
-        }
+        const int gate = tail_gate_n_iter(rc_host, end, max_iter, tol);
+        res->n_iter = gate < 0 ? end : gate;
+        res->converged = gate > 0 && rc_host[gate - 1] < tol;
+        res->end = end;
+        if (queue_tail && gate >= 0) res->tail_done = true;
         done = end;
         queued_ahead = ahead;
         chunk = std::max(std::min(ci == 0 ? chunk : chunk * 2, 32), ahead);
@@ -222,9 +254,21 @@
         }
         return 0;
     };
+    int route = p.verbose || max_iter <= 0 || K_real != K || !solver_tail_fused_ok(g, p.ld, p.ldh, K) ? (int)TAIL_TWO_KERNELS : p.tail_route;
+    constexpr int kGateUpTo = 8;
+    int gated_end = -1;
+    std::function<int(int)> queue_tail;
+    if (route == TAIL_GATED)
+        queue_tail = [&](int end) -> int {
+            if (end > kGateUpTo && end < max_iter) return 0;
+            gated_end = end;
+            FitTail t = p.tail;
+            t.gate_trace = stats.rel_change; t.gate_end = end; t.gate_max_iter = max_iter; t.tol = p.tol; t.gate_n_iter = nullptr;
+            return solver_fit_tail(g, t, p.beta[0], p.beta[1], p.ld, p.H, p.ldh, p.XtX, K, obj_partials.as<double>(), stats.tail_sums, st);
+        };
     LoopResult loop;
     const int n_ahead = p.verbose ? 0 : 2;
-    FDX_TRY(solver_loop(stats, max_iter, p.tol, p.first_chunk, n_ahead, queue_sweep, &loop, st));
+    FDX_TRY(solver_loop(stats, max_iter, p.tol, p.first_chunk, n_ahead, queue_sweep, &loop, st, queue_tail));
 
     const int n_iter = loop.n_iter;
     res->sweep_ms = loop.sweep_ms;
@@ -235,7 +279,23 @@
     res->rel_changes.assign(loop.rel_changes, loop.rel_changes + n_iter);
     for (auto& t : trace)
         if (t.first < n_iter) { res->objective_iters.push_back(t.first); res->objectives.push_back(t.second); }
-    if (p.compute_objective)
+    if (route == TAIL_GATED) {
+        if (!loop.tail_done) return fail(FDX_ERR_INTERNAL, "solver: the loop ended behind a closed gate");
+        if (gated_end == loop.end)
+            for (int o = 0; o < 4; ++o) res->tail_sums[o] = loop.tail_sums[o];
+        else
+            route = TAIL_FUSED;
+    }
+    res->tail_route = route;
+    if (route == TAIL_FUSED) {
+        FitTail t = p.tail;
+        t.gate_trace = nullptr;
+        FDX_TRY(solver_fit_tail(g, t, p.beta[res->result_buffer], nullptr, p.ld, p.H, p.ldh, p.XtX, K, obj_partials.as<double>(),
+                                obj_out.as<double>(), st));
+        FDX_HIP(hipMemcpyAsync(res->tail_sums, obj_out.p, 4 * sizeof(double), hipMemcpyDeviceToHost, st));
+        FDX_HIP(hipStreamSynchronize(st));
+    }
+    if (p.compute_objective && route == TAIL_TWO_KERNELS)
         FDX_TRY(solver_objective(g, p.beta[res->result_buffer], p.ld, p.H, p.ldh, p.XtX, K, p.YtY, p.lambda, p.rho_eff,
                                  obj_partials.as<double>(), obj_out.as<double>(), &res->final_objective, st));
     return 0;
diff --git a/flashdeconv_amd/csrc/solver.h b/flashdeconv_amd/csrc/solver.h
--- a/flashdeconv_amd/csrc/solver.h
+++ b/flashdeconv_amd/csrc/solver.h
@@ -7,6 +7,17 @@
 #include "fdx_kernels.h"
 
 namespace fdx {
+
+struct FitTail {
+    double* beta_out = nullptr;
+    double* prop_out = nullptr;
+    const int* perm = nullptr;
+    const double* gate_trace = nullptr;
+    int gate_end = 0, gate_max_iter = 0;
+    double tol = 0.0;
+    int* gate_n_iter = nullptr;
+};
+enum TailRoute { TAIL_TWO_KERNELS = 0, TAIL_FUSED = 1, TAIL_GATED = 2 };
 
 struct SolveProblem {
     const fdx_graph* graph = nullptr;
@@ -27,6 +38,8 @@
     int beta0_virtual = 0;
     int compute_objective = 1;
     int first_chunk = 4;
+    int tail_route = TAIL_TWO_KERNELS;
+    FitTail tail;
 };
 
 struct SolveResult {
@@ -39,6 +52,8 @@
     std::vector<int> objective_iters;
     std::vector<double> objectives;
     std::vector<double> rel_changes;
+    int tail_route = TAIL_TWO_KERNELS;
+    double tail_sums[4] = {0.0, 0.0, 0.0, 0.0};
 };
 
 int solver_init_beta(double* beta, long long ld, long long n_fill, int K, hipStream_t st, int K_planes = 0);
@@ -50,6 +65,9 @@
                      const double* XtX, int K, double YtY, double lambda, double rho_eff, double* scratch_partials,
                      double* scratch_out4, double* obj_host, hipStream_t st);
 int solver_run(const SolveProblem& p, SolveResult* res, hipStream_t st);
+bool solver_tail_fused_ok(const fdx_graph& g, long long ld, long long ldh, int K);
+int solver_fit_tail(const fdx_graph& g, const FitTail& t, const double* beta0, const double* beta1, long long ld, const double* H,
+                    long long ldh, const double* XtX, int K, double* scratch_partials, double* out4_dev, hipStream_t st);
 
 BcdSweepArgs sweep_args_for_graph(const fdx_graph& g, bool honour_no_tiled);
 int sweep_scratch_prepare(const double* XtX, int K, int n_slices, DevBuf* scratch, size_t* scratch_ld, hipStream_t st);
@@ -63,6 +81,7 @@
     DevBuf block;
     unsigned long long* stats = nullptr;
     double* rel_change = nullptr;
+    double* tail_sums = nullptr;
     int init(int max_iter, hipStream_t st);
 };
 struct LoopResult {
@@ -70,8 +89,12 @@
     bool converged = false;
     const double* rel_changes = nullptr;
     double sweep_ms = 0.0;
+    int end = 0;
+    bool tail_done = false;
+    const double* tail_sums = nullptr;
 };
 int solver_loop(const SweepStats& s, int max_iter, double tol, int first_chunk, int n_ahead,
-                const std::function<int(int, bool)>& queue_iteration, LoopResult* res, hipStream_t st);
+                const std::function<int(int, bool)>& queue_iteration, LoopResult* res, hipStream_t st,
+                const std::function<int(int)>& queue_tail = nullptr);
 
 }
diff --git a/flashdeconv_amd/csrc/tail_gate.h b/flashdeconv_amd/csrc/tail_gate.h
--- /dev/null
+++ b/flashdeconv_amd/csrc/tail_gate.h
@@ -0,0 +1,17 @@
+#pragma once
+
+#if defined(__HIPCC__)
+#define FDX_GATE_HD __host__ __device__
+#else
+#define FDX_GATE_HD
+#endif
+
+namespace fdx {
+
+FDX_GATE_HD inline int tail_gate_n_iter(const double* rel_change, int end, int max_iter, double tol) {
+    for (int it = 0; it < end; ++it)
+        if (rel_change[it] < tol) return it + 1;
+    return end >= max_iter ? max_iter : -1;
+}
+
+}
diff --git a/include/fdx.h b/include/fdx.h
--- a/include/fdx.h
+++ b/include/fdx.h
@@ -142,6 +142,9 @@
     double* spot_diag_out_dev;
 } fdx_fit_params;
 #define FDX_FIT_TIES 3
+#define FDX_TAIL_TWO_KERNELS 0
+#define FDX_TAIL_FUSED 1
+#define FDX_TAIL_GATED 2
 
 typedef struct fdx_fit_info {
     fdx_solve_info solve;
@@ -153,7 +156,7 @@
     double prologue_ms, span_ms;
     int64_t knn_ties;
     int32_t status;
-    int32_t reserved;
+    int32_t tail_route;
     void* carry;
     double diag_ms;
 } fdx_fit_info;
@@ -290,6 +293,11 @@
                       void* stream);
 int fdx_export_dev(const fdx_graph* g, const double* beta_dev, int64_t ld, int32_t K, double* beta_out_dev, double* prop_out_dev,
                    void* stream);
+
+int fdx_fit_tail_dev(const fdx_graph* g, const double* beta0_dev, const double* beta1_dev, int64_t ld, const double* H_dev, int64_t ldh,
+                     const double* XtX_dev, int32_t K, const double* trace_dev, int32_t end, int32_t max_iter, double tol,
+                     double* beta_out_dev, double* prop_out_dev, double* partials_dev, double* out4_host, int32_t* n_iter_out,
+                     void* stream);
 
 typedef struct fdx_comm fdx_comm;
 typedef struct fdx_local_world fdx_local_world;
```
